# ISLA-UH/quantum-inferno

Measured on AMD Instinct MI355X. Metric: TFR Mpoints/sec (CWT+STX+entropy), higher is better.
Workload: dtype f32; 1 GPU; BASELINE configs[1]: 1 channel(s) per GPU x 2^20 samples @ 1000 Hz, order N=3, CWT+STX+entropy, 48 bands; channels_per_gpu=1, n=1048576, bands=48, engine=auto, world_size=1, backend=none, gather_message_bytes_per_rank=0

## Files before the change

include/qi_tfr.h:

```cpp
#ifndef QI_TFR_H
#define QI_TFR_H

#include <stddef.h>
#include <stdint.h>

#ifdef __cplusplus
extern "C" {
#endif

#define QI_TFR_ABI_VERSION 1

typedef struct qi_plan qi_plan;
typedef void* qi_stream;

typedef enum { QI_F32 = 0, QI_F64 = 1 } qi_dtype;

typedef enum {
  QI_OK = 0,
  QI_ERR_ARG = -1,
  QI_ERR_STATE = -2,
  QI_ERR_HIP = -3,
  QI_ERR_FFT = -4,
  QI_ERR_NOMEM = -5,
  QI_ERR_UNSUPPORTED = -6
} qi_status;

typedef enum {
  QI_BANK_STYX = 0,
  QI_BANK_ATOMS = 1
} qi_bank;

typedef enum {
  QI_ENGINE_AUTO = 0,
  QI_ENGINE_HIPFFT = 1,
  QI_ENGINE_NATIVE = 2
} qi_engine;

typedef struct {
  int64_t n;
  int32_t dtype;
  int32_t device;
  int32_t engine;
  int32_t flags;
  int64_t workspace_bytes;
} qi_plan_desc;

typedef struct {
  void* coef;
  void* bits;
  void* power_band;
  void* power_time;
  void* stats;
  double power_scale;
  double eps;
} qi_tfr_out;

int qi_abi_version(void);
const char* qi_last_error(void);
int qi_device_info(int device, char* name, size_t name_len, int64_t* hbm_bytes, int32_t* compute_units);

int qi_plan_create(qi_plan** plan, const qi_plan_desc* desc);
int qi_plan_destroy(qi_plan* plan);

int qi_plan_set_gabor_bank(qi_plan* plan, int bank, int32_t n_bands, const double* p_re, const double* p_im,
                           const double* omega, const double* amp, qi_stream stream);

int qi_gabor_atoms(int device, int64_t n, int32_t n_bands, const double* p_re, const double* p_im,
                   const double* omega, const double* amp, void* out, qi_stream stream);

int qi_gabor_atoms_at(int device, int64_t n, int32_t n_bands, const double* p_re, const double* p_im,
                      const double* omega, const double* amp, const void* x, void* out, qi_stream stream);

int qi_plan_set_stx_bands(qi_plan* plan, int32_t n_bands, const int64_t* shift_index, const double* sigma);

int64_t qi_plan_bands(const qi_plan* plan, int which );
int64_t qi_plan_stage_bands(const qi_plan* plan, int which, int stage);

int64_t qi_plan_forward_low(const qi_plan* plan, int which );

typedef struct {
  int32_t stage, cls, run_cls, flags;
} qi_band_route;
#define QI_ROUTE_ANALYTIC(f) ((f) & 3)
#define QI_ROUTE_NARROW(f) (((f) >> 2) & 3)
#define QI_ROUTE_NOWRAP 16
#define QI_ROUTE_SPLIT 32
#define QI_ROUTE_PASS2_KIND(f) (((f) >> 6) & 3)
#define QI_ROUTE_BEHIND 256
#define QI_ROUTE_F64_ZOOM 512
int qi_plan_band_route(const qi_plan* plan, int which, int32_t band, int64_t records, qi_band_route* route);

typedef enum {
  QI_STAGE_FORWARD = 0,
  QI_STAGE_MULTIPLY = 1,
  QI_STAGE_INVERSE = 2,
  QI_STAGE_EPILOGUE = 3,
  QI_STAGE_PASS1 = 4,
  QI_STAGE_PASS2 = 5,
  QI_STAGE_BLOCK = 6,
  QI_STAGE_ZOOM = 7,
  QI_STAGE_ZOOM_COARSE = 8,
  QI_STAGE_SMALL = 9,
  QI_STAGE_COUNT = 10
} qi_stage;
int qi_plan_profile(qi_plan* plan, int enable);
int qi_plan_profile_read(qi_plan* plan, double* stage_ms, int64_t* stage_launches, int32_t n_stages);

int qi_cwt(qi_plan* plan, int bank, const void* sig, int64_t n_channels, const qi_tfr_out* out, qi_stream stream);

int qi_stx(qi_plan* plan, const void* sig, int64_t n_channels, const qi_tfr_out* out, qi_stream stream);

int qi_cwt_stx(qi_plan* plan, int bank, const void* sig, int64_t n_channels, const qi_tfr_out* out_cwt,
               const qi_tfr_out* out_stx, qi_stream stream);

int64_t qi_stft_segments(int64_t n, int64_t seg, int64_t hop);
int64_t qi_stft_scratch_bytes(int dtype, int64_t n_channels, int64_t n, int64_t seg, int64_t hop, int64_t nfft);
int qi_stft(int dtype, int device, const void* sig, int64_t n_channels, int64_t n, const void* window, int64_t seg,
            int64_t hop, int64_t nfft, double scale, void* Z, void* bits, double eps, void* scratch,
            int64_t scratch_bytes, qi_stream stream);

int64_t qi_welch_scratch_bytes(int dtype, int64_t n_channels, int64_t n, int64_t seg, int64_t hop, int64_t nfft);
int qi_welch(int dtype, int device, const void* sig, int64_t n_channels, int64_t n, const void* window, int64_t seg,
             int64_t hop, int64_t nfft, double scale, void* pxx, void* scratch, int64_t scratch_bytes,
             qi_stream stream);

int qi_power_marginals(int dtype, int device, const void* power, int64_t n_channels, int64_t n_bands, int64_t n,
                       void* power_band, void* power_time, void* stats, void* scratch, int64_t scratch_bytes,
                       qi_stream stream);
int64_t qi_power_marginals_scratch_bytes(int64_t n_channels, int64_t n_bands, int64_t n);

int qi_log2_offset(int dtype, int device, const void* in, void* out, int64_t n_channels, int64_t count, double eps,
                   const void* ref, qi_stream stream);

int qi_widen(int device, const void* in, void* out, int64_t count, qi_stream stream);

int qi_log2_abs(int dtype, int device, const void* in, int is_complex, void* out, int64_t count, double eps,
                qi_stream stream);

int qi_shannon_panel(int dtype, int device, const void* power, const void* mult, int mode, int64_t n_channels,
                     int64_t n_bands, int64_t n, double deg_free, void* info, void* shannon_bits, void* isnr,
                     void* esnr, qi_stream stream);

int64_t qi_sliding_scratch_bytes(int dtype, int64_t n_channels, int64_t nfft, int64_t n_slices);
int qi_sliding_stft(int dtype, int device, const void* sig, int64_t n_channels, int64_t n, const void* window,
                    int64_t seg, int64_t hop, int64_t nfft, int64_t first, int64_t n_slices, int pad_mode, int detrend,
                    int64_t roll, void* Z, void* real_out, int real_kind, void* scratch, int64_t scratch_bytes,
                    qi_stream stream);
int qi_sliding_istft(int dtype, int device, const void* S, int64_t n_channels, const void* dual_window, int64_t seg,
                     int64_t hop, int64_t nfft, int64_t first, int64_t n_slices, int64_t roll, int64_t k0, int64_t k1,
                     void* out, void* scratch, int64_t scratch_bytes, qi_stream stream);

int qi_shannon_1d(int dtype, int device, const void* marginal, int64_t n_channels, int64_t n, void* info, void* entropy,
                  void* isnr, void* esnr, qi_stream stream);
int64_t qi_shannon_scratch_bytes(int dtype, int64_t n_channels, int64_t n);
int qi_shannon_tdr(int dtype, int device, const void* sig, int64_t n_channels, int64_t n, void* sig_norm, void* marginal,
                   void* scratch, int64_t scratch_bytes, qi_stream stream);
int qi_shannon_fft(int dtype, int device, const void* sig, int64_t n_channels, int64_t n, void* spectrum, void* angle,
                   void* marginal, void* scratch, int64_t scratch_bytes, qi_stream stream);

typedef enum { QI_POOL_NTH = 0, QI_POOL_AVERAGE = 1, QI_POOL_MAX = 2, QI_POOL_MIN = 3, QI_POOL_MEDIAN = 4 } qi_pool_method;
typedef enum { QI_POOL_REAL = 0,
// ... 30 lines not shown
```

quantum_inferno_amd/_lib.py:

```python
import ctypes as C
import os

import torch

_HERE = os.path.dirname(os.path.abspath(__file__))
LIB_PATH = os.environ.get("QI_TFR_LIB") or os.path.join(_HERE, "libqi_tfr.so")

QI_F32, QI_F64 = 0, 1
QI_BANK_STYX, QI_BANK_ATOMS, QI_TABLE_STX = 0, 1, 2
QI_ENGINE_AUTO, QI_ENGINE_HIPFFT, QI_ENGINE_NATIVE = 0, 1, 2
STAGES = ("forward", "multiply", "inverse", "epilogue", "pass1", "pass2", "block", "zoom", "zoom_coarse", "small")
QI_POOL_NTH, QI_POOL_AVERAGE, QI_POOL_MAX, QI_POOL_MIN, QI_POOL_MEDIAN = 0, 1, 2, 3, 4
QI_POOL_REAL, QI_POOL_COMPLEX, QI_POOL_POWER = 0, 1, 2
QI_IIR_BA, QI_IIR_SOS = 0, 1
IIR_MAX = 16
POOL_MEDIAN_MAX = 4096
ROUTE_NOWRAP, ROUTE_SPLIT, ROUTE_BEHIND, ROUTE_F64_ZOOM = 16, 32, 256, 512


def route_analytic(flags):
    return flags & 3


def route_narrow(flags):
    return (flags >> 2) & 3


def route_pass2_kind(flags):
    return (flags >> 6) & 3


class QiError(RuntimeError):
    pass


class PlanDesc(C.Structure):
    _fields_ = [
        ("n", C.c_int64),
        ("dtype", C.c_int32),
        ("device", C.c_int32),
        ("engine", C.c_int32),
        ("flags", C.c_int32),
        ("workspace_bytes", C.c_int64),
    ]


class BandRoute(C.Structure):
    _fields_ = [("stage", C.c_int32), ("cls", C.c_int32), ("run_cls", C.c_int32), ("flags", C.c_int32)]


class TfrOut(C.Structure):
    _fields_ = [
        ("coef", C.c_void_p),
        ("bits", C.c_void_p),
        ("power_band", C.c_void_p),
        ("power_time", C.c_void_p),
        ("stats", C.c_void_p),
        ("power_scale", C.c_double),
        ("eps", C.c_double),
    ]


_P = C.c_void_p
_D = C.POINTER(C.c_double)
_I64 = C.POINTER(C.c_int64)
_i64, _i32, _int, _dbl = C.c_int64, C.c_int32, C.c_int, C.c_double

PROTOTYPES = {
    "qi_abi_version": (_int, []),
    "qi_last_error": (C.c_char_p, []),
    "qi_device_info": (_int, [_int, C.c_char_p, C.c_size_t, _I64, C.POINTER(_i32)]),
    "qi_plan_create": (_int, [C.POINTER(_P), C.POINTER(PlanDesc)]),
    "qi_plan_destroy": (_int, [_P]),
    "qi_plan_set_gabor_bank": (_int, [_P, _int, _i32, _D, _D, _D, _D, _P]),
    "qi_gabor_atoms": (_int, [_int, _i64, _i32, _D, _D, _D, _D, _P, _P]),
    "qi_gabor_atoms_at": (_int, [_int, _i64, _i32, _D, _D, _D, _D, _P, _P, _P]),
    "qi_plan_set_stx_bands": (_int, [_P, _i32, _I64, _D]),
    "qi_plan_bands": (_i64, [_P, _int]),
    "qi_plan_stage_bands": (_i64, [_P, _int, _int]),
    "qi_plan_forward_low": (_i64, [_P, _int]),
    "qi_plan_band_route": (_int, [_P, _int, _i32, _i64, C.POINTER(BandRoute)]),
    "qi_plan_profile": (_int, [_P, _int]),
    "qi_plan_profile_read": (_int, [_P, _D, _I64, _i32]),
    "qi_cwt": (_int, [_P, _int, _P, _i64, C.POINTER(TfrOut), _P]),
    "qi_stx": (_int, [_P, _P, _i64, C.POINTER(TfrOut), _P]),
    "qi_cwt_stx": (_int, [_P, _int, _P, _i64, C.POINTER(TfrOut), C.POINTER(TfrOut), _P]),
    "qi_stft_segments": (_i64, [_i64, _i64, _i64]),
    "qi_stft_scratch_bytes": (_i64, [_int, _i64, _i64, _i64, _i64, _i64]),
    "qi_stft": (_int, [_int, _int, _P, _i64, _i64, _P, _i64, _i64, _i64, _dbl, _P, _P, _dbl, _P, _i64, _P]),
    "qi_stft_out_scratch_bytes": (_i64, [_int, _i64, _i64, _i64, _i64, _i64, _int, _int]),
    "qi_stft_out": (_int, [_int, _int, _P, _i64, _i64, _P, _i64, _i64, _i64, _dbl, C.POINTER(TfrOut), _P, _i64, _P]),
    "qi_welch_scratch_bytes": (_i64, [_int, _i64, _i64, _i64, _i64, _i64]),
    "qi_welch": (_int, [_int, _int, _P, _i64, _i64, _P, _i64, _i64, _i64, _dbl, _P, _P, _i64, _P]),
    "qi_power_marginals": (_int, [_int, _int, _P, _i64, _i64, _i64, _P, _P, _P, _P, _i64, _P]),
    "qi_power_marginals_scratch_bytes": (_i64, [_i64, _i64, _i64]),
    "qi_log2_offset": (_int, [_int, _int, _P, _P, _i64, _i64, _dbl, _P, _P]),
    "qi_widen": (_int, [_int, _P, _P, _i64, _P]),
    "qi_log2_abs": (_int, [_int, _int, _P, _int, _P, _i64, _dbl, _P]),
    "qi_shannon_panel": (_int, [_int, _int, _P, _P, _int, _i64, _i64, _i64, _dbl, _P, _P, _P, _P, _P]),
    "qi_sliding_scratch_bytes": (_i64, [_int, _i64, _i64, _i64]),
    "qi_sliding_stft": (_int, [_int, _int, _P, _i64, _i64, _P, _i64, _i64, _i64, _i64, _i64, _int, _int, _i64, _P, _P, _int, _P, _i64, _P]),
    "qi_sliding_istft": (_int, [_int, _int, _P, _i64, _P, _i64, _i64, _i64, _i64, _i64, _i64, _i64, _i64, _P, _P, _i64, _P]),
    "qi_shannon_1d": (_int, [_int, _int, _P, _i64, _i64, _P, _P, _P, _P, _P]),
    "qi_shannon_scratch_bytes": (_i64, [_int, _i64, _i64]),
    "qi_shannon_tdr": (_int, [_int, _int, _P, _i64, _i64, _P, _P, _P, _i64, _P]),
    "qi_shannon_fft": (_int, [_int, _int, _P, _i64, _i64, _P, _P, _P, _P, _i64, _P]),
    "qi_pool_columns": (_i64, [_i64, _i64, _int]),
    "qi_pool_panel": (_int, [_int, _int, _P, _int, _i64, _i64, _i64, _int, _dbl, _P, _P]),
    "qi_pool_strip": (_int, [_int, _int, _P, _i64, _i64, _i64, _i64, _i64, _dbl, _P, _P, _i64, _P, _P]),
    "qi_pool_strip_stats": (_int, [_int, _P, _i64, _i64, _P, _P]),
    "qi_filtfilt_scratch_bytes": (_i64, [_i64, _i64, _i64]),
    "qi_filtfilt": (_int, [_int, _int, _P, _i64, _i64, _P, _int, _i32, _i32, _D, _D, _i64, _P, _P, _i64, _P]),
}

_lib = None


def _hip_runtimes_mapped():
    try:
        with open("/proc/self/maps") as fh:
            return sorted({ln.split()[-1] for ln in fh if "libamdhip64" in ln})
    except OSError:
        return []


def load():
    global _lib
    if _lib is not None:
        return _lib
    if not os.path.exists(LIB_PATH):
        raise QiError(
            f"{LIB_PATH} is missing: build it with `python -c 'import __graft_entry__ as g; g.build()'` "
            "(hipcc --offload-arch=gfx950).  There is no CPU fallback."
        )
    lib = C.CDLL(LIB_PATH)
    for name, (res, args) in PROTOTYPES.items():
        fn = getattr(lib, name)
        fn.restype = res
        fn.argtypes = args
    rts = _hip_runtimes_mapped()
    if len(rts) > 1:
        raise QiError(f"two HIP runtimes are mapped ({rts}); libqi_tfr.so must share torch's")
    _lib = lib
    return lib


def check(rc):
    if rc != 0:
        msg = load().qi_last_error()
        raise QiError(f"libqi_tfr error {rc}: {msg.decode() if msg else '?'}")


def require_gpu():
    if not torch.cuda.is_available():
        raise QiError("no HIP device visible: the TFR transforms run only on the GPU (no CPU fallback)")
    return load()


def darr(a):
    import numpy as np

    a = np.ascontiguousarray(a, dtype=np.float64)
    return a, a.ctypes.data_as(_D)
# ... 16 lines not shown
```

quantum_inferno_amd/csrc/qi_api.hip:

```cpp
#include "qi_host.hpp"

using namespace qi;
using namespace qi::host;

extern "C" {

int qi_abi_version(void) { return QI_TFR_ABI_VERSION; }
const char* qi_last_error(void) { return qi::last_error(); }

int qi_device_info(int device, char* name, size_t name_len, int64_t* hbm_bytes, int32_t* compute_units) {
  hipDeviceProp_t prop;
  QI_HIP(hipGetDeviceProperties(&prop, device));
  if (name && name_len) snprintf(name, name_len, "%s (%s)", prop.name, prop.gcnArchName);
  if (hbm_bytes) *hbm_bytes = (int64_t)prop.totalGlobalMem;
  if (compute_units) *compute_units = prop.multiProcessorCount;
  return QI_OK;
}

int qi_plan_create(qi_plan** plan, const qi_plan_desc* desc) {
  QI_REQUIRE(plan && desc, "null plan/desc");
  *plan = nullptr;
  QI_REQUIRE(desc->n >= 2 && desc->n <= (1ll << 28), "n = %lld out of range", (long long)desc->n);
  QI_REQUIRE(desc->dtype == QI_F32 || desc->dtype == QI_F64, "bad dtype %d", desc->dtype);
  QI_REQUIRE(desc->engine >= QI_ENGINE_AUTO && desc->engine <= QI_ENGINE_NATIVE, "bad engine %d", desc->engine);
  QI_REQUIRE(desc->flags == 0, "qi_plan_desc.flags = %d: the field is reserved and must be 0", desc->flags);
  if (desc->engine == QI_ENGINE_NATIVE && !(is_pow2(desc->n) && desc->n >= (1 << 18) &&
                                            (desc->dtype == QI_F32 || desc->n == (1 << 20)))) {
    set_error("native engine: float32 records of a power-of-two length >= 2^18, float64 records of 2^20 samples (got n = %lld, dtype %d)",
              (long long)desc->n, desc->dtype);
    return QI_ERR_UNSUPPORTED;
  }
  DeviceGuard g(desc->device);
  if (!g.ok) {
    set_error("hipSetDevice(%d) failed", desc->device);
    return QI_ERR_HIP;
  }
  qi_plan* p = new (std::nothrow) qi_plan();
  QI_REQUIRE(p, "out of host memory");
  p->d = *desc;
  p->n = desc->n;
  p->L = is_pow2(desc->n) ? 2 * desc->n : next_pow2(2 * desc->n - 1);
  if (p->native_kmax > (int64_t)native::kMaxPrunedTerms * native::kN2)
    p->native_kmax = (int64_t)native::kMaxPrunedTerms * native::kN2;
  if (const char* e = tune_env("QI_NATIVE_DEBUG")) p->native_debug = atoi(e);
  if (const char* e = tune_env("QI_NATIVE_FWD")) p->native_fwd = atoi(e);
  if (const char* e = tune_env("QI_NATIVE_FWD_LOW")) p->native_fwd_low = atoi(e);
#ifdef QI_NATIVE_STAMPS
  if (tune_env("QI_NATIVE_STAMPS")) {
    if (hipMalloc((void**)&p->stamps, 65536 * 8 * sizeof(unsigned long long)) != hipSuccess) p->stamps = nullptr;
    if (p->stamps) (void)hipMemset(p->stamps, 0, 65536 * 8 * sizeof(unsigned long long));
    if (hipMalloc((void**)&p->blk_stamps, 65536 * 8 * sizeof(unsigned long long)) != hipSuccess) p->blk_stamps = nullptr;
    if (p->blk_stamps) (void)hipMemset(p->blk_stamps, 0, 65536 * 8 * sizeof(unsigned long long));
  }
#endif
  if (const char* e = tune_env("QI_NATIVE_SHORT")) p->native_short = atoi(e);
  if (const char* e = tune_env("QI_NATIVE_BLOCK")) p->native_block = atoi(e);
  if (const char* e = tune_env("QI_NATIVE_ZOOM")) p->native_zoom = atoi(e);
  if (const char* e = tune_env("QI_NATIVE_ZOOM_LEVELS")) p->native_zoom_max_level = atoi(e);
  if (const char* e = tune_env("QI_NATIVE_SPLIT")) p->native_split = atoi(e);
  if (const char* e = tune_env("QI_NATIVE_FUSE")) p->native_fuse = atoi(e);
  if (const char* e = tune_env("QI_NATIVE_F64")) p->native_f64 = atoi(e);
  if (const char* e = tune_env("QI_NATIVE_Z64")) p->native_z64 = atoi(e);
  if (const char* e = tune_env("QI_NATIVE_Z64_FINE")) p->native_z64_fine = atoi(e);
  if (const char* e = tune_env("QI_NATIVE_Z64_COARSE")) p->native_z64_coarse = atoi(e);
  if (const char* e = tune_env("QI_NATIVE_Z64_BLOCK_FROM")) p->native_z64_block_from = atoi(e);
  if (const char* e = tune_env("QI_NATIVE_BLK64_WTAB")) p->native_blk64_wtab = atoi(e);
  if (const char* e = tune_env("QI_NATIVE_BLK64_NARROW")) p->native_blk64_narrow = atoi(e);
  if (const char* e = tune_env("QI_NATIVE_MIN_LOG2N")) p->native_min_log2n = atoi(e);
  if (desc->dtype == QI_F64) {
    if (!tune_env("QI_NATIVE_MIN_LOG2N")) p->native_min_log2n = 15;
    const int short64 = p->native_short && !(tune_env("QI_NATIVE_SHORT64") && atoi(tune_env("QI_NATIVE_SHORT64")) == 0);
    const int block64 = p->native_block && !(tune_env("QI_NATIVE_BLOCK64") && atoi(tune_env("QI_NATIVE_BLOCK64")) == 0);
    const int split64 = p->native_split && block64 && p->native_z64 &&
                        !(tune_env("QI_NATIVE_SPLIT64") && atoi(tune_env("QI_NATIVE_SPLIT64")) == 0);
    p->native_zoom = 0;
    p->native_split = split64;
    p->native_split_e = 2048;
    p->native_block = block64;
    p->native_short = short64;
    p->native_rows = 8;
    if (p->native_group <= 0) p->native_group = 8;
  }
  p->ws_bytes = desc->workspace_bytes > 0 ? (size_t)desc->workspace_bytes : ((size_t)2 << 30);
  if (hipMalloc((void**)&p->ws, p->ws_bytes) != hipSuccess) {
    set_error("hipMalloc of %zu workspace bytes failed", p->ws_bytes);
    delete p;
    return QI_ERR_HIP;
  }
  if (const char* e = tune_env("QI_SMALL_CHUNK_BANDS")) p->small_chunk_bands = atoi(e);
  if (const char* e = tune_env("QI_SMALL_JOINT")) p->small_joint = atoi(e);
  if (build_small_twiddles(p) != QI_OK) {
    free_device(p->ws);
    delete p;
    return QI_ERR_HIP;
  }
  *plan = p;
  return QI_OK;
}

int qi_plan_destroy(qi_plan* p) {
  if (!p) return QI_OK;
  DeviceGuard g(p->d.device);
  (void)hipDeviceSynchronize();
  p->fft.clear();
  p->prof.clear();
#ifdef QI_NATIVE_STAMPS
  if (p->stamps) {
    std::vector<unsigned long long> h(65536 * 8);
    if (hipMemcpy(h.data(), p->stamps, h.size() * sizeof(unsigned long long), hipMemcpyDeviceToHost) == hipSuccess) {
      double sum[8] = {0};
      long cnt = 0;
      for (size_t w = 0; w < 65536; ++w) {
        unsigned long long tot = 0;
        for (int k = 0; k < 8; ++k) tot += h[w * 8 + k];
        if (!tot) continue;
        ++cnt;
        for (int k = 0; k < 8; ++k) sum[k] += (double)h[w * 8 + k];
      }
      fprintf(stderr, "[qi stamps] last pass-2 launch, %ld workgroups, mean cycles per workgroup: load %.0f | barrier %.0f | "
              "step1 %.0f | barrier %.0f | exchange %.0f | step2 %.0f | epilogue %.0f | loop head %.0f\n", cnt,
              sum[0] / cnt, sum[1] / cnt, sum[2] / cnt, sum[3] / cnt, sum[4] / cnt, sum[5] / cnt, sum[6] / cnt, sum[7] / cnt);
    }
    (void)hipFree(p->stamps);
  }
  if (p->blk_stamps) {
    std::vector<unsigned long long> h(65536 * 8);
    if (hipMemcpy(h.data(), p->blk_stamps, h.size() * sizeof(unsigned long long), hipMemcpyDeviceToHost) == hipSuccess) {
      if (const char* path = tune_env("QI_NATIVE_TIMELINE")) {
        if (FILE* f = fopen(path, "w")) {
// ... 107 lines not shown
  drop_band_slots(p, bank);
  const int rc = build_gabor_bank(p, bank, B, p_re, p_im, omega, amp, use_native, st);
  if (rc == QI_OK) {
    p->nb[bank] = B;
  } else {
    drop_gabor_tables(p, bank);
    free_device(p->bank[bank]);
  }
  return rc;
}

static int atoms_rows(int64_t n, int32_t B, const double* p_re, const double* p_im, const double* omega, const double* amp,
                      const double* x, void* out, hipStream_t st) {
  std::vector<double> host;
  DeviceTemp<double> d_par;
  QI_TRY(upload_atom_params(B, p_re, p_im, omega, amp, &host, &d_par));
  const double* q = d_par.ptr;
  QI_TRY(launch_bank_rows((double2*)out, n, n, 1, q, q + B, q + 2 * B, q + 3 * B, 0, B, st, 0.0, x));
  if (hipStreamSynchronize(st) != hipSuccess) {
    set_error("atom kernel failed: %s", hipGetErrorString(hipGetLastError()));
    return QI_ERR_HIP;
  }
  return QI_OK;
}

int qi_gabor_atoms(int device, int64_t n, int32_t B, const double* p_re, const double* p_im, const double* omega,
                   const double* amp, void* out, qi_stream stream) {
  QI_REQUIRE(p_re && p_im && omega && amp && out, "null argument");
  QI_REQUIRE(n >= 2 && B > 0 && B <= 65535, "bad atom bank shape");
  DeviceGuard g(device);
  return atoms_rows(n, B, p_re, p_im, omega, amp, nullptr, out, (hipStream_t)stream);
}

int qi_gabor_atoms_at(int device, int64_t n, int32_t B, const double* p_re, const double* p_im, const double* omega,
                      const double* amp, const void* x, void* out, qi_stream stream) {
  QI_REQUIRE(p_re && p_im && omega && amp && x && out, "null argument");
  QI_REQUIRE(n >= 1 && B > 0 && B <= 65535, "bad atom bank shape");
  DeviceGuard g(device);
  return atoms_rows(n, B, p_re, p_im, omega, amp, static_cast<const double*>(x), out, (hipStream_t)stream);
}

int qi_plan_set_stx_bands(qi_plan* p, int32_t B, const int64_t* shift_index, const double* sigma) {
  QI_REQUIRE(p && shift_index && sigma, "null argument");
  QI_REQUIRE(B > 0 && B <= 65535, "band count %d out of range", B);
  for (int32_t j = 0; j < B; ++j)
    QI_REQUIRE(shift_index[j] >= 0 && shift_index[j] < p->n, "shift_index[%d] = %lld outside [0, n)", j,
               (long long)shift_index[j]);
  for (int32_t j = 0; j < B; ++j)
    QI_REQUIRE(std::isfinite(sigma[j]) && sigma[j] > 0.0, "sigma[%d] = %g: must be positive and finite", j, sigma[j]);
  DeviceGuard g(p->d.device);
  p->table_gen++;
  if (p->d_stx_idx) {
    QI_HIP(hipDeviceSynchronize());
    QI_HIP(hipFree(p->d_stx_idx));
    QI_HIP(hipFree(p->d_stx_coef));
    p->d_stx_idx = nullptr;
    p->d_stx_coef = nullptr;
    p->nb_stx = 0;
  }
  std::vector<double> coef(B);
  const double k = 2.0 * M_PI / (double)p->n * std::sqrt(0.5 * M_LOG2E);
  for (int32_t j = 0; j < B; ++j) coef[j] = sigma[j] * k;
  QI_TRY(upload_table(&p->d_stx_idx, std::vector<int64_t>(shift_index, shift_index + B)));
  QI_TRY(upload_table(&p->d_stx_coef, coef));
  p->nb_stx = 0;
  drop_stx_tables(p);
  drop_band_slots(p, 2);
  QI_TRY(build_stx_tables(p, B, shift_index, sigma, coef));
  p->nb_stx = B;
  return QI_OK;
}

int64_t qi_plan_bands(const qi_plan* p, int which) {
  if (!p) return 0;
  if (which == QI_BANK_STYX || which == QI_BANK_ATOMS) return p->nb[which];
  return which == 2 ? p->nb_stx : 0;
}

int64_t qi_plan_forward_low(const qi_plan* p, int which) {
  if (!p || which < 0 || which > 2 || !forward_low(p)) return 0;
  return table_low_bins(p, which);
}

int64_t qi_plan_stage_bands(const qi_plan* p, int which, int stage) {
  if (!p || which < 0 || which > 2) return 0;
  const int64_t total = qi_plan_bands(p, which);
  if (on_small(p, which)) return stage == QI_STAGE_SMALL ? total : 0;
  if (!p->nat[which].ready) return stage == QI_STAGE_INVERSE ? total : 0;
  int64_t blk = 0;
  if (which != 1 && p->blk[which].ready) blk = p->blk[which].rows;
  const int64_t zoom = p->nat[which].nzoom + p->nat[which].nz64;
  const int64_t left = which == 2 ? p->stx_left_n : 0;
  if (stage == QI_STAGE_BLOCK) return blk;
  if (stage == QI_STAGE_ZOOM) return zoom;
  if (stage == QI_STAGE_INVERSE) return left;
  return stage == QI_STAGE_PASS2 ? total - blk - zoom - left : 0;
}

int qi_plan_band_route(const qi_plan* p, int which, int32_t band, int64_t records, qi_band_route* route) {
  QI_REQUIRE(p && route, "null argument");
  QI_REQUIRE(which >= 0 && which <= 2, "bad table %d", which);
  QI_REQUIRE(band >= 0 && band < qi_plan_bands(p, which), "band %d outside the table's %lld rows", band,
             (long long)qi_plan_bands(p, which));
  QI_REQUIRE(records > 0, "records must be positive");
  *route = qi_band_route{QI_STAGE_INVERSE, 0, 0, 0};
  const auto& t = p->nat[which];
  if (on_small(p, which)) {
    int32_t lg = 0;
    while (((int64_t)1 << lg) < (which == 0 ? p->L : p->n)) ++lg;
    *route = qi_band_route{QI_STAGE_SMALL, lg, lg, 0};
    return QI_OK;
  }
  if (!t.ready) return QI_OK;
  if (which == 2 && p->stx_left_n > 0 && band >= p->stx_left_lo && band < p->stx_left_lo + p->stx_left_n) {
    route->flags = QI_ROUTE_BEHIND;
    return QI_OK;
  }
  int found = 0;
  const bool split = which == 0 && std::find(p->h_split_bands.begin(), p->h_split_bands.end(), band) != p->h_split_bands.end();
  for (const auto& z : t.h_zoom)
    if (z.first == band) {
      const int run = records < p->native_zoom_short_from && z.second >= native::kZoomLevels ? 0 : z.second;
      *route = qi_band_route{QI_STAGE_ZOOM, z.second, run, split ? QI_ROUTE_SPLIT : 0};
      ++found;
    }
  for (size_t q = 0; q < t.h_z64.size(); ++q)
    if (t.h_z64[q] == band) {
      int level = -1, fine = -1;
      for (int g = 0; g < native::kZ64Levels; ++g)
        if ((int32_t)q >= t.z64_first[g] && (int32_t)q < t.z64_first[g] + t.z64_count[g]) level = g;
      for (int c = 0; c < native::kZ64FineClasses; ++c)
        if ((int32_t)q >= t.zf_first[c] && (int32_t)q < t.zf_first[c] + t.zf_count[c]) fine = c;
      *route = qi_band_route{QI_STAGE_ZOOM, level, fine, QI_ROUTE_F64_ZOOM | (split ? QI_ROUTE_SPLIT : 0)};
      ++found;
    }
  if (which != 1 && p->blk[which].ready) {
    const int cut = records >= batch_from(p) ? 1 : 0;
    for (const auto& b : p->blk[which].var[cut].h_route)
      if (b.out_band == band) {
        *route = qi_band_route{QI_STAGE_BLOCK, b.wq, b.wq, (b.analytic & 3) | ((b.narrow & 3) << 2) | (b.nowrap ? QI_ROUTE_NOWRAP : 0)};
        ++found;
      }
  }
  for (size_t q = 0; q < t.h_rows.size(); ++q)
    if (t.h_rows[q] == band) {
      *route = qi_band_route{QI_STAGE_PASS2, 0, 0, (t.h_row_mode[q] & 3) << 6};
      ++found;
    }
  if (which == 0 && p->nat[3].ready)
    for (int32_t r : p->nat[3].h_rows)
      if (r == band) {
        *route = qi_band_route{QI_STAGE_PASS2, 0, 0, 2 << 6};
        ++found;
      }
  if (found != 1) {
    set_error("band %d of table %d has %d producers", band, which, found);
    return QI_ERR_STATE;
  }
  return QI_OK;
}

int qi_plan_profile(qi_plan* p, int enable) {
  QI_REQUIRE(p, "null plan");
  DeviceGuard g(p->d.device);
  double ms[Profiler::kStages];
  int64_t c[Profiler::kStages];
// ... 152 lines not shown
```

quantum_inferno_amd/csrc/qi_block.hip:

```cpp
#include "qi_common.hpp"
#include "qi_device.hpp"
#include "qi_native.hpp"
#include "qi_fft_reg.hpp"
#include "qi_zoom_gather.hpp"

namespace qi {
namespace native {

namespace {

constexpr int kBlkThreads = 256;
#ifndef QI_BLK_WAVES
#define QI_BLK_WAVES 3
#endif
#ifndef QI_BLK_LONG_WAVES
#define QI_BLK_LONG_WAVES 2
#endif
#ifdef QI_NATIVE_DEBUG
#define QI_BDBG(bit) (a.debug & (bit))
#else
#define QI_BDBG(bit) false
#endif
#ifdef QI_NATIVE_STAMPS
#define QI_BSTAMP(k)                                               \
// ... 194 lines not shown
  fft_reg<T, 16, DIR>(v);
}

template <typename T>
__device__ __forceinline__ void flush_band_sum(const BlockArgs<T>& a, int64_t ch, int64_t blk, int pending, const double* sums,
                                               int tid) {
  if (pending >= 0 && tid == 0) {
    double r = 0.0;
    for (int q = 0; q < kBlkThreads / kWave; ++q) r += sums[q];
    a.part_band[((int64_t)ch * a.panel_bands + pending) * a.nblk + blk] = r;
  }
}

template <typename T>
__device__ __forceinline__ void reduce_stats(const BlockArgs<T>& a, cplx<T>* __restrict__ buf, double r0, double r1, double r2,
                                             int64_t ch, int32_t stat_slot, int tid, bool follows = false, int64_t band_slot = -1) {
  constexpr int NW = kBlkThreads / kWave;
  if (!a.part_stat && band_slot < 0) return;
  const int lane = tid & (kWave - 1), wv = tid / kWave;
  double* fin = reinterpret_cast<double*>(buf);
  if (lane == 0) {
    fin[wv] = r0;
    fin[NW + wv] = r1;
    fin[2 * NW + wv] = r2;
  }
  __syncthreads();
  if (tid == 0) {
    double m = 0.0, s1 = 0.0, s2 = 0.0;
    for (int q = 0; q < NW; ++q) {
      m = fin[q] > m ? fin[q] : m;
      s1 += fin[NW + q];
      s2 += fin[2 * NW + q];
    }
    if (band_slot >= 0 && a.part_band) a.part_band[band_slot] = s1;
    if (a.part_stat) {
      double* o = a.part_stat + ((int64_t)ch * a.stat_stride + a.stat_base + stat_slot) * 3;
      o[0] = follows ? (o[0] > m ? o[0] : m) : m;
      o[1] = follows ? o[1] + s1 : s1;
      o[2] = follows ? o[2] + s2 : s2;
    }
  }
}

template <typename T, bool DEMOD>
__device__ __forceinline__ T gauss_weight(const BlockBandT<T>& bd, int k, bool fold) {
  T dk = (T)(k - bd.kappa_int) - (T)bd.kappa_frac;
  T amp = (T)bd.amp;
  if (fold && dk > (T)(kBlk / 2)) {
    dk -= (T)kBlk;
    if (!DEMOD) amp = -amp;
  }
  if (DEMOD && fold && dk < -(T)(kBlk / 2)) dk += (T)kBlk;
  const T e = (T)bd.cw * dk;
  return amp * fast_exp2(-e * e);
}
template <typename T>
__device__ __forceinline__ T gauss_weight_nowrap(const BlockBandT<T>& bd, T kf) {
  const T e = fma_t((T)bd.cw, kf, -(T)bd.cw * (T)bd.kappa_frac);
  return fast_exp2(fma_t(-e, e, (T)bd.la));
}

template <typename T, bool CIRC>
__device__ __forceinline__ void block_forward(const T* __restrict__ sig, int64_t n, int64_t t0, cplx<T> (&S)[16],
                                              cplx<T>* __restrict__ buf, const cplx<T>* __restrict__ tw256, cplx<T> w,
                                              int tid, int col) {
#pragma unroll
  for (int b = 0; b < 16; ++b) {
    int64_t t = t0 + col + 256 * b;
    T x;
    if (CIRC) {
      t = (t + n) & (n - 1);
      x = sig[t];
    } else {
      x = (t >= 0 && t < n) ? sig[t] : T(0);
    }
    S[b] = mk<T>(x, T(0));
  }
  fft4096<T, -1>(S, buf, tw256, w, tid, col);
  cplx<T> t[16];
#pragma unroll
  for (int c = 0; c < 16; ++c) t[c] = S[brev(c, 4)];
#pragma unroll
  for (int c = 0; c < 16; ++c) S[c] = t[c];
}

template <typename T, int WQ, bool DEMOD, bool COEF, bool BITS, bool EDGE = false>
__device__ __forceinline__ void block_bands(const BlockArgs<T>& a, int32_t blk_i, int32_t band_first, int32_t band_count,
                                            int32_t plane, int32_t stat_slot, cplx<T> (&S)[16], cplx<T>* __restrict__ buf,
                                            const cplx<T>* __restrict__ tw256, double (*s_red)[kBlkThreads / kWave],
                                            cplx<T> w, int col, int edge_piece = 0) {
  static_assert(!EDGE || !DEMOD, "split bands belong to the styx table");
  constexpr int W = 256 * WQ, V = kBlk - 2 * W, NOUT = 16 - 2 * WQ;
  constexpr bool F64 = sizeof(T) == 8;
  const int tid = threadIdx.x, lane = tid & (kWave - 1), wv = tid / kWave;
  const int64_t blk = blk_i, ch = blockIdx.z;
  const int64_t n = a.n;
#ifdef QI_NATIVE_STAMPS
  unsigned long long st_acc[8] = {0, 0, 0, 0, 0, 0, 0, 0};
  unsigned long long st_last = __builtin_amdgcn_s_memtime();
#endif
  const int64_t t0 = blk * V - W;
  if (!DEMOD && !EDGE) {
    const cplx<T> r0 = unit_phasor<T>(-(double)col / (double)kBlk);
    rotate_rows16<T>(S, r0, std::make_integer_sequence<int, 16>{});
  }

  QI_BSTAMP(0);
  T col_p[NOUT];
#pragma unroll
  for (int i = 0; i < NOUT; ++i) col_p[i] = T(0);
  T mx = T(0);
  double plogp = 0.0;
  const uint32_t tb0 = (uint32_t)(t0 + W + col);
  const uint32_t tb_pair = (uint32_t)(t0 + W + kWave * wv + 2 * (lane & 31)) + (lane < 32 ? 0u : 256u);
  int pending = -1, par = 0;

  BlockBandT<T> bd_next{};
  if constexpr (!EDGE) bd_next = load_uniform(a.bands + band_first);
  for (int jj = 0; jj < band_count; ++jj) {
    BlockBandT<T> bd = bd_next;
    if constexpr (EDGE) {
      bd.out_band = a.edge_band[band_first + jj];
    } else {
      if (jj + 1 < band_count) bd_next = load_uniform(a.bands + band_first + jj + 1);
    }
    cplx<T> v[16];
    if (!EDGE && bd.narrow == 1) {
      QI_BSTAMP(1);
      QI_BSTAMP(2);
      const int kres = (col - bd.klo) & 255;
      const int k = (bd.klo + kres) & (kBlk - 1);
      const bool first = (k >> 8) == (bd.klo >> 8);
      const cplx<T> x = pick_pair16<T>(S, __builtin_amdgcn_readfirstlane(bd.klo >> 8), first);
      T r;
      if constexpr (F64) {
        r = a.gauss_w[(int64_t)(band_first + jj) * kBlk + k];
      } else {
        r = gauss_weight<T, DEMOD>(bd, k, true);
      }
      cplx<T> wq = w;
      asm volatile("" : "+v"(wq.x), "+v"(wq.y));
      const cplx<T> om = cmul(wq, first ? mk<T>((T)bd.rot_a[0], (T)bd.rot_a[1]) : mk<T>((T)bd.rot_b[0], (T)bd.rot_b[1]));
      sparse_head16<T>(v, mk<T>(x.x * r, x.y * r), om);
      if (!QI_BDBG(4)) fft4096_tail<T, 1>(v, buf, tw256, tid, col);
    } else if (!EDGE && F64 && a.gauss_w) {
      const T* __restrict__ gw = a.gauss_w + (int64_t)(band_first + jj) * kBlk + col;
      T r[16];
#pragma unroll
      for (int b = 0; b < 16; ++b) r[b] = gw[256 * b];
#pragma unroll
      for (int b = 0; b < 16; ++b) v[b] = mk<T>(S[b].x * r[b], S[b].y * r[b]);
    } else if (!EDGE && (F64 || bd.analytic)) {
      QI_BSTAMP(1);
      QI_BSTAMP(2);
      const bool lower = bd.narrow == 2;
      if (bd.nowrap) {
        const T kf0 = (T)(col - bd.kappa_int);
#pragma unroll
        for (int b = 0; b < 8; ++b) {
          const T r = gauss_weight_nowrap<T>(bd, kf0 + (T)(256 * b));
          v[b] = mk<T>(S[b].x * r, S[b].y * r);
        }
        if (lower) {
#pragma unroll
          for (int b = 8; b < 16; ++b) v[b] = mk<T>(T(0), T(0));
        } else {
// ... 63 lines not shown
    T rowacc = T(0), pl = T(0);
    [[maybe_unused]] const cplx<T> R1 = mk<T>((T)bd.rot[0], (T)bd.rot[1]), R4 = mk<T>((T)bd.rot[4], (T)bd.rot[5]);
    uint32_t tp = tb_pair;
    asm volatile("" : "+v"(tp));
    auto finish_band = [&](auto guard) {
      constexpr bool GUARD = decltype(guard)::value;
      cplx<T> seed = ph, rcur = ph;
#pragma unroll
      for (int i = 0; i < NOUT; i += 2) {
        cplx<T> z[2];
#pragma unroll
        for (int h = 0; h < 2; ++h) {
          z[h] = v[brev(i + h + WQ, 4)];
          if constexpr (DEMOD && F64) {
            if constexpr (COEF)
              if (!QI_BDBG(32)) z[h] = cmul_rn(z[h], cmul_rn(ph, mk<T>(demod_pow[2 * (i + h)], demod_pow[2 * (i + h) + 1])));
          } else if (DEMOD && !QI_BDBG(32)) {
            if (i + h > 0) {
              if (((i + h) & 3) == 0) {
                seed = cmul_rn(seed, R4);
                rcur = seed;
              } else {
                rcur = cmul_rn(rcur, R1);
              }
            }
            z[h] = cmul_rn(z[h], rcur);
          }
        }
        half_swap(z[0].x, z[1].x);
        half_swap(z[0].y, z[1].y);
        const uint32_t tt = tp + 256u * (uint32_t)i;
        const bool inside = !GUARD || tt < (uint32_t)n;
        if constexpr (EDGE) {
          if (inside) {
            const cplx<T> pa = part[tt], pb = part[tt + 1];
            z[0].x += pa.x;
            z[0].y += pa.y;
            z[1].x += pb.x;
            z[1].y += pb.y;
          }
        }
        T lg[2];
#pragma unroll
        for (int h = 0; h < 2; ++h) {
          const T m2 = norm2(z[h].x, z[h].y);
          if (BITS) lg[h] = log2_t(sqrt_t(m2) + a.eps);
          const T p = inside ? mul_rn(a.power_scale, m2) : T(0);
          col_p[i + h] += p;
          rowacc += p;
          mx = max_t(mx, p);
          if constexpr (F64) {
            if (!QI_BDBG(16)) pl += plog2p_flat(p, reinterpret_cast<const double (*)[2]>(tw256 + 256));
          } else {
            if (!QI_BDBG(16)) pl += plog2p(p);
          }
        }
        if (COEF && inside && !QI_BDBG(1)) store_pair(coef_row, tt, z[0], z[1]);
        if (BITS && inside) store_real_pair(bits_row, tt, lg[0], lg[1]);
      }
    };
    if (t0 + W + V > n) finish_band(std::true_type{});
    else finish_band(std::false_type{});
    plogp += (double)pl;
    if (a.part_band && !QI_BDBG(64)) {
      const double r = wave_sum((double)rowacc);
      if (lane == 0) s_red[par][wv] = r;
      pending = bd.out_band;
      par ^= 1;
    }
    QI_BSTAMP(4);
  }
#ifdef QI_NATIVE_STAMPS
  if (a.stamps && tid == 0) {
    unsigned long long* o = a.stamps + ((int64_t)blockIdx.z * gridDim.x + blockIdx.x) * 8;
    for (int k = 0; k < 5; ++k) o[k] = st_acc[k];
    o[5] = (unsigned long long)band_count;
  }
#endif

  T tot = T(0);
  char* __restrict__ time_row = reinterpret_cast<char*>(
      a.time_part ? a.time_part + ((int64_t)ch * a.chunk_total + a.chunk_base + plane) * n : nullptr);
#pragma unroll
  for (int i = 0; i < NOUT; i += 2) {
    tot += col_p[i] + col_p[i + 1];
    const uint32_t tt = tb_pair + 256u * (uint32_t)i;
    if (time_row && tt < (uint32_t)n) store_real_pair(time_row, tt, col_p[i], col_p[i + 1]);
  }
  const double r0 = wave_max((double)mx), r1 = wave_sum((double)tot), r2 = wave_sum(plogp);
  __syncthreads();
  flush_band_sum(a, ch, blk, pending, s_red[par ^ 1], tid);
  reduce_stats(a, buf, r0, r1, r2, ch, stat_slot, tid);
}

template <typename T, int WQ, bool DEMOD, bool COEF, bool BITS>
__device__ __forceinline__ void block_item(const BlockArgs<T>& a, const BlockItem& it, cplx<T>* __restrict__ buf,
                                           const cplx<T>* __restrict__ tw256, double (*s_red)[kBlkThreads / kWave],
                                           cplx<T> w, int col) {
  cplx<T> S[16];
  block_forward<T, DEMOD>(a.sig + (int64_t)blockIdx.z * a.n, a.n, (int64_t)it.block * (kBlk - 512 * WQ) - 256 * WQ, S, buf, tw256,
                          w, threadIdx.x, col);
  block_bands<T, WQ, DEMOD, COEF, BITS>(a, it.block, it.band_first, it.band_count, it.plane, it.stat_slot, S, buf, tw256,
                                        s_red, w, col);
}


template <typename T, bool CIRC>
__device__ __forceinline__ void block_forward8(const T* __restrict__ sig, int64_t n, int64_t t0, cplx<T> (&S)[16],
                                               cplx<T>* __restrict__ buf, const cplx<T>* __restrict__ tw256, cplx<T> w,
                                               cplx<T> w8, int tid, int col) {
  cplx<T> O[16];
#pragma unroll
  for (int par = 1; par >= 0; --par) {
#pragma unroll
    for (int b = 0; b < 16; ++b) {
      int64_t t = t0 + 2 * (col + 256 * b) + par;
      T x;
      if (CIRC) {
        t = (t + n) & (n - 1);
        x = sig[t];
      } else {
        x = (t >= 0 && t < n) ? sig[t] : T(0);
      }
      S[b] = mk<T>(x, T(0));
    }
    fft4096<T, -1>(S, buf, tw256, w, tid, col);
    if (par == 1) {
#pragma unroll
      for (int c = 0; c < 16; ++c) O[c] = S[brev(c, 4)];
    }
  }
  const cplx<T> w8c = cconj<T>(w8);
  cplx<T> t[16];
#pragma unroll
  for (int c = 0; c < 16; ++c) t[c] = S[brev(c, 4)];
  long_combine<T>(S, t, O, w8c, std::make_integer_sequence<int, 16>{});
}

template <typename T, bool DEMOD, bool COEF, bool BITS>
__device__ __forceinline__ void long_bands(const BlockArgs<T>& a, int32_t blk_i, int32_t band_first, int32_t band_count,
                                           int32_t plane, int32_t stat_slot, cplx<T> (&S)[16], cplx<T>* __restrict__ buf,
                                           const cplx<T>* __restrict__ tw256, double (*s_red)[kBlkThreads / kWave],
                                           cplx<T> w, cplx<T> w8, int col) {
  constexpr int W = 1024, V = kBlkLongValid, NOUT = 12, C0 = 2;
  const int tid = threadIdx.x, lane = tid & (kWave - 1), wv = tid / kWave;
  const int64_t blk = blk_i, ch = blockIdx.z, n = a.n;
  const int64_t t0 = blk * V - W;
  if (!DEMOD) {
    float sn, cs;
    sincospif(-(float)col * (1.0f / (float)kBlkLong), &sn, &cs);
    long_rotate<T>(S, mk<T>((T)cs, (T)sn), std::make_integer_sequence<int, 16>{});
  }
  T col_p[2 * NOUT];
#pragma unroll
  for (int i = 0; i < 2 * NOUT; ++i) col_p[i] = T(0);
  T mx = T(0);
  double plogp = 0.0;
  const uint32_t tb0 = (uint32_t)(t0 + 2 * (col + 256 * C0));
  int pending = -1, par = 0;
  BlockBand bd_next = load_uniform(a.bands + band_first);
  for (int jj = 0; jj < band_count; ++jj) {
    const BlockBand bd = bd_next;
    if (jj + 1 < band_count) bd_next = load_uniform(a.bands + band_first + jj + 1);
    const int kres = (col - bd.klo) & 255;
    const int k = (bd.klo + kres) & (kBlk - 1);
    const bool first = (k >> 8) == (bd.klo >> 8);
    const cplx<T> x = pick_pair16<T>(S, __builtin_amdgcn_readfirstlane(bd.klo >> 8), first);
    const T r = gauss_weight<T, DEMOD>(bd, k, false);
    const cplx<T> y = mk<T>(x.x * r, x.y * r);
    cplx<T> wq = w, wq8 = w8;
    asm volatile("" : "+v"(wq.x), "+v"(wq.y), "+v"(wq8.x), "+v"(wq8.y));
    const cplx<T> om = cmul(wq, first ? mk<T>((T)bd.rot_a[0], (T)bd.rot_a[1]) : mk<T>((T)bd.rot_b[0], (T)bd.rot_b[1]));
    const cplx<T> tw_odd = cmul(wq8, first ? mk<T>((T)bd.rot8_a[0], (T)bd.rot8_a[1]) : mk<T>((T)bd.rot8_b[0], (T)bd.rot8_b[1]));
    cplx<T> v[16];
    cplx<T> ph = mk<T>(T(1), T(0)), ph1 = ph;
    if (DEMOD) {
      const uint32_t m = (0u - (uint32_t)bd.shift * tb0) & (uint32_t)(n - 1);
      float s, c;
      sincospif((float)m * a.two_over_n, &s, &c);
      ph = mk<T>((T)c, (T)s);
      ph1 = mk<T>((T)bd.rot1[0], (T)bd.rot1[1]);
    }
    const int64_t orow = ((int64_t)ch * a.panel_bands + bd.out_band) * n;
    char* __restrict__ coef_row = reinterpret_cast<char*>(a.coef ? a.coef + orow : nullptr);
    char* __restrict__ bits_row = reinterpret_cast<char*>(a.bits ? a.bits + orow : nullptr);
    uint32_t tb = tb0;
    asm volatile("" : "+v"(tb));
    T rowacc = T(0), pl = T(0);
    const cplx<T> R1 = mk<T>((T)bd.rot[2], (T)bd.rot[3]), R4 = mk<T>((T)bd.rot[6], (T)bd.rot[7]);
    {
      cplx<T> ze[NOUT];
      sparse_head16<T>(v, y, om);
      fft4096_tail<T, 1>(v, buf, tw256, tid, col);
#pragma unroll
      for (int i = 0; i < NOUT; ++i) ze[i] = v[brev(i + C0, 4)];
      sparse_head16<T>(v, cmul(y, tw_odd), om);
      fft4096_tail<T, 1>(v, buf, tw256, tid, col);
      flush_band_sum(a, ch, blk, pending, s_red[par ^ 1], tid);
      auto finish_band = [&](auto guard) {
      constexpr bool GUARD = decltype(guard)::value;
      cplx<T> seed = ph, rcur = ph;
#pragma unroll
      for (int i = 0; i < NOUT; ++i) {
        cplx<T> z[2] = {ze[i], v[brev(i + C0, 4)]};
        if (DEMOD) {
          if (i > 0) {
            if ((i & 3) == 0) {
              seed = cmul_rn(seed, R4);
              rcur = seed;
            } else {
              rcur = cmul_rn(rcur, R1);
            }
          }
          z[0] = cmul_rn(z[0], rcur);
          z[1] = cmul_rn(z[1], cmul_rn(rcur, ph1));
        }
        const uint32_t tt = tb + 512u * (uint32_t)i;
        const bool inside = !GUARD || tt < (uint32_t)n;
        T lg[2];
#pragma unroll
        for (int hh = 0; hh < 2; ++hh) {
          const T m2 = norm2(z[hh].x, z[hh].y);
          if (BITS) lg[hh] = log2_t(sqrt_t(m2) + a.eps);
          const T p = inside ? mul_rn(a.power_scale, m2) : T(0);
          col_p[2 * i + hh] += p;
          rowacc += p;
          mx = max_t(mx, p);
          pl += plog2p(p);
        }
        if (COEF && inside)
          stream_store(reinterpret_cast<float4*>(coef_row + (size_t)(tt * (uint32_t)sizeof(cplx<T>))),
                       make_float4(z[0].x, z[0].y, z[1].x, z[1].y));
        if (BITS && inside) *reinterpret_cast<float2*>(bits_row + (size_t)(tt * (uint32_t)sizeof(T))) = make_float2(lg[0], lg[1]);
      }
      };
      if (t0 + W + V > n) finish_band(std::true_type{});
      else finish_band(std::false_type{});
    }
    plogp += (double)pl;
    if (a.part_band) {
      const double rs = wave_sum((double)rowacc);
      if (lane == 0) s_red[par][wv] = rs;
      pending = bd.out_band;
      par ^= 1;
    }
  }
  T tot = T(0);
  char* __restrict__ time_row = reinterpret_cast<char*>(
      a.time_part ? a.time_part + ((int64_t)ch * a.chunk_total + a.chunk_base + plane) * n : nullptr);
#pragma unroll
  for (int i = 0; i < NOUT; ++i) {
    tot += col_p[2 * i] + col_p[2 * i + 1];
    const uint32_t tt = tb0 + 512u * (uint32_t)i;
    if (time_row && tt < (uint32_t)n)
      *reinterpret_cast<float2*>(time_row + (size_t)(tt * (uint32_t)sizeof(T))) = make_float2(col_p[2 * i], col_p[2 * i + 1]);
  }
  const double r0 = wave_max((double)mx), r1 = wave_sum((double)tot), r2 = wave_sum(plogp);
  __syncthreads();
  flush_band_sum(a, ch, blk, pending, s_red[par ^ 1], tid);
  reduce_stats(a, buf, r0, r1, r2, ch, stat_slot, tid);
}

template <typename T, bool DEMOD, bool COEF, bool BITS>
__device__ __forceinline__ void long_item(const BlockArgs<T>& a, const BlockItem& it, cplx<T>* __restrict__ buf,
                                          const cplx<T>* __restrict__ tw256, double (*s_red)[kBlkThreads / kWave], cplx<T> w,
                                          cplx<T> w8, int col) {
  cplx<T> S[16];
  block_forward8<T, DEMOD>(a.sig + (int64_t)blockIdx.z * a.n, a.n, (int64_t)it.block * kBlkLongValid - 1024, S, buf, tw256, w, w8,
                           threadIdx.x, col);
  long_bands<T, DEMOD, COEF, BITS>(a, it.block, it.band_first, it.band_count, it.plane, it.stat_slot, S, buf, tw256, s_red, w, w8,
                                   col);
}

template <typename T, bool COEF, bool BITS>
__device__ __forceinline__ void long_dual_item(const BlockArgs<T>& a0, const BlockArgs<T>& a2, const DualItem& it,
                                               cplx<T>* __restrict__ buf, const cplx<T>* __restrict__ tw256,
                                               double (*s_red)[kBlkThreads / kWave], cplx<T> w, cplx<T> w8, int col) {
  const int tid = threadIdx.x;
  const int64_t n = a0.n, t0 = (int64_t)it.block * kBlkLongValid - 1024;
  const bool inside = t0 >= 0 && t0 + kBlkLong <= n;
  const T* sig = a0.sig + (int64_t)blockIdx.z * n;
  cplx<T> S[16];
  if (it.count2 > 0 || inside) block_forward8<T, true>(sig, n, t0, S, buf, tw256, w, w8, tid, col);
  if (it.count2 > 0)
    long_bands<T, true, COEF, BITS>(a2, it.block, it.first2, it.count2, it.plane2, it.slot2, S, buf, tw256, s_red, w, w8, col);
  if (it.count0 > 0) {
    if (!inside) block_forward8<T, false>(sig, n, t0, S, buf, tw256, w, w8, tid, col);
    long_bands<T, false, COEF, BITS>(a0, it.block, it.first0, it.count0, it.plane0, it.slot0, S, buf, tw256, s_red, w, w8, col);
  }
}

template <typename T, int WQ, bool COEF, bool BITS>
__device__ __forceinline__ void dual_item(const BlockArgs<T>& a0, const BlockArgs<T>& a2, const DualItem& it,
                                          cplx<T>* __restrict__ buf, const cplx<T>* __restrict__ tw256,
                                          double (*s_red)[kBlkThreads / kWave], cplx<T> w, int col) {
  const int tid = threadIdx.x;
  const int64_t n = a0.n, t0 = (int64_t)it.block * (kBlk - 512 * WQ) - 256 * WQ;
  const bool inside = t0 >= 0 && t0 + kBlk <= n;
  const T* sig = a0.sig + (int64_t)blockIdx.z * n;
  cplx<T> S[16];
  if (it.count2 > 0 || inside) block_forward<T, true>(sig, n, t0, S, buf, tw256, w, tid, col);
  if (it.count2 > 0)
    block_bands<T, WQ, true, COEF, BITS>(a2, it.block, it.first2, it.count2, it.plane2, it.slot2, S, buf, tw256, s_red, w, col);
  if (it.count0 > 0) {
    if (!inside) block_forward<T, false>(sig, n, t0, S, buf, tw256, w, tid, col);
    block_bands<T, WQ, false, COEF, BITS>(a0, it.block, it.first0, it.count0, it.plane0, it.slot0, S, buf, tw256, s_red, w, col);
  }
}

template <typename T, int WQ, bool COEF, bool BITS>
__device__ __forceinline__ void edge_item(const BlockArgs<T>& a, const BlockItem& it, cplx<T>* __restrict__ buf,
                                          const cplx<T>* __restrict__ tw256, cplx<T> w, int col, bool follows = false) {
  constexpr int W = 256 * WQ, V = kBlk - 2 * W, NOUT = 16 - 2 * WQ;
  const int tid = threadIdx.x;
  const int64_t n = a.n, ch = blockIdx.z, blk = it.block;
  const int sb = it.band_first, out_band = a.edge_band[sb];
  const int64_t t0 = blk * V - W;
  const T* __restrict__ sig = a.sig + ch * n;
  const cplx<T>* __restrict__ bank = a.edge_bank + (int64_t)sb * 2 * kBlk;
  const cplx<T>* __restrict__ part = a.edge_part + (ch * a.nsplit + sb) * n;
  const uint32_t tb = (uint32_t)(t0 + W + col);
  cplx<T> z0[NOUT];
#pragma unroll
  for (int i = 0; i < NOUT; ++i) {
    const uint32_t t = tb + 256u * (uint32_t)i;
    z0[i] = t < (uint32_t)n ? part[t] : mk<T>(T(0), T(0));
  }
  cplx<T> acc[16];
#pragma unroll
  for (int b = 0; b < 16; ++b) acc[b] = mk<T>(T(0), T(0));
  for (int piece = 0; piece < 2; ++piece) {
    const int64_t in0 = t0 + (piece == 0 ? n / 2 - W : -(n / 2 - W));
    if (in0 >= n || in0 + kBlk <= 0) continue;
    cplx<T> S[16];
#pragma unroll
// ... 231 lines not shown
  fft4096<double, 1>(v, buf, tw256, w, tid, col);
  double2* __restrict__ z = a.Z + ((int64_t)ch * a.nbands + band) * (a.M + 2 * kZ64Pad) + kZ64Pad;
#pragma unroll
  for (int c = 0; c < 16; ++c) {
    const int64_t tau = (int64_t)P * (col + 256 * c) + tau1;
    const double2 val = v[brev(c, 4)];
    z[tau] = val;
    if (tau < kZ64Pad) z[a.M + tau] = val;
    if (tau >= a.M - kZ64Pad) z[tau - a.M] = val;
  }
}

template <typename T, bool DEMOD, bool COEF, bool BITS>
__global__ void __launch_bounds__(kBlkThreads, QI_BLK_LONG_WAVES) k_block_long(BlockArgs<T> a, const BlockItem* __restrict__ items) {
  __shared__ cplx<T> buf[kBlkBuf];
  __shared__ cplx<T> tw256[256];
  __shared__ double s_red[2][kBlkThreads / kWave];
  const int tid = threadIdx.x, col = fft4096_col(tid);
  const cplx<T> w = fft4096_setup<T>(tw256, tid, col), w8 = long_setup_w8<T>(col);
  long_item<T, DEMOD, COEF, BITS>(a, load_uniform(items + blockIdx.x), buf, tw256, s_red, w, w8, col);
}
template <typename T, bool COEF, bool BITS>
__global__ void __launch_bounds__(kBlkThreads, QI_BLK_LONG_WAVES) k_block_long_dual(BlockArgs<T> a0, BlockArgs<T> a2,
                                                                                    const DualItem* __restrict__ items) {
  __shared__ cplx<T> buf[kBlkBuf];
  __shared__ cplx<T> tw256[256];
  __shared__ double s_red[2][kBlkThreads / kWave];
  const int tid = threadIdx.x, col = fft4096_col(tid);
  const cplx<T> w = fft4096_setup<T>(tw256, tid, col), w8 = long_setup_w8<T>(col);
  long_dual_item<T, COEF, BITS>(a0, a2, load_uniform(items + blockIdx.x), buf, tw256, s_red, w, w8, col);
}

template <typename T, bool COEF, bool BITS>
__global__ void __launch_bounds__(kBlkThreads, QI_BLK_WAVES) k_block_dual(BlockArgs<T> a0, BlockArgs<T> a2,
                                                                         const DualItem* __restrict__ items) {
  __shared__ cplx<T> buf[kBlkBuf];
  __shared__ cplx<T> tw256[256];
  __shared__ double s_red[2][kBlkThreads / kWave];
  const int tid = threadIdx.x, col = fft4096_col(tid);
  const cplx<T> w = fft4096_setup<T>(tw256, tid, col);
  const DualItem it = load_uniform(items + blockIdx.x);
#ifdef QI_NATIVE_STAMPS
  const unsigned long long wall0 = __builtin_amdgcn_s_memrealtime();
#endif
  if (it.wq < 0) {
    const BlockItem e{it.wq, it.block, it.first0, it.count0, it.plane0, it.slot0};
    QI_WITH_REACH(-it.wq, edge_item<T, WQ, COEF, BITS>(a0, e, buf, tw256, w, col));
  } else {
    QI_WITH_REACH(it.wq, dual_item<T, WQ, COEF, BITS>(a0, a2, it, buf, tw256, s_red, w, col));
  }
#ifdef QI_NATIVE_STAMPS
  if (a0.stamps && tid == 0) {
    asm volatile("s_waitcnt vmcnt(0) lgkmcnt(0)" ::: "memory");
    unsigned long long* o = a0.stamps + ((int64_t)blockIdx.z * gridDim.x + blockIdx.x) * 8;
    unsigned hw;
    asm volatile("s_getreg_b32 %0, hwreg(HW_REG_HW_ID)" : "=s"(hw));
    unsigned xcc;
    asm volatile("s_getreg_b32 %0, hwreg(HW_REG_XCC_ID)" : "=s"(xcc));
    o[6] = (wall0 & 0xffffffffffffull) | ((unsigned long long)(xcc & 15) << 56) | ((unsigned long long)((hw >> 8) & 0xff) << 48);
    o[7] = (__builtin_amdgcn_s_memrealtime() & 0xffffffffffffull) | ((unsigned long long)(it.wq & 0xff) << 56) |
           ((unsigned long long)((it.count0 + it.count2) & 0xff) << 48);
  }
#endif
}

template <typename T>
__device__ __forceinline__ void zoom_coarse_plane(cplx<T>* __restrict__ plane0) {
  __shared__ cplx<T> buf[kBlkBuf];
  __shared__ cplx<T> tw256[256];
  const int tid = threadIdx.x, col = fft4096_col(tid);
  cplx<T>* __restrict__ plane = plane0 + col;
  cplx<T> v[16];
#pragma unroll
  for (int b = 0; b < 16; ++b) v[b] = plane[256 * b];
  const cplx<T> w = fft4096_setup<T>(tw256, tid, col);
  fft4096<T, 1>(v, buf, tw256, w, tid, col);
#pragma unroll
  for (int c = 0; c < 16; ++c) plane[256 * c] = v[brev(c, 4)];
}
template <typename T, bool STX, int NF>
__device__ __forceinline__ void zoom_coarse_plane_gather(const ZoomArgs<T>& a, const uint32_t plane_i,
                                                         cplx<T>* __restrict__ buf, cplx<T>* __restrict__ tw256) {
  const int tid = threadIdx.x, col = fft4096_col(tid);
  const BandDesc bd = load_uniform(a.bands + *as_const(a.plane_band + plane_i));
  const uint32_t tau1 = plane_i - (uint32_t)bd.edge;
  const int64_t ch = blockIdx.z;
  const cplx<T>* __restrict__ X = a.X + ch * ((int64_t)a.x_mask + 1);
  cplx<T> v[16];
#ifdef QI_NATIVE_DEBUG
  if (a.debug & 256) {
#pragma unroll
    for (int b = 0; b < 16; ++b) v[b] = mk<T>((T)(col + b), (T)tau1);
  } else
#endif
  zoom_gather16<T, STX, NF>(a, bd, tau1, col, X, v);
  const cplx<T> w = fft4096_setup<T>(tw256, tid, col);
#ifdef QI_NATIVE_DEBUG
  if (!(a.debug & 512))
#endif
  fft4096<T, 1>(v, buf, tw256, w, tid, col);
  cplx<T>* __restrict__ plane = a.coarse + ((int64_t)ch * a.planes + plane_i) * kBlk + col;
#ifdef QI_NATIVE_DEBUG
  if ((a.debug & 1024) && v[3].x != (T)12345.678f) return;
#endif
#pragma unroll
  for (int c = 0; c < 16; ++c) plane[256 * c] = v[brev(c, 4)];
}
template <typename T, int NF>
__global__ void __launch_bounds__(kBlkThreads) k_zoom_coarse2g(ZoomArgs<T> a0, ZoomArgs<T> a2) {
  __shared__ cplx<T> buf[kBlkBuf];
  __shared__ cplx<T> tw256[256];
#ifdef QI_COARSE_PLAIN_ORDER
  const uint32_t pi = blockIdx.x;
#else
  const uint32_t q = blockIdx.x >> 3, pi = (q >> 3) * 64u + (blockIdx.x & 7u) * 8u + (q & 7u);
#endif
  if (pi >= (uint32_t)(a0.planes + a2.planes)) return;
  if (pi < (uint32_t)a0.planes) zoom_coarse_plane_gather<T, false, NF>(a0, pi, buf, tw256);
  else zoom_coarse_plane_gather<T, true, NF>(a2, pi - (uint32_t)a0.planes, buf, tw256);
}
template <typename T, bool STX>
__global__ void __launch_bounds__(kBlkThreads) k_zoom_coarse_g(ZoomArgs<T> a) {
  __shared__ cplx<T> buf[kBlkBuf];
  __shared__ cplx<T> tw256[256];
  zoom_coarse_plane_gather<T, STX, 8>(a, blockIdx.x, buf, tw256);
}

template <typename T>
__global__ void __launch_bounds__(kBlkThreads) k_zoom_coarse(ZoomArgs<T> a) {
  zoom_coarse_plane<T>(a.coarse + ((int64_t)blockIdx.z * a.planes + blockIdx.x) * kBlk);
}
template <typename T>
__global__ void __launch_bounds__(kBlkThreads) k_zoom_coarse2(ZoomArgs<T> a0, ZoomArgs<T> a2) {
  const bool first = blockIdx.x < (uint32_t)a0.planes;
  const ZoomArgs<T>& a = first ? a0 : a2;
  const int64_t plane = first ? blockIdx.x : blockIdx.x - (uint32_t)a0.planes;
  zoom_coarse_plane<T>(a.coarse + ((int64_t)blockIdx.z * a.planes + plane) * kBlk);
}

__global__ void k_block_taps_gabor(double2* __restrict__ g, int w, const double* __restrict__ par, int nb_total,
                                   const int32_t* __restrict__ ids) {
  const int j = ids[blockIdx.y];
  const double p_re = par[j], p_im = par[nb_total + j], omega = par[2 * nb_total + j], amp = par[3 * nb_total + j];
  double2* row = g + (int64_t)blockIdx.y * kBlk;
  for (int m = blockIdx.x * blockDim.x + threadIdx.x; m < kBlk; m += gridDim.x * blockDim.x) {
    int u;
    bool on = true;
    if (m <= w) u = -m;
    else if (m > kBlk - w) u = kBlk - m;
    else { u = 0; on = false; }
    double2 v = make_double2(0.0, 0.0);
    if (on) {
      const double x = (double)u + 0.5;
      const double env = amp * exp(-p_re * x * x);
      const double ph = omega * x - p_im * x * x;
      double s, c;
      sincos(ph, &s, &c);
      v = make_double2(env * c, -env * s);
    }
    row[m] = v;
  }
}


__global__ void k_block_taps_edge(double2* __restrict__ g, int w, int64_t n, double taper_e,
                                  const double* __restrict__ par, int nb_total, const int32_t* __restrict__ ids) {
  const int j = ids[blockIdx.y >> 1], piece = blockIdx.y & 1;
// ... 307 lines not shown
```

quantum_inferno_amd/csrc/qi_host.hpp:

```cpp
#pragma once
#include <algorithm>
#include <cmath>
#include <cstring>
#include <map>
#include <mutex>
#include <new>
#include <tuple>
#include <vector>

#include <cstdlib>

#include "qi_common.hpp"
#include "qi_native.hpp"

namespace qi {

struct DeviceGuard {
  int prev = -1;
  bool ok = true;
  explicit DeviceGuard(int dev) {
    if (hipGetDevice(&prev) != hipSuccess) prev = -1;
    if (prev != dev) ok = hipSetDevice(dev) == hipSuccess;
  }
  ~DeviceGuard() {
// ... 136 lines not shown
      }
    }
    for (auto e : used) pool.push_back(e);
    used.clear();
    spans.clear();
    cur = last = -1;
  }
  void clear() {
    double ms[kStages];
    int64_t c[kStages];
    read(ms, c);
    for (auto e : pool) (void)hipEventDestroy(e);
    pool.clear();
  }
};

template <typename P>
inline void free_device(P*& ptr) {
  if (ptr) (void)hipFree(ptr);
  ptr = nullptr;
}
template <typename P, typename X>
inline int upload_table(P** dst, const std::vector<X>& v) {
  QI_HIP(hipMalloc((void**)dst, v.size() * sizeof(X)));
  QI_HIP(hipMemcpy(*dst, v.data(), v.size() * sizeof(X), hipMemcpyHostToDevice));
  return QI_OK;
}
template <typename X>
struct DeviceTemp {
  X* ptr = nullptr;
  DeviceTemp() = default;
  DeviceTemp(const DeviceTemp&) = delete;
  DeviceTemp& operator=(const DeviceTemp&) = delete;
  ~DeviceTemp() { free_device(ptr); }
};

extern std::mutex g_stft_mu;
extern std::map<int, FftCache> g_stft_fft;
const char* last_error();

}

using namespace qi;

struct FusedCarry {
  bool active = false;
  size_t ws_used = 0;
  native::BlockArgs<float> blk{};
  int demod = 0;
  int64_t ct = 0;
  native::TailCall<float> tail;
  bool has_zoom = false;
  native::ZoomArgs<float> zoom{};
};

struct qi_plan {
  qi_plan_desc d{};
  int64_t n = 0;
  int64_t L = 0;
  void* bank[2] = {nullptr, nullptr};
  int32_t nb[2] = {0, 0};
  int64_t* d_stx_idx = nullptr;
  double* d_stx_coef = nullptr;
  int32_t nb_stx = 0;
  char* ws = nullptr;
  size_t ws_bytes = 0;
  FftCache fft;
  Profiler prof;
  struct NativeGroup {
    int32_t first = 0, count = 0;
    int32_t gen_first = 0, ngen = 0;
  };
  struct NativeTable {
    bool ready = false;
    int64_t Lf = 0;
    int32_t nbands = 0, ngen = 0, imd_slots = 0;
    native::BandDesc* d_bands = nullptr;
    int32_t* d_gen_list = nullptr;
    std::vector<NativeGroup> groups;
    void* Hc = nullptr;
    void* Hfull = nullptr;
    native::BandDesc* d_zoom = nullptr;
    int32_t* d_zoom_plane_band = nullptr;
    std::vector<std::pair<int32_t, int32_t>> h_zoom;
    std::vector<int32_t> h_rows;
    std::vector<int32_t> h_row_mode;
    std::vector<int32_t> h_z64;
    int32_t nzoom = 0, zoom_count[native::kZoomClasses] = {0, 0, 0, 0, 0, 0, 0};
    int64_t x_lo = 0, x_hi = -1;
    int64_t zoom_planes = 0;
    int zoom_max_level = 0;
    native::BandDesc* d_z64 = nullptr;
    int32_t nz64 = 0, z64_first[native::kZ64Levels] = {}, z64_count[native::kZ64Levels] = {};
    int32_t zf_first[native::kZ64FineClasses] = {}, zf_count[native::kZ64FineClasses] = {};
    double2* d_z64_lane_ph = nullptr;
    double2* d_z64_wave_ph = nullptr;
    void release() {
      free_device(d_z64);
      free_device(d_z64_lane_ph);
      free_device(d_z64_wave_ph);
      free_device(d_zoom);
      free_device(d_zoom_plane_band);
      free_device(d_bands);
      free_device(d_gen_list);
      free_device(Hc);
      free_device(Hfull);
      *this = NativeTable();
    }
  } nat[4];
  struct BlockTable {
    bool ready = false;
    int demod = 0;
    void* bank = nullptr;
    int32_t rows = 0;
    struct ItemList {
      void* d_bands = nullptr;
      void* d_demod_pow = nullptr;
      void* d_gauss_w = nullptr;
      std::vector<std::pair<int32_t, int32_t>> h_bands;
      struct Route {
        int32_t out_band, wq, analytic, narrow, nowrap;
      };
      std::vector<Route> h_route;
      native::BlockItem* d_items = nullptr;
      int32_t nitems = 0, nplanes = 0;
      int32_t nlong = 0;
      int32_t nedge_items = 0;
      bool edge_merged = false;
      std::vector<native::BlockItem> h_items;
    } var[2];
    int64_t max_blocks = 0;
    void release() {
      free_device(bank);
      for (auto& v : var) {
        free_device(v.d_bands);
        free_device(v.d_demod_pow);
        free_device(v.d_gauss_w);
        free_device(v.d_items);
      }
      *this = BlockTable();
    }
  } blk[3];
  struct {
    int64_t C = -1, tile = 0;
    unsigned flags = 0;
    uint64_t gen = 0;
  } tile_cache;
  uint64_t table_gen = 1;
  int native_block = 1;
  const void* shared_sig = nullptr;
  int64_t shared_C = 0;
  bool shared_valid = false;
  int32_t* d_band_slots[3][2] = {};
  int native_zoom = 1;
  int native_zoom_short = 1;
  int native_zoom_short_from = 4;
  int native_zoom_max_level = 3;
  int native_zoom_waves = 2048;
  int native_zoom_wgs_joint = 768;
  int native_zoom_wgs = 0;
  float* d_zoom_w[native::kZoomClasses] = {};
  int native_z64 = 1;
  int native_z64_levels = native::kZ64Levels;
  double* d_z64_w[native::kZ64Levels] = {};
  double* d_z64f_w[native::kZ64FineClasses] = {};
  double2* d_demod_t1 = nullptr;
  double2* d_demod_t2 = nullptr;
  int native_z64_fine = 1;
  int32_t stx_left_lo = -1, stx_left_n = 0;
  void* small_tw = nullptr;
  int small_chunk_bands = 2;
  int small_joint = 2;
  int native_min_log2n = 14;
  int native_blk64_narrow = 1;
  int native_blk64_wtab = 1;
  int native_z64_block_from = 4;
  int native_z64_coarse = 3;
  int native_z64_rows = 0;
  int native_f64 = 1;
  int native_gather_fused = 1;
  hipStream_t side = nullptr;
  hipEvent_t ev_fork = nullptr, ev_join = nullptr;
  int native_split = 1;
  int64_t native_split_e = 1024;
  void* split_bank = nullptr;
  int32_t* d_split_bands = nullptr;
  std::vector<int32_t> h_split_bands;
  int32_t nsplit = 0;
  int native_blk_analytic = 1;
  FusedCarry carry;
  native::DualItem* d_dual[2] = {nullptr, nullptr};
  int32_t n_dual[2] = {0, 0};
  int32_t n_dual_long[2] = {0, 0};
  bool dual_valid[2] = {false, false};
  int native_fuse = 4;
  int native_blk_narrow = 1;
  int native_blk_fastw = 1;
  int native_edge_merge = 1;
  int native_blk_long = 1;
  int native_blk_half = 1;
  int native_tail = 1;
  int64_t native_tile = 0;
  int native_blk_maxwq = 4;
  int native_blk_bands = 6;
  int native_blk_bands_batch = 12;
  int native_blk_batch_from = 0;
  native::EdgeBand* d_edge = nullptr;
  int32_t nedge = 0;
  int64_t edge_wmax = 0;
  int native_short = 1;
  int64_t native_kmax = 12288;
  int native_debug = 0;
  int native_fwd = 1;
  int native_fwd_low = 1;
  int native_wgs = 256;
  unsigned long long* stamps = nullptr;
  unsigned long long* blk_stamps = nullptr;
  int native_group = 0;
  int native_rows = 16;
};

namespace qi {
namespace host {

inline size_t align_up(size_t v, size_t a = 256) { return (v + a - 1) / a * a; }
inline double power_scale_or_default(double power_scale) { return power_scale == 0.0 ? 1.0 : power_scale; }
inline double eps_or_default(double eps) { return eps == 0.0 ? 2.220446049250313e-16 : eps; }
enum class Kind { Linear, Circular, Stockwell };
#ifdef QI_HOST_SANITIZE
void layout_begin(const qi_plan* p, const char* run, bool keep_previous);
void layout_note(const qi_plan* p, const char* what, const void* ptr, size_t bytes, bool shared = false);
#define QI_LAYOUT_BEGIN(p, run, keep) ::qi::host::layout_begin(p, run, keep)
#define QI_LAYOUT_NOTE(p, what, ptr, bytes, ...) ::qi::host::layout_note(p, what, ptr, bytes, ##__VA_ARGS__)
#else
#define QI_LAYOUT_BEGIN(p, run, keep) ((void)0)
#define QI_LAYOUT_NOTE(p, what, ptr, bytes, ...) ((void)0)
#endif
constexpr int kZoomListOrder[native::kZoomClasses] = {6, 5, 0, 1, 2, 3, 4};

bool native_len_ok(int64_t Lf);
bool native_wanted(const qi_plan* p, int kind);
int64_t table_low_bins(const qi_plan* p, int kind);
bool forward_low(const qi_plan* p);
int batch_from(const qi_plan* p);
void release_styx_extras(qi_plan* p);
void drop_gabor_tables(qi_plan* p, int bank);
void drop_stx_tables(qi_plan* p);
void drop_band_slots(qi_plan* p, int kind);
int upload_atom_params(int32_t B, const double* p_re, const double* p_im, const double* omega, const double* amp,
                       std::vector<double>* host, DeviceTemp<double>* d_par);
template <typename T>
int build_native_bank(qi_plan* p, int bank, int32_t B, const double* d_par, const double* h_par, hipStream_t st);
template <typename T>
int build_bank(qi_plan* p, int bank, int32_t B, const double* d_par, hipStream_t st);
int build_stx_tables(qi_plan* p, int32_t B, const int64_t* shift_index, const double* sigma, const std::vector<double>& coef);

bool small_wanted(const qi_plan* p, int kind);
bool on_small(const qi_plan* p, int kind);
int build_small_twiddles(qi_plan* p);

template <typename T>
int run_transform(qi_plan* p, Kind kind, const void* sig_v, int64_t C, const qi_tfr_out* out, hipStream_t st);
template <typename T>
int run_native(qi_plan* p, int kind, const void* sig_v, int64_t C, const qi_tfr_out* out, hipStream_t st,
               bool may_share = false, FusedCarry* defer = nullptr, FusedCarry* finish = nullptr, size_t* probe = nullptr);
template <typename T>
int run_stx_leftover(qi_plan* p, const void* sig, int64_t C, const qi_tfr_out* out, hipStream_t st);
template <typename T>
int run_small(qi_plan* p, int njobs, const int* kinds, const qi_tfr_out* const* outs, const void* sig_v, int64_t C, hipStream_t st,
              bool* ran);
int run_native64(qi_plan* p, int kind, const void* sig_v, int64_t C, const qi_tfr_out* out, hipStream_t st);
int flush_carry(qi_plan* p, FusedCarry* c, hipStream_t st);

}
}
```

quantum_inferno_amd/csrc/qi_native.hip:

```cpp
#include <utility>

#include "qi_common.hpp"
#include "qi_device.hpp"
#include "qi_native.hpp"
#include "qi_fft_reg.hpp"
#include "qi_finalize.hpp"

namespace qi {
namespace native {

namespace {

template <typename T, int G_ = 16>
struct Cfg {
  static constexpr int NR = 1024, G = G_, TH = 64 * G_;
  static constexpr int SR = NR + 1;
  static constexpr int SA = 16 * G + 1;
  static constexpr int BUF = (G * SR > 64 * SA) ? G * SR : 64 * SA;
  static constexpr int TW1 = (kMaxPrunedTerms + 1) * G;
  static constexpr int TW2 = 64;
  static constexpr size_t LDS_BYTES = ((size_t)BUF + NR + TW2 + TW1) * sizeof(cplx<T>) + 256;
};

#ifdef QI_NATIVE_DEBUG
// ... 464 lines not shown
    T rowacc = T(0), pl = T(0);
    if (KIND == 1 && !COEF && bd.edge > 0 && a.edge_z) {
      cplx<T>* ez = a.edge_z + ((int64_t)ch * a.nedge + bd.edge_slot) * 2 * a.edge_wmax;
      const uint32_t t_lo = tb, t_hi = (uint32_t)a.n - 1u - (tb + 15u * tstep);
      if (t_lo < (uint32_t)bd.edge) ez[t_lo] = u[brev(8, 4)];
      if (t_hi < (uint32_t)bd.edge) ez[a.edge_wmax + t_hi] = u[brev(7, 4)];
    }
#pragma unroll
    for (int i = 0; i < NOUT; ++i) {
      const int c = KIND == 0 ? i + 4 : (KIND == 1 ? ((i + 8) & 15) : i);
      const cplx<T> z = u[brev(c, 4)];
      const uint32_t tt = tb + (uint32_t)i * tstep;
      if (COEF && !QI_DBG(1)) stream_store(reinterpret_cast<cplx<T>*>(coef_row + (size_t)(tt * (uint32_t)sizeof(cplx<T>))), z);
      const T m2 = norm2(z.x, z.y);
      if (BITS) *reinterpret_cast<T*>(bits_row + (size_t)(tt * (uint32_t)sizeof(T))) = log2_t(sqrt_t(m2) + a.eps);
      T p = mul_rn(a.power_scale, m2);
      if (KIND == 1) {
        const bool inside = (uint32_t)(tt - (uint32_t)bd.edge) < (uint32_t)(a.n - 2 * (int64_t)bd.edge);
        p = inside ? p : T(0);
      }
      col[i] += p;
      if (!QI_DBG(8)) {
        rowacc += p;
        mx = max_t(mx, p);
        pl += plog2p(p, ltab);
      }
    }
    plogp += (double)pl;
    if (a.part_band) {
      const double r = wave_sum((double)rowacc);
      if (lane == 0) s_red[par][wv] = r;
      pending = j;
      par ^= 1;
    }
    QI_STAMP(6);
  }
#ifdef QI_NATIVE_STAMPS
  if (a.stamps && tid == 0) {
    unsigned long long* o = a.stamps + ((((int64_t)ch * gridDim.y + blockIdx.y) * gridDim.x + blockIdx.x) * 8);
    for (int k = 0; k < 8; ++k) o[k] = st_acc[k];
  }
#endif

  __syncthreads();
  if (pending >= 0 && tid == 0) {
    double s = 0.0;
    for (int w = 0; w < C::TH / kWave; ++w) s += s_red[par ^ 1][w];
    a.part_band[((int64_t)ch * a.panel_bands + pending) * a.nblk + grp] = s;
  }
  T tot = T(0);
  char* __restrict__ time_row =
      reinterpret_cast<char*>(a.time_part ? a.time_part + ((int64_t)ch * a.chunk_total + a.chunk_base + blockIdx.y) * a.n
                                          : nullptr);
#pragma unroll
  for (int i = 0; i < NOUT; ++i) {
    tot += col[i];
    const uint32_t tt = tbase + (uint32_t)i * tstep;
    if (time_row) *reinterpret_cast<T*>(time_row + (size_t)(tt * (uint32_t)sizeof(T))) = col[i];
  }
  if (a.part_stat) {
    const double r0 = wave_max((double)mx), r1 = wave_sum((double)tot), r2 = wave_sum(plogp);
    if (lane == 0) {
      s_fin[0][wv] = r0;
      s_fin[1][wv] = r1;
      s_fin[2][wv] = r2;
    }
    __syncthreads();
    if (tid == 0) {
      double m = 0.0, s1 = 0.0, s2 = 0.0;
      for (int w = 0; w < C::TH / kWave; ++w) {
        m = s_fin[0][w] > m ? s_fin[0][w] : m;
        s1 += s_fin[1][w];
        s2 += s_fin[2][w];
      }
      double* o = a.part_stat + ((int64_t)ch * a.stat_stride + (int64_t)(a.chunk_base + blockIdx.y) * a.stat_nblk + grp) * 3;
      o[0] = m;
      o[1] = s1;
      o[2] = s2;
    }
  }
}

template <typename T, int VEC>
__device__ __forceinline__ void time_reduce_block(const T* __restrict__ part, T* __restrict__ out, int64_t n, int nchunk,
                                                  const T* __restrict__ edge_time, int64_t wmax, int64_t bx, int64_t gx,
                                                  int64_t c) {
  struct alignas(sizeof(T) * VEC) Pack {
    T v[VEC];
  };
  for (int64_t t = (bx * blockDim.x + threadIdx.x) * VEC; t < n; t += gx * blockDim.x * VEC) {
    if (t + VEC <= n) {
      Pack s = *reinterpret_cast<const Pack*>(part + (c * nchunk) * n + t);
      for (int q = 1; q < nchunk; ++q) {
        const Pack x = *reinterpret_cast<const Pack*>(part + (c * nchunk + q) * n + t);
#pragma unroll
        for (int i = 0; i < VEC; ++i) s.v[i] += x.v[i];
      }
      if (edge_time) {
#pragma unroll
        for (int i = 0; i < VEC; ++i) {
          if (t + i < wmax) s.v[i] += edge_time[(c * 2 + 0) * wmax + t + i];
          if (t + i >= n - wmax) s.v[i] += edge_time[(c * 2 + 1) * wmax + (n - 1 - t - i)];
        }
      }
      *reinterpret_cast<Pack*>(out + c * n + t) = s;
    } else {
      for (int64_t u = t; u < n; ++u) {
        T s = T(0);
        for (int q = 0; q < nchunk; ++q) s += part[(c * nchunk + q) * n + u];
        if (edge_time) {
          if (u < wmax) s += edge_time[(c * 2 + 0) * wmax + u];
          if (u >= n - wmax) s += edge_time[(c * 2 + 1) * wmax + (n - 1 - u)];
        }
        out[c * n + u] = s;
      }
    }
  }
}
template <typename T, int VEC>
__global__ void __launch_bounds__(256) k_time_reduce(const T* __restrict__ part, T* __restrict__ out, int64_t n, int nchunk,
                                                     const T* __restrict__ edge_time, int64_t wmax) {
  time_reduce_block<T, VEC>(part, out, n, nchunk, edge_time, wmax, blockIdx.x, gridDim.x, blockIdx.y);
}

struct TailFin {
  const double* part_band;
  const double* part_stat;
  double* power_band;
  double* stats;
  int64_t B, nblk, nstat;
  const int32_t* band_slots;
};
template <typename T, int VEC>
__global__ void __launch_bounds__(256) k_tail(const T* __restrict__ part, T* __restrict__ out, int64_t n, int nchunk,
                                              const T* __restrict__ edge_time, int64_t wmax, TailFin f, int nfin) {
  __shared__ double s[3][256 / kWave];
  if ((int)blockIdx.x < nfin) {
    finalize_block(f.part_band, f.part_stat, f.power_band, f.stats, f.B, f.nblk, f.nstat, f.band_slots, blockIdx.x,
                   blockIdx.y, s);
    return;
  }
  time_reduce_block<T, VEC>(part, out, n, nchunk, edge_time, wmax, (int64_t)blockIdx.x - nfin, (int64_t)gridDim.x - nfin,
                            blockIdx.y);
}

template <typename T>
__global__ void k_even_bins(const cplx<T>* __restrict__ x2, cplx<T>* __restrict__ x1, int64_t n) {
  const int64_t k = (int64_t)blockIdx.x * blockDim.x + threadIdx.x, c = blockIdx.y;
  if (k < n) x1[c * n + k] = x2[c * 2 * n + 2 * k];
}

template <typename T>
__global__ void __launch_bounds__(256) k_edge_fix(EdgeArgs<T> a) {
  const int lane = threadIdx.x & (kWave - 1), wv = threadIdx.x / kWave;
  const int64_t e = blockIdx.y, c = blockIdx.z;
  const EdgeBand eb = a.bands[e];
  const int64_t o = (int64_t)blockIdx.x * (256 / kWave) + wv;
  const int side = o >= a.wmax ? 1 : 0;
  const int64_t tloc = o - (int64_t)side * a.wmax;
  if (tloc >= eb.w) return;
  const int64_t cnt = eb.w - tloc;
  const int64_t t = side ? a.n - 1 - tloc : tloc;
  const T* __restrict__ sig = a.sig + c * a.n;
  T sr = T(0), si = T(0);
  const int64_t m0 = side ? 0 : a.n - eb.w + t;
  const double x0 = (side ? (double)(1 + tloc) : (double)(-eb.w)) + 0.5;
  const int64_t chunk = (cnt + kWave - 1) / kWave;
  if constexpr (sizeof(T) == 8) {
    for (int64_t i = lane; i < cnt; i += kWave) {
      const double x = x0 + (double)i;
      const double ph = eb.omega * x - eb.p_im * x * x;
      const double turns = ph * 0.15915494309189535;
      double sn, cs;
      sincospi(2.0 * (turns - rint(turns)), &sn, &cs);
      const double env = eb.amp * exp(-(eb.p_re * x * x));
      const double v = (double)sig[m0 + i] * env;
      sr += (T)(v * cs);
      si -= (T)(v * sn);
    }
  } else if (eb.p_im == 0.0 && chunk >= 4) {
    const int64_t i0 = (int64_t)lane * chunk;
    const int64_t i1 = i0 + chunk < cnt ? i0 + chunk : cnt;
    if (i0 < i1) {
      const double x = x0 + (double)i0;
      const double turns = eb.omega * x * 0.15915494309189535;
      float sn, cs, sw, cw;
      sincospif(2.0f * (float)(turns - rint(turns)), &sn, &cs);
      const double tw_ = eb.omega * 0.15915494309189535;
      sincospif(2.0f * (float)(tw_ - rint(tw_)), &sw, &cw);
      float env = (float)eb.amp * expf(-(float)(eb.p_re * x * x));
      float ratio = expf(-(float)(eb.p_re * (2.0 * x + 1.0)));
      const float ratio2 = expf(-(float)(2.0 * eb.p_re));
      float pr = cs, pi = -sn;
      for (int64_t i = i0; i < i1; ++i) {
        const T v = sig[m0 + i] * (T)env;
        sr += v * (T)pr;
        si += v * (T)pi;
        const float nr = pr * cw + pi * sw;
        pi = pi * cw - pr * sw;
        pr = nr;
        env *= ratio;
        ratio *= ratio2;
      }
    }
  } else {
    for (int64_t i = lane; i < cnt; i += kWave) {
      const double x = x0 + (double)i;
      const double ph = eb.omega * x - eb.p_im * x * x;
      const double turns = ph * 0.15915494309189535;
      float sn, cs;
      sincospif(2.0f * (float)(turns - rint(turns)), &sn, &cs);
      const float env = (float)eb.amp * expf(-(float)(eb.p_re * x * x));
      const T v = sig[m0 + i] * (T)env;
      sr += v * (T)cs;
      si -= v * (T)sn;
    }
  }
  sr = wave_sum(sr);
  si = wave_sum(si);
  if (lane == 0) {
    const int64_t row = (c * a.panel_bands + eb.out_band) * a.n;
    cplx<T> z = a.coef ? a.coef[row + t] : a.edge_z[((c * a.nedge + e) * 2 + side) * a.wmax + tloc];
    z.x -= sr;
    z.y -= si;
    if (a.coef) a.coef[row + t] = z;
// ... 186 lines not shown

template <typename T, class C1, bool LOW>
static int launch_forward_p1(const RowArgs<T>& a0, int64_t n_channels, hipStream_t st) {
  RowArgs<T> a = a0;
  a.phase_split = a.N1 == 2048 && (a.N2 / C1::G) * n_channels < 256 ? 1 : 0;
  dim3 g1((unsigned)(a.N2 / C1::G), a.phase_split ? 2u : 1u, (unsigned)n_channels);
  if (a.N1 == 1024) return launch_p1<T, C1, 2, 1, LOW>(a, g1, st);
  if (a.N1 == 2048) return launch_p1<T, C1, 2, 2, LOW>(a, g1, st);
  set_error("native forward transform supports N1 = 1024 or 2048, got %lld", (long long)a.N1);
  return QI_ERR_UNSUPPORTED;
}
template <typename T, class C1>
static int launch_forward_cfg(const RowArgs<T>& a, cplx<T>* Xout, int64_t n_channels, hipStream_t st) {
  using C2 = C1;
  QI_TRY((launch_forward_p1<T, C1, false>(a, n_channels, st)));
  auto kern = k_fwd2<T, C2>;
  QI_TRY(allow_dynamic_lds(reinterpret_cast<const void*>(kern), C2::LDS_BYTES));
  dim3 g2((unsigned)(a.N1 / C2::G), 1, (unsigned)n_channels);
  kern<<<g2, C2::TH, C2::LDS_BYTES, st>>>(a, Xout);
  QI_LAUNCH_CHECK();
  return QI_OK;
}
template <typename T, class C2>
static int launch_fwd2_low(const RowArgs<T>& a, cplx<T>* Xlow, int64_t n_channels, hipStream_t st) {
  auto kern = k_fwd2_low<T, C2>;
  QI_TRY(allow_dynamic_lds(reinterpret_cast<const void*>(kern), C2::LDS_BYTES));
  dim3 g2((unsigned)ceil_div(fwd_low_rows(a.N1), C2::G), 1, (unsigned)n_channels);
  kern<<<g2, C2::TH, C2::LDS_BYTES, st>>>(a, Xlow);
  QI_LAUNCH_CHECK();
  return QI_OK;
}
template <>
int launch_forward<float>(const RowArgs<float>& a, float2* Xout, int64_t n_channels, hipStream_t st, bool low) {
  const bool few = n_channels * (a.N2 / 16) < 256;
  if (!low) {
    if (few) return launch_forward_cfg<float, Cfg<float, 8>>(a, Xout, n_channels, st);
    return launch_forward_cfg<float, Cfg<float, 16>>(a, Xout, n_channels, st);
  }
  if (few) QI_TRY((launch_forward_p1<float, Cfg<float, 8>, true>(a, n_channels, st)));
  else QI_TRY((launch_forward_p1<float, Cfg<float, 16>, true>(a, n_channels, st)));
  const int64_t rows = fwd_low_rows(a.N1) * n_channels;
  if (rows >= 256 * 16) return launch_fwd2_low<float, Cfg<float, 16>>(a, Xout, n_channels, st);
  if (rows >= 256 * 8) return launch_fwd2_low<float, Cfg<float, 8>>(a, Xout, n_channels, st);
  return launch_fwd2_low<float, Cfg<float, 4>>(a, Xout, n_channels, st);
}
template <>
int launch_forward<double>(const RowArgs<double>& a, double2* Xout, int64_t n_channels, hipStream_t st, bool low) {
  if (low) {
    set_error("the low-bins forward transform is float32 only");
    return QI_ERR_UNSUPPORTED;
  }
  return launch_forward_cfg<double, Cfg<double, 8>>(a, Xout, n_channels, st);
}

template <typename T, class C>
static int launch_pass2_cfg(const RowArgs<T>& a, int kind, int nchunk, int64_t n_channels, hipStream_t st) {
  dim3 grid((unsigned)(a.N1 / C::G), (unsigned)nchunk, (unsigned)n_channels);
  switch (kind) {
    case 0: return launch_p2<T, C, 0>(a, grid, st);
    case 1: return launch_p2<T, C, 1>(a, grid, st);
    default: return launch_p2<T, C, 2>(a, grid, st);
  }
}
template <>
int launch_pass2<double>(const RowArgs<double>& a, int kind, int rows_per_group, int nchunk, int64_t n_channels,
                         hipStream_t st) {
  if (rows_per_group != 8) {
    set_error("float64 pass 2 runs 8 rows per workgroup, got %d", rows_per_group);
    return QI_ERR_UNSUPPORTED;
  }
  return launch_pass2_cfg<double, Cfg<double, 8>>(a, kind, nchunk, n_channels, st);
}

template <>
int launch_pass2<float>(const RowArgs<float>& a, int kind, int rows_per_group, int nchunk, int64_t n_channels,
                        hipStream_t st) {
  if (rows_per_group == 16) return launch_pass2_cfg<float, Cfg<float, 16>>(a, kind, nchunk, n_channels, st);
  if (rows_per_group == 8) return launch_pass2_cfg<float, Cfg<float, 8>>(a, kind, nchunk, n_channels, st);
  set_error("pass 2 supports 8 or 16 rows per workgroup, got %d", rows_per_group);
  return QI_ERR_UNSUPPORTED;
}

template <typename T>
int launch_time_reduce(const T* part, T* out, int64_t C, int64_t n, int nchunk, const T* edge_time, int64_t wmax,
                       hipStream_t st) {
  const bool aligned = n % 4 == 0 && reinterpret_cast<uintptr_t>(out) % (4 * sizeof(T)) == 0 &&
                       reinterpret_cast<uintptr_t>(part) % (4 * sizeof(T)) == 0;
  if (aligned) {
    dim3 g((unsigned)(ceil_div(n, 1024) > 4096 ? 4096 : ceil_div(n, 1024)), (unsigned)C);
    k_time_reduce<T, 4><<<g, 256, 0, st>>>(part, out, n, nchunk, edge_time, wmax);
  } else {
    dim3 g((unsigned)(ceil_div(n, 256) > 4096 ? 4096 : ceil_div(n, 256)), (unsigned)C);
    k_time_reduce<T, 1><<<g, 256, 0, st>>>(part, out, n, nchunk, edge_time, wmax);
  }
  QI_LAUNCH_CHECK();
  return QI_OK;
}
template <typename T>
struct TailPack {
  const T* part;
  T* out;
  int64_t n;
  int nchunk, nfin;
  TailFin f;
};
template <typename T, int VEC>
__global__ void __launch_bounds__(256) k_tail2(TailPack<T> p0, TailPack<T> p1) {
  __shared__ double s[3][256 / kWave];
  const TailPack<T>& p = blockIdx.z == 0 ? p0 : p1;
  if ((int)blockIdx.x < p.nfin) {
    finalize_block(p.f.part_band, p.f.part_stat, p.f.power_band, p.f.stats, p.f.B, p.f.nblk, p.f.nstat, p.f.band_slots,
                   blockIdx.x, blockIdx.y, s);
    return;
  }
  time_reduce_block<T, VEC>(p.part, p.out, p.n, p.nchunk, nullptr, 0, (int64_t)blockIdx.x - p.nfin,
                            (int64_t)gridDim.x - p.nfin, blockIdx.y);
}

template <typename T>
int launch_tail(const TailCall<T>& t, hipStream_t st) {
  const bool aligned = t.n % 4 == 0 && reinterpret_cast<uintptr_t>(t.out_time) % (4 * sizeof(T)) == 0 &&
                       reinterpret_cast<uintptr_t>(t.time_part) % (4 * sizeof(T)) == 0;
  if (!aligned) {
    if (int rc = launch_time_reduce<T>(t.time_part, t.out_time, t.ct, t.n, t.chunk_total, t.edge_time, t.wmax, st)) return rc;
    return launch_finalize(t.part_band, t.part_stat, t.power_band, t.stats, t.ct, t.B, t.nbk, t.stat_slots, st, t.band_slots);
  }
  const TailFin f{t.part_band, t.part_stat, t.power_band, t.stats, t.B, t.nbk, t.stat_slots, t.band_slots};
  const int nfin = (int)t.B + 1;
  const int64_t gt = ceil_div(t.n, 1024) > 4096 ? 4096 : ceil_div(t.n, 1024);
  dim3 g((unsigned)(gt + nfin), (unsigned)t.ct);
  k_tail<T, 4><<<g, 256, 0, st>>>(t.time_part, t.out_time, t.n, t.chunk_total, t.edge_time, t.wmax, f, nfin);
  QI_LAUNCH_CHECK();
  return QI_OK;
}

template <typename T>
int launch_tail2(const TailCall<T>& t0, const TailCall<T>& t1, hipStream_t st) {
  const int64_t n = t1.n;
  const bool aligned = n % 4 == 0 && reinterpret_cast<uintptr_t>(t0.out_time) % 16 == 0 &&
                       reinterpret_cast<uintptr_t>(t0.time_part) % 16 == 0 && reinterpret_cast<uintptr_t>(t1.out_time) % 16 == 0 &&
                       reinterpret_cast<uintptr_t>(t1.time_part) % 16 == 0;
  if (!aligned) {
    if (int rc = launch_tail<T>(t0, st)) return rc;
    return launch_tail<T>(t1, st);
  }
  TailPack<T> p0{t0.time_part, t0.out_time, n, t0.chunk_total, (int)t0.B + 1,
                 TailFin{t0.part_band, t0.part_stat, t0.power_band, t0.stats, t0.B, t0.nbk, t0.stat_slots, t0.band_slots}};
  TailPack<T> p1{t1.time_part, t1.out_time, n, t1.chunk_total, (int)t1.B + 1,
                 TailFin{t1.part_band, t1.part_stat, t1.power_band, t1.stats, t1.B, t1.nbk, t1.stat_slots, t1.band_slots}};
  const int64_t gt = ceil_div(n, 1024) > 4096 ? 4096 : ceil_div(n, 1024);
  const int nfin = p0.nfin > p1.nfin ? p0.nfin : p1.nfin;
  dim3 g((unsigned)(gt + nfin), (unsigned)t1.ct, 2);
  k_tail2<T, 4><<<g, 256, 0, st>>>(p0, p1);
  QI_LAUNCH_CHECK();
  return QI_OK;
}
template int launch_tail2<float>(const TailCall<float>&, const TailCall<float>&, hipStream_t);
template int launch_tail2<double>(const TailCall<double>&, const TailCall<double>&, hipStream_t);
template int launch_tail<float>(const TailCall<float>&, hipStream_t);
template int launch_tail<double>(const TailCall<double>&, hipStream_t);
template int launch_time_reduce<float>(const float*, float*, int64_t, int64_t, int, const float*, int64_t, hipStream_t);
template int launch_time_reduce<double>(const double*, double*, int64_t, int64_t, int, const double*, int64_t,
                                        hipStream_t);

template <typename T>
int launch_even_bins(const cplx<T>* x2, cplx<T>* x1, int64_t C, int64_t n, hipStream_t st) {
  dim3 g((unsigned)ceil_div(n, 256), (unsigned)C);
  k_even_bins<T><<<g, 256, 0, st>>>(x2, x1, n);
  QI_LAUNCH_CHECK();
  return QI_OK;
}
template int launch_even_bins<float>(const float2*, float2*, int64_t, int64_t, hipStream_t);
template int launch_even_bins<double>(const double2*, double2*, int64_t, int64_t, hipStream_t);

template <typename T>
int launch_edge(const EdgeArgs<T>& a, int64_t C, T* edge_time, double* part_band, int64_t nblk, int64_t band_slot,
                double* part_stat, int64_t stat_slot, hipStream_t st) {
  if (a.nedge <= 0) return QI_OK;
  dim3 g((unsigned)ceil_div(2 * a.wmax, 256 / kWave), (unsigned)a.nedge, (unsigned)C);
  k_edge_fix<T><<<g, 256, 0, st>>>(a);
  QI_LAUNCH_CHECK();
  dim3 gr((unsigned)(a.nedge + ceil_div(2 * a.wmax, 256)), (unsigned)C);
  k_edge_reduce<T><<<gr, 256, 0, st>>>(a, edge_time, part_band, nblk, band_slot, part_stat, stat_slot);
  QI_LAUNCH_CHECK();
  return QI_OK;
}
template int launch_edge<float>(const EdgeArgs<float>&, int64_t, float*, double*, int64_t, int64_t, double*, int64_t,
                                hipStream_t);
template int launch_edge<double>(const EdgeArgs<double>&, int64_t, double*, double*, int64_t, int64_t, double*, int64_t,
                                 hipStream_t);

int launch_band_support(const double2* F, int64_t L, int nb, double thr2, double* out, hipStream_t st) {
  k_band_support<<<nb, 256, 0, st>>>(F, L, thr2, out);
  QI_LAUNCH_CHECK();
  return QI_OK;
}

template <typename T>
int launch_copy_window(const double2* F, cplx<T>* dst, int64_t k_lo, int64_t count, int conj, double scale,
                       int64_t row_len, hipStream_t st, double ramp, int64_t ramp_center) {
  k_copy_window<T><<<(unsigned)ceil_div(count, 256), 256, 0, st>>>(F, dst, k_lo, count, conj, scale, row_len, ramp, ramp_center);
  QI_LAUNCH_CHECK();
  return QI_OK;
}
template int launch_copy_window<float>(const double2*, float2*, int64_t, int64_t, int, double, int64_t, hipStream_t, double,
                                       int64_t);
template int launch_copy_window<double>(const double2*, double2*, int64_t, int64_t, int, double, int64_t, hipStream_t,
                                        double, int64_t);

}
}
```

quantum_inferno_amd/csrc/qi_native.hpp:

```cpp
#pragma once
#include "qi_common.hpp"

namespace qi {
namespace native {

constexpr int kN2 = 1024;
constexpr int kMaxPrunedTerms = 16;

struct BandDesc {
  int32_t mode;
  int32_t k_lo;
  int32_t k_len;
  int32_t gen_slot;
  int32_t out_band;
  int32_t bank_row;
  int32_t edge;
  int32_t edge_slot;
  int32_t add_row;
  int32_t pad_;
  int64_t src_off;
  int64_t shift;
  double coef;
};

// ... 43 lines not shown
template <typename T>
int launch_pass2(const RowArgs<T>& a, int kind, int rows_per_group, int nchunk, int64_t n_channels, hipStream_t st);
struct EdgeBand {
  int32_t out_band, w;
  double p_re, p_im, omega, amp;
};
template <typename T>
struct EdgeArgs {
  const EdgeBand* bands;
  int32_t nedge, panel_bands;
  int64_t n, wmax, stat_slots;
  const T* sig;
  cplx<T>* coef;
  cplx<T>* edge_z;
  T* bits;
  T* edge_p;
  T power_scale, eps;
};

constexpr int kBlk = 4096;
template <typename R>
struct BlockBandT {
  int32_t out_band;
  int32_t bank_row;
  int32_t shift;
  int32_t analytic;
  R rot[8];
  int32_t kappa_int;
  R kappa_frac, cw, amp;
  int32_t narrow, klo;
  R rot_a[2], rot_b[2];
  R rot8_a[2], rot8_b[2];
  R rot1[2];
  int32_t nowrap;
  R la;
};
using BlockBand = BlockBandT<float>;

constexpr int kBlkLongWq = 8;
constexpr int kBlkLong = 2 * kBlk;
constexpr int kBlkLongValid = kBlkLong - 2048;
struct BlockItem {
  int32_t wq;
  int32_t block;
  int32_t band_first, band_count;
  int32_t plane;
  int32_t stat_slot;
};
struct DualItem {
  int32_t wq, block;
  int32_t first0, count0, plane0, slot0;
  int32_t first2, count2, plane2, slot2;
};
template <typename T>
struct BlockArgs {
  int64_t n;
  int32_t nitems, panel_bands;
  int32_t nedge_items, nsplit;
  int32_t edge_merged;
  int32_t edge_wq;
  int32_t nlong;
  const int32_t* edge_band;
  const cplx<T>* edge_bank;
  const cplx<T>* edge_part;
  const BlockItem* items;
  const BlockBandT<T>* bands;
  const cplx<T>* bank;
  const T* gauss_w;
  const cplx<T>* demod_pow;
  const cplx<T>* demod_t1;
  const cplx<T>* demod_t2;
  const T* sig;
  cplx<T>* coef;
  T* bits;
  T* time_part;
  double* part_band;
  double* part_stat;
  int64_t nblk, stat_stride, stat_base;
  int32_t chunk_base, chunk_total;
  T power_scale, eps;
  float two_over_n;
  int32_t debug;
  unsigned long long* stamps;
};
int block_valid(int wq);
template <typename T>
int launch_block(const BlockArgs<T>& a, int demod, int64_t n_channels, hipStream_t st, hipStream_t side = nullptr,
                 hipEvent_t fork = nullptr, hipEvent_t join = nullptr);
template <typename T>
int launch_block_dual(const BlockArgs<T>& a0, const BlockArgs<T>& a2, const DualItem* items, int32_t nitems, int32_t nlong,
                      int32_t n_edge, int64_t n_channels, hipStream_t st);
int launch_block_taps_gabor(double2* g, int w, const double* d_par, int nb_total, const int32_t* d_ids, int count,
                            hipStream_t st);
int launch_block_taps_stx(double2* g, int w, const double2* om, int64_t n, int64_t idx, hipStream_t st);
int launch_stx_window_row(double2* row, int64_t n, double coef, hipStream_t st);
int launch_block_rotate_rows(double2* rows, int count, hipStream_t st);

int launch_block_taps_edge(double2* g, int w, int64_t n, double taper_e, const double* d_par, int nb_total,
                           const int32_t* d_ids, int count, hipStream_t st);

constexpr int kZoomD = 64;
constexpr int kZoomLevels = 5;
constexpr int kZoomClasses = 7;
constexpr int zoom_grid(int cls) { return cls < kZoomLevels ? cls : 0; }
constexpr int zoom_ntap(int cls) { return cls < kZoomLevels ? 10 : (cls == 5 ? 6 : 4); }
constexpr int zoom_design_oversampling(int cls) { return cls < kZoomLevels ? 4 : (cls == 5 ? 8 : 32); }
constexpr int zoom_span(int cls) { return 1 << zoom_grid(cls); }
constexpr int zoom_taps(int cls) { return zoom_ntap(cls) + zoom_span(cls) - 1; }
constexpr int zoom_steps(int cls) { return zoom_grid(cls) <= 2 ? 16 : (64 >> zoom_grid(cls)); }
constexpr int kZoomOversample = 4;
template <typename T>
struct ZoomArgs {
  int64_t n, Lf;
  int64_t planes;
  int32_t nbands, panel_bands;
  const BandDesc* bands;
  const int32_t* plane_band;
  int32_t lvl_first[kZoomClasses], lvl_count[kZoomClasses], lvl_chunk0[kZoomClasses], lvl_nchunk[kZoomClasses];
  int64_t lvl_stat_base[kZoomClasses];
  const float* lvl_weights[kZoomClasses];
  const cplx<T>* X;
  int32_t x_shift;
  uint32_t x_mask;
  const cplx<T>* Hc;
  cplx<T>* split_part;
  int32_t split_rows;
  int32_t debug;
  cplx<T>* coarse;
  int32_t stx;
  int32_t lane_off;
  int64_t tau_off;
  T inv_len;
  float two_over_len;
  cplx<T>* coef;
  T* bits;
  T* time_part;
  double* part_band;
  double* part_stat;
  int64_t nblk, stat_stride;
  int32_t chunk_base, chunk_total;
  T power_scale, eps;
};
int64_t zoom_groups(int64_t n, int level);
template <typename T>
int launch_zoom_gather(const ZoomArgs<T>& a, int64_t n_channels, hipStream_t st);
template <typename T>
int launch_zoom_coarse(const ZoomArgs<T>& a, int64_t n_channels, hipStream_t st);
template <typename T>
int launch_zoom(const ZoomArgs<T>& a, int64_t n_channels, hipStream_t st);
template <typename T>
int launch_zoom_gather2(const ZoomArgs<T>& a0, const ZoomArgs<T>& a2, int64_t n_channels, hipStream_t st);
template <typename T>
int launch_zoom2(const ZoomArgs<T>& a0, const ZoomArgs<T>& a2, int64_t n_channels, hipStream_t st);
template <typename T>
int launch_zoom_coarse2(const ZoomArgs<T>& a0, const ZoomArgs<T>& a2, int64_t n_channels, hipStream_t st);
template <typename T>
int launch_zoom_coarse_gather(const ZoomArgs<T>& a, int64_t n_channels, hipStream_t st);
template <typename T>
int launch_zoom_coarse_gather2(const ZoomArgs<T>& a0, const ZoomArgs<T>& a2, int64_t n_channels, hipStream_t st);
constexpr int kZ64Taps = 16;
#ifndef QI_Z64_TILE
#define QI_Z64_TILE 2048
#endif
constexpr int kZ64Tile = QI_Z64_TILE;
constexpr int kZ64Levels = 5;
constexpr int kZ64Pad = 16;
struct Z64Args {
  int64_t Lf, n, M;
  int32_t log2d, kind;
  int32_t nbands, panel_bands;
  const BandDesc* bands;
  const cplx<double>* X;
  const cplx<double>* Hc;
  cplx<double>* Z;
  const double* weights;
  double inv_len;
  float two_over_len;
  cplx<double>* coef;
  double* bits;
  cplx<double>* split_part;
  int32_t split_rows;
  double* time_part;
  double* part_band;
  double* part_stat;
  int64_t nblk, stat_stride;
  int64_t pb_stride, stat_nblk;
  int32_t chunk_base, chunk_total;
  double power_scale, eps;
};
int launch_z64_gather(const Z64Args& a, int64_t n_channels, hipStream_t st);
int launch_z64_interp(const Z64Args& a, int nchunk, int64_t n_channels, hipStream_t st);
int launch_z64_pad(cplx<double>* Z, int64_t M, int64_t rows, hipStream_t st);
int launch_z64_coarse(const Z64Args& a, int64_t n_channels, hipStream_t st);
void z64_weights(int log2d, double* w );

constexpr int kZ64FineLevels = 2;
constexpr int kZ64FineClasses = kZ64FineLevels + 4;
constexpr int z64f_level(int c) { return c < kZ64FineLevels ? c : 0; }
constexpr int z64f_ntap(int c) { return c < kZ64FineLevels ? 16 : 12 - 2 * (c - kZ64FineLevels); }
constexpr int z64f_oversampling(int c) { return c < kZ64FineLevels ? 4 : (8 << (c - kZ64FineLevels)); }
constexpr int z64f_span(int c) { return 1 << z64f_level(c); }
constexpr int z64f_win(int c) { return z64f_ntap(c) + z64f_span(c) - 1; }
constexpr int kZ64FineSteps = 16;
constexpr int kZ64FineWave = 64 * kZ64FineSteps;
struct Z64FineArgs {
  Z64Args z;
  int32_t cls;
  int32_t nrow;
  int32_t lvl_bands;
  int32_t lvl_index0;
  const double* w;
  const cplx<double>* lane_ph;
  const cplx<double>* wave_ph;
  int32_t debug;
};
int launch_z64_fine(const Z64FineArgs& a, int64_t n_channels, hipStream_t st);
void z64_fine_weights(int cls, double* w );

void zoom_weights(int level, int lane_off, float* w );
void chebyshev_taps(int N, long double band, long double x, long double* out );

constexpr int kSmallMinLog2 = 10, kSmallMaxLog2 = 14;
constexpr size_t kSmallLdsBytes = 128 * 1024;
bool small_len_ok(int64_t L, size_t elem_bytes);
template <typename T>
struct SmallArgs {
  const cplx<T>* X;
  const cplx<T>* H;
  const int64_t* stx_idx;
  const double* stx_coef;
  const cplx<T>* tw;
  int32_t tw_shift;
  int32_t kind;
  int32_t n, L, off;
  int32_t B, nchunk;
  int32_t chunk_total;
  cplx<T>* coef;
  T* bits;
  T* time_part;
  double* part_band;
  double* part_stat;
  T power_scale, eps;
};
template <typename T>
int launch_small_band(const SmallArgs<T>& a, int64_t ct, hipStream_t st);
template <typename T>
int launch_small_forward(const T* sig, cplx<T>* X2, cplx<T>* X1, const cplx<T>* tw, int64_t tw_len, int64_t n, int64_t ct,
                         hipStream_t st);

template <typename T>
int launch_time_reduce(const T* part, T* out, int64_t C, int64_t n, int nchunk, const T* edge_time, int64_t wmax,
                       hipStream_t st);
template <typename T>
struct TailCall {
  const T* time_part = nullptr;
  T* out_time = nullptr;
  int64_t ct = 0, n = 0;
  int chunk_total = 0;
  const T* edge_time = nullptr;
  int64_t wmax = 0;
  const double* part_band = nullptr;
  const double* part_stat = nullptr;
  double* power_band = nullptr;
  double* stats = nullptr;
  int64_t B = 0, nbk = 0, stat_slots = 0;
  const int32_t* band_slots = nullptr;
};
template <typename T>
int launch_tail(const TailCall<T>& t, hipStream_t st);
template <typename T>
int launch_tail2(const TailCall<T>& t0, const TailCall<T>& t1, hipStream_t st);
template <typename T>
int launch_even_bins(const cplx<T>* x2, cplx<T>* x1, int64_t C, int64_t n, hipStream_t st);
template <typename T>
int launch_edge(const EdgeArgs<T>& a, int64_t C, T* edge_time, double* part_band, int64_t nblk, int64_t band_slot,
                double* part_stat, int64_t stat_slot, hipStream_t st);
int launch_band_support(const double2* F, int64_t L, int nb, double thr2, double* out, hipStream_t st);
template <typename T>
int launch_copy_window(const double2* F, cplx<T>* dst, int64_t k_lo, int64_t count, int conj, double scale,
                       int64_t row_len, hipStream_t st, double ramp = 0.0, int64_t ramp_center = 0);

}
}
```

quantum_inferno_amd/csrc/qi_plan_build.hip:

```cpp
#include <algorithm>

#include "qi_host.hpp"

using namespace qi;

namespace qi {
namespace host {

bool native_len_ok(int64_t Lf) { return Lf == (1ll << 20) || Lf == (1ll << 21); }

int64_t table_low_bins(const qi_plan* p, int kind) {
  const auto& t = p->nat[kind];
  if (!t.ready || p->d.dtype != QI_F32 || !p->native_fwd || !p->native_fwd_low || !native_len_ok(t.Lf)) return 0;
  if (!t.h_rows.empty() || (kind == 0 && p->nat[3].ready && p->nedge > 0)) return 0;
  const int64_t kmax = native::fwd_low_bins(t.Lf);
  int64_t K = 1;
  while (K <= kmax && !(t.x_lo > -K && t.x_hi < K)) K *= 2;
  return K <= kmax ? K : 0;
}
bool forward_low(const qi_plan* p) {
  if (p->d.dtype != QI_F32) return false;
  bool any = false;
  for (int kind = 0; kind < 3; ++kind) {
    if (!p->nat[kind].ready) continue;
// ... 92 lines not shown
  int wq;
  int64_t shift;
  int analytic = 0;
  double kappa = 0.0, cw = 0.0, amp = 0.0;
};
int block_group_of(double reach) { return reach <= 256.0 ? 1 : (reach <= 512.0 ? 2 : (reach <= 1024.0 ? 4 : 0)); }
void gabor_gaussian(BlockPick& pk, double p_re, double om, double am) {
  pk.kappa = om * (double)native::kBlk / (2.0 * M_PI);
  pk.cw = (2.0 * M_PI / (double)native::kBlk) * std::sqrt(M_LOG2E / (4.0 * p_re));
  pk.amp = am * std::sqrt(M_PI / p_re) / (double)native::kBlk;
}
void stx_gaussian(BlockPick& pk, int64_t n, double sigma) {
  pk.kappa = (double)pk.shift * (double)native::kBlk / (double)n;
  pk.cw = (2.0 * M_PI / (double)native::kBlk) * sigma * std::sqrt(M_LOG2E / 2.0);
  pk.amp = 1.0 / (double)native::kBlk;
}

double2 unit_root(int64_t m, int64_t N, bool negative) {
  const long double two_pi = 6.283185307179586476925286766559005768L;
  const long double ang = (negative ? -two_pi : two_pi) * (long double)(((m % N) + N) % N) / (long double)N;
  return make_double2((double)cosl(ang), (double)sinl(ang));
}

int upload_zoom_list(qi_plan* p, qi_plan::NativeTable& t, int64_t Lf, std::vector<native::BandDesc>& bands, bool stx) {
  std::vector<native::BandDesc> rest;
  std::vector<std::vector<native::BandDesc>> by_level(native::kZoomClasses);
  for (const auto& d : bands) {
    if (d.mode >= 2) by_level[d.mode - 2].push_back(d);
    else rest.push_back(d);
  }
  auto join = [&](int from, int to) {
    by_level[to].insert(by_level[to].begin(), by_level[from].begin(), by_level[from].end());
    by_level[from].clear();
  };
  if (!by_level[6].empty() && by_level[6].size() < 6) join(6, 5);
  if (!by_level[5].empty() && by_level[5].size() < 6) join(5, 0);
  for (int g = 0; g + 1 < native::kZoomLevels; ++g) {
    if (by_level[g].empty() || by_level[g].size() >= 6) continue;
    for (int h = g + 1; h <= g + 2 && h < native::kZoomLevels; ++h)
      if (!by_level[h].empty()) {
        join(g, h);
        break;
      }
  }
  std::vector<native::BandDesc> zoom;
  t.h_zoom.clear();
  t.zoom_planes = 0;
  t.zoom_max_level = 0;
  t.x_lo = 0;
  t.x_hi = -1;
  for (const auto& lvl : by_level)
    for (const auto& d : lvl) {
      const int64_t lo = d.k_lo + (stx ? d.shift : 0), hi = lo + d.k_len - 1;
      if (t.x_lo > t.x_hi) {
        t.x_lo = lo;
        t.x_hi = hi;
      }
      t.x_lo = lo < t.x_lo ? lo : t.x_lo;
      t.x_hi = hi > t.x_hi ? hi : t.x_hi;
    }
  for (int g = 0; g < native::kZoomClasses; ++g) t.zoom_count[g] = (int32_t)by_level[g].size();
  for (int gi = 0; gi < native::kZoomClasses; ++gi) {
    const int g = kZoomListOrder[gi];
    const int grid = native::zoom_grid(g);
    for (auto d : by_level[g]) {
      d.edge_slot = grid;
      d.edge = (int32_t)t.zoom_planes;
      t.zoom_planes += ((Lf / native::kZoomD) << grid) / native::kBlk;
      if (grid > t.zoom_max_level) t.zoom_max_level = grid;
      zoom.push_back(d);
      t.h_zoom.push_back({d.out_band, g});
    }
  }
  bands.swap(rest);
  if (zoom.empty()) return QI_OK;
  QI_TRY(upload_table(&t.d_zoom, zoom));
  t.nzoom = (int32_t)zoom.size();
  std::vector<int32_t> owner((size_t)t.zoom_planes);
  for (size_t j = 0; j < zoom.size(); ++j) {
    const int64_t planes = ((Lf / native::kZoomD) << zoom[j].edge_slot) / native::kBlk;
    for (int64_t q = 0; q < planes; ++q) owner[(size_t)(zoom[j].edge + q)] = (int32_t)j;
  }
  QI_TRY(upload_table(&t.d_zoom_plane_band, owner));
  for (int g = 0; g < native::kZoomClasses; ++g) {
    const bool needed = t.zoom_count[g] > 0 || (g == 0 && t.zoom_count[5] + t.zoom_count[6] > 0);
    if (p->d_zoom_w[g] || !needed) continue;
    std::vector<float> w((size_t)64 * native::zoom_taps(g));
    native::zoom_weights(g, 0, w.data());
    QI_TRY(upload_table(&p->d_zoom_w[g], w));
  }
  return QI_OK;
}

int order_z64_fine_classes(qi_plan* p, qi_plan::NativeTable& t, int64_t Lf, std::vector<std::vector<native::BandDesc>>& lvl) {
  const int64_t M0 = Lf / 64;
  std::vector<std::vector<native::BandDesc>> cls(native::kZ64FineClasses);
  for (const auto& d : lvl[0]) {
    int c = 0;
    for (int q = native::kZ64FineClasses - 1; q >= native::kZ64FineLevels && c == 0; --q)
      if ((int64_t)native::z64f_oversampling(q) * d.k_len <= M0) c = q;
    cls[c].push_back(d);
  }
  for (int q = native::kZ64FineClasses - 1; q >= native::kZ64FineLevels; --q) {
    if (cls[q].empty() || cls[q].size() >= 4) continue;
    const int to = q == native::kZ64FineLevels ? 0 : q - 1;
    cls[to].insert(cls[to].end(), cls[q].begin(), cls[q].end());
    cls[q].clear();
  }
  lvl[0].clear();
  int32_t pos = 0;
  std::vector<int> order0{0};
  for (int c = native::kZ64FineLevels; c < native::kZ64FineClasses; ++c) order0.push_back(c);
  for (int c : order0) {
    t.zf_first[c] = pos;
    t.zf_count[c] = (int32_t)cls[c].size();
    pos += t.zf_count[c];
    lvl[0].insert(lvl[0].end(), cls[c].begin(), cls[c].end());
  }
  for (int g = 1; g < native::kZ64FineLevels && g < native::kZ64Levels; ++g) {
    t.zf_first[g] = pos;
    t.zf_count[g] = (int32_t)lvl[g].size();
    pos += t.zf_count[g];
  }
  for (int c = 0; c < native::kZ64FineClasses; ++c) {
    if (t.zf_count[c] == 0 || p->d_z64f_w[c]) continue;
    std::vector<double> w((size_t)native::z64f_win(c) * 64);
    native::z64_fine_weights(c, w.data());
    QI_TRY(upload_table(&p->d_z64f_w[c], w));
  }
  return QI_OK;
}

int upload_z64_carriers(qi_plan::NativeTable& t, int kind, int64_t Lf, const std::vector<native::BandDesc>& z) {
  const int e = kind == 0 ? 1 : 0;
  std::vector<double2> lane(z.size() * 65);
  for (size_t j = 0; j < z.size(); ++j) {
    const int64_t kc = (int64_t)z[j].k_lo + z[j].k_len / 2;
    for (int l = 0; l < 64; ++l) lane[j * 65 + l] = unit_root(kc * (l - e), Lf, false);
    lane[j * 65 + 64] = unit_root(kc * 64, Lf, false);
  }
  const int64_t nw = Lf / native::kZ64FineWave;
  std::vector<double2> wave((size_t)nw);
  for (int64_t j = 0; j < nw; ++j) wave[(size_t)j] = unit_root(j * native::kZ64FineWave, Lf, false);
  QI_TRY(upload_table(&t.d_z64_lane_ph, lane));
  return upload_table(&t.d_z64_wave_ph, wave);
}

int upload_z64_list(qi_plan* p, qi_plan::NativeTable& t, int kind, int64_t Lf, std::vector<native::BandDesc>& bands) {
  std::vector<native::BandDesc> rest;
  std::vector<std::vector<native::BandDesc>> lvl(native::kZ64Levels);
  for (const auto& d : bands) {
    const int g = d.mode == 0 ? z64_level(p, kind, Lf, d.k_len) : -1;
    if (g >= 0) lvl[g].push_back(d);
    else rest.push_back(d);
  }
  for (int c = 0; c < native::kZ64FineClasses; ++c) t.zf_first[c] = t.zf_count[c] = 0;
  if (p->native_z64_fine) QI_TRY(order_z64_fine_classes(p, t, Lf, lvl));
  std::vector<native::BandDesc> z;
  for (int g = 0; g < native::kZ64Levels; ++g) {
    t.z64_first[g] = (int32_t)z.size();
    t.z64_count[g] = (int32_t)lvl[g].size();
    z.insert(z.end(), lvl[g].begin(), lvl[g].end());
    if (!lvl[g].empty() && !p->d_z64_w[g]) {
      const int log2d = 6 - g;
      std::vector<double> w((size_t)(1 << log2d) * native::kZ64Taps);
      native::z64_weights(log2d, w.data());
// ... 172 lines not shown
  const double half8 = std::ceil(std::sqrt(drop_bits(false)) / (0.5 * pk.cw));
  const int64_t klo8 = long_window(pk);
  return 2.0 * pk.kappa - half8 - 1.0 >= (double)klo8 && 2.0 * pk.kappa + half8 + 1.0 <= (double)(klo8 + 255);
}

template <typename T>
int block_band_desc(const qi_plan* p, const BlockPick& pk, int32_t row, bool is_long, native::BlockBandT<T>* out) {
  constexpr bool F64 = sizeof(T) == 8;
  native::BlockBandT<T>& b = *out;
  memset(&b, 0, sizeof(b));
  b.out_band = pk.band;
  b.bank_row = row;
  b.shift = (int32_t)pk.shift;
  b.analytic = p->native_blk_analytic ? pk.analytic : 0;
  const double grid = is_long ? 2.0 : 1.0;
  const double kappa = grid * pk.kappa, cw = pk.cw / grid;
  b.kappa_int = (int32_t)std::floor(kappa);
  b.kappa_frac = (T)(kappa - std::floor(kappa));
  b.cw = (T)cw;
  b.amp = (T)(pk.amp / grid);
  const double half = std::ceil(std::sqrt(drop_bits(F64)) / cw);
  if (F64 && !b.analytic) {
    set_error("block engine: float64 tables take analytic (Gaussian) bands only");
    return QI_ERR_STATE;
  }
  if ((!F64 || (b.analytic == 1 && p->native_blk64_wtab && p->native_blk64_narrow)) && b.analytic && p->native_blk_narrow &&
      2.0 * half + 2.0 <= 256.0) {
    b.narrow = 1;
    b.klo = is_long ? (int32_t)long_window(pk)
                    : (int32_t)((((int64_t)std::llround(kappa) - 128) % native::kBlk + native::kBlk) % native::kBlk);
    const int ba = b.klo >> 8;
    b.rot_a[0] = (T)std::cos(2.0 * M_PI * ba / 16.0);
    b.rot_a[1] = (T)std::sin(2.0 * M_PI * ba / 16.0);
    b.rot_b[0] = (T)std::cos(2.0 * M_PI * ((ba + 1) & 15) / 16.0);
    b.rot_b[1] = (T)std::sin(2.0 * M_PI * ((ba + 1) & 15) / 16.0);
    b.rot8_a[0] = (T)std::cos(M_PI * ba / 16.0);
    b.rot8_a[1] = (T)std::sin(M_PI * ba / 16.0);
    b.rot8_b[0] = (T)std::cos(M_PI * (ba + 1) / 16.0);
    b.rot8_b[1] = (T)std::sin(M_PI * (ba + 1) / 16.0);
  } else if (!F64 && b.analytic && p->native_blk_half && kappa - half - 1.0 >= 0.0 && kappa + half + 1.0 < (double)(native::kBlk / 2)) {
    b.narrow = 2;
  }
  if (b.analytic && p->native_blk_fastw && b.amp > (T)0 && kappa - half - 1.0 >= 0.0 && kappa + half + 1.0 < (double)native::kBlk) {
    b.nowrap = 1;
    b.la = (T)std::log2(pk.amp / grid);
  }
  for (int k = 0; k < 4; ++k) {
    const int64_t m = (int64_t)(((__int128)pk.shift * 256 * (1 << k)) % p->n);
    const double ang = -2.0 * M_PI * (double)m / (double)p->n;
    b.rot[2 * k] = (T)std::cos(ang);
    b.rot[2 * k + 1] = (T)std::sin(ang);
  }
  const int64_t m1 = pk.shift % p->n;
  b.rot1[0] = (T)std::cos(-2.0 * M_PI * (double)m1 / (double)p->n);
  b.rot1[1] = (T)std::sin(-2.0 * M_PI * (double)m1 / (double)p->n);
  return QI_OK;
}

template <typename T>
std::vector<native::BlockItem> block_cut_items(const qi_plan* p, int kind, int cut, qi_plan::BlockTable::ItemList& il,
                                               const std::vector<native::BlockBandT<T>>& list, const int32_t* first,
                                               const int32_t* count, int64_t split_blocks) {
  std::vector<native::BlockItem> items;
  for (int g = 0; g < kBlockGroups; ++g) {
    if (count[g] == 0) continue;
    const int per_wg = cut == 0 ? p->native_blk_bands : p->native_blk_bands_batch;
    const int32_t nchunk = (int32_t)ceil_div(count[g], per_wg);
    const int64_t nblocks = ceil_div(p->n, native::block_valid(kBlockGroupWq[g]));
    if (tune_env("QI_NATIVE_VERBOSE")) {
      auto count_if = [&](auto pred) { return (int)std::count_if(list.begin() + first[g], list.begin() + first[g] + count[g], pred); };
      fprintf(stderr, "[qi plan] block table %d cut %d, reach <= %d%s: %d bands (%d analytic, %d narrow, %d half) in %d workgroups x %lld blocks\n", kind, cut,
              g == 3 ? 1024 : 256 * (kBlockGroupWq[g] & 15), g == 3 ? " (8192-sample blocks)" : "", count[g],
              count_if([](const native::BlockBandT<T>& b) { return b.analytic != 0; }),
              count_if([](const native::BlockBandT<T>& b) { return b.narrow == 1; }),
              count_if([](const native::BlockBandT<T>& b) { return b.narrow == 2; }), nchunk, (long long)nblocks);
    }
    for (int32_t c = 0; c < nchunk; ++c) {
      const int32_t lo = first[g] + (int32_t)((int64_t)count[g] * c / nchunk);
      const int32_t hi = first[g] + (int32_t)((int64_t)count[g] * (c + 1) / nchunk);
      for (int64_t b = 0; b < nblocks; ++b) items.push_back({kBlockGroupWq[g], (int32_t)b, lo, hi - lo, il.nplanes, 0});
      il.nplanes += 1;
    }
  }
  std::stable_sort(items.begin(), items.end(), [](const native::BlockItem& x, const native::BlockItem& y) {
    const bool lx = x.wq == native::kBlkLongWq, ly = y.wq == native::kBlkLongWq;
    return lx != ly ? lx : x.band_count > y.band_count;
  });
  for (size_t i = 0; i < items.size(); ++i) items[i].stat_slot = (int32_t)i;
  il.nitems = (int32_t)items.size();
  il.nlong = (int32_t)std::count_if(items.begin(), items.end(), [](const native::BlockItem& x) { return x.wq == native::kBlkLongWq; });
  if (kind == 0 && p->nsplit > 0) {
    const int wq = (int)(p->native_split_e / 512);
    il.edge_merged = (cut == 1 && p->native_edge_merge != 0) || sizeof(T) == 8;
    if (il.edge_merged) {
      for (int64_t b = 0; b < split_blocks; ++b)
        items.push_back({-wq, (int32_t)b, 0, p->nsplit, il.nplanes, (int32_t)items.size()});
      il.nplanes += 1;
    } else {
      for (int32_t sb = 0; sb < p->nsplit; ++sb) {
        for (int64_t b = 0; b < split_blocks; ++b)
          items.push_back({-wq, (int32_t)b, sb, 0, il.nplanes, (int32_t)items.size()});
        il.nplanes += 1;
      }
    }
    il.nedge_items = (int32_t)items.size() - il.nitems;
  }
  return items;
}

std::vector<double> block_gauss_weights(const std::vector<native::BlockBandT<double>>& list, int demod) {
  std::vector<double> gw(list.size() * (size_t)native::kBlk);
  for (size_t q = 0; q < list.size(); ++q) {
    const auto& b = list[q];
    for (int k = 0; k < native::kBlk; ++k) {
      if (b.analytic == 2) {
        double acc = 0.0;
        for (int m = -6; m <= 6; ++m) {
          const double e = (double)b.cw * ((double)(k - b.kappa_int) - (double)b.kappa_frac + (double)native::kBlk * m);
          acc += ((m & 1) && !demod ? -1.0 : 1.0) * std::exp2(-e * e);
        }
        gw[q * native::kBlk + k] = (double)b.amp * acc;
        continue;
      }
      double dk = (double)(k - b.kappa_int) - (double)b.kappa_frac, amp = (double)b.amp;
      if (dk > (double)(native::kBlk / 2)) {
        dk -= (double)native::kBlk;
        if (!demod) amp = -amp;
      }
      if (demod && dk < -(double)(native::kBlk / 2)) dk += (double)native::kBlk;
      const double e = (double)b.cw * dk;
      gw[q * native::kBlk + k] = amp * std::exp2(-e * e);
    }
  }
  return gw;
}

int upload_demod_tables(qi_plan* p, qi_plan::BlockTable::ItemList& il, const std::vector<native::BlockBandT<double>>& list) {
  std::vector<double2> pw(list.size() * 16);
  for (size_t q = 0; q < list.size(); ++q)
    for (int i = 0; i < 16; ++i) pw[q * 16 + i] = unit_root((int64_t)(((__int128)list[q].shift * 256 * i) % p->n), p->n, true);
  QI_TRY(upload_table(&il.d_demod_pow, pw));
  if (p->d_demod_t1 || p->n < 1024) return QI_OK;
  std::vector<double2> t1((size_t)(p->n / 1024)), t2(1024);
  for (int64_t j = 0; j < p->n / 1024; ++j) t1[(size_t)j] = unit_root(1024 * j, p->n, true);
  for (int64_t j = 0; j < 1024; ++j) t2[(size_t)j] = unit_root(j, p->n, true);
  QI_TRY(upload_table(&p->d_demod_t1, t1));
  return upload_table(&p->d_demod_t2, t2);
}

template <typename T>
int finish_block_table(qi_plan* p, int kind, int demod, const std::vector<BlockPick>& picks, double2* taps,
                       hipStream_t st) {
  constexpr bool F64 = sizeof(T) == 8;
  auto& bt = p->blk[kind];
  bt.release();
  p->dual_valid[0] = p->dual_valid[1] = false;
  if (picks.empty()) return QI_OK;
  const int32_t rows = (int32_t)picks.size();
  QI_TRY(fft_c2c<double>(p->fft, taps, native::kBlk, rows, HIPFFT_FORWARD, st));
  if (!demod) QI_TRY(native::launch_block_rotate_rows(taps, rows, st));
  QI_HIP(hipMalloc(&bt.bank, (size_t)rows * native::kBlk * sizeof(cplx<T>)));
  QI_TRY(launch_bank_convert<T>(taps, static_cast<cplx<T>*>(bt.bank), (int64_t)rows * native::kBlk, 0,
                                1.0 / (double)native::kBlk, st));
  bt.rows = rows;
  bt.demod = demod;
  const bool edges = kind == 0 && p->nsplit > 0;
// ... 432 lines not shown
```

quantum_inferno_amd/csrc/qi_run.hip:

```cpp
#include "qi_host.hpp"

using namespace qi;

namespace qi {
namespace host {



struct Tile {
  int64_t Ct, Bt, ntb, nblk;
  size_t off_x, off_y, off_pb, off_ps;
};

template <typename T>
int plan_tiles(const qi_plan* p, int64_t C, int64_t B, int64_t L, Tile* t) {
  const size_t row = (size_t)L * sizeof(cplx<T>);
  const int64_t nblk = ceil_div(p->n, kEpiSpan);
  const size_t part = align_up((size_t)B * nblk * 8) + align_up((size_t)B * nblk * 24);
  const size_t per_chan_full = row * (size_t)(B + 1) + part + 2048;
  int64_t Ct, Bt;
  if (per_chan_full <= p->ws_bytes) {
    Bt = B;
    Ct = (int64_t)(p->ws_bytes / per_chan_full);
    if (Ct > C) Ct = C;
// ... 479 lines not shown
      a.chunk_base = chunk_base;
      if (grp.ngen > 0) {
        p->prof.begin(st, QI_STAGE_PASS1);
        QI_TRY(native::launch_pass1<T>(a, sb.kernel_kind, ct, st));
        p->prof.end(QI_STAGE_PASS1, st);
      }
      p->prof.begin(st, QI_STAGE_PASS2);
      QI_TRY(native::launch_pass2<T>(a, sb.kernel_kind, G, sb.nchunk[g], ct, st));
      p->prof.end(QI_STAGE_PASS2, st);
      chunk_base += sb.nchunk[g];
    }
  }
  return QI_OK;
}

template <typename T>
native::BlockArgs<T> block_args(const qi_plan* p, const qi_plan::BlockTable& bt, const qi_plan::BlockTable::ItemList& il,
                                const TileOut<T>& v, const T* sig, cplx<T>* zadd, int32_t nsplit, int64_t stat_base,
                                int chunk_base) {
  native::BlockArgs<T> b{};
  b.n = v.n;
  b.nitems = il.nitems;
  b.nedge_items = il.nedge_items;
  b.edge_merged = il.edge_merged ? 1 : 0;
  b.nsplit = nsplit;
  b.edge_band = p->d_split_bands;
  b.edge_bank = static_cast<const cplx<T>*>(p->split_bank);
  b.edge_part = zadd;
  b.panel_bands = (int32_t)v.B;
  b.items = il.d_items;
  b.bands = static_cast<const native::BlockBandT<T>*>(il.d_bands);
  b.bank = static_cast<const cplx<T>*>(bt.bank);
  b.sig = sig;
  v.fill(b);
  b.stat_base = stat_base;
  b.chunk_base = chunk_base;
  b.two_over_n = (float)(2.0 / (double)v.n);
  b.debug = p->native_debug;
  b.stamps = p->blk_stamps;
  return b;
}

template <typename T>
int launch_edges(const qi_plan* p, const TileOut<T>& v, const Scratch<T>& s, const T* sig, int64_t ct, hipStream_t st) {
  native::EdgeArgs<T> e{};
  e.bands = p->d_edge;
  e.nedge = p->nedge;
  e.panel_bands = (int32_t)v.B;
  e.n = v.n;
  e.wmax = p->edge_wmax;
  e.stat_slots = v.stat_slots;
  e.sig = sig;
  v.fill_panel(e);
  e.edge_z = s.edge_z;
  e.edge_p = s.edge_p;
  return native::launch_edge<T>(e, ct, v.out_time ? s.edge_time : nullptr, v.part_band, v.nbk, v.nbk - 1, v.part_stat,
                                v.stat_slots - p->nedge, st);
}

template <typename T>
native::TailCall<T> tail_call(const TileOut<T>& v, int64_t ct, const int32_t* band_slots) {
  native::TailCall<T> t;
  t.time_part = v.time_part;
  t.out_time = v.out_time;
  t.ct = ct;
  t.n = v.n;
  t.chunk_total = v.chunk_total;
  t.part_band = v.part_band;
  t.part_stat = v.part_stat;
  t.power_band = v.power_band;
  t.stats = v.stats;
  t.B = v.B;
  t.nbk = v.nbk;
  t.stat_slots = v.stat_slots;
  t.band_slots = band_slots;
  return t;
}

template <typename T>
int launch_reductions(const native::TailCall<T>& t, bool time_via_part, bool one_launch, hipStream_t st) {
  const bool sums = t.part_band || t.part_stat;
  if (time_via_part && sums && one_launch) return native::launch_tail<T>(t, st);
  if (time_via_part)
    QI_TRY(native::launch_time_reduce<T>(t.time_part, t.out_time, t.ct, t.n, t.chunk_total, t.edge_time, t.wmax, st));
  if (sums)
    QI_TRY(launch_finalize(t.part_band, t.part_stat, t.power_band, t.stats, t.ct, t.B, t.nbk, t.stat_slots, st, t.band_slots));
  return QI_OK;
}


struct ZoomRows {
  int count[native::kZoomClasses] = {}, nchunk[native::kZoomClasses] = {};
  int64_t stat_base[native::kZoomClasses] = {}, groups[native::kZoomClasses] = {};
  int planes = 0;
  int64_t stats = 0, slots = 0;
};

ZoomRows plan_zoom_rows(const qi_plan* p, int kind, int64_t C, bool joint) {
  constexpr int NL = native::kZoomClasses;
  const auto& zt = p->nat[kind];
  const int64_t n = p->n;
  ZoomRows r;
  for (int g = 0; g < NL; ++g) r.count[g] = zt.zoom_count[g];
  if (C < p->native_zoom_short_from) {
    r.count[0] += r.count[5] + r.count[6];
    r.count[5] = r.count[6] = 0;
  }
  if (zt.nzoom <= 0) return r;
  const double level_cost[NL] = {1.0, 1.08, 1.25, 0.75, 1.0, 0.85, 0.75};
  int64_t wgs = 0;
  for (int g = 0; g < NL; ++g) {
    if (r.count[g] <= 0) continue;
    r.groups[g] = native::zoom_groups(n, g);
    r.nchunk[g] = 1;
    wgs += r.groups[g] * C;
  }
  const int64_t zoom_wgs = p->native_zoom_wgs > 0 ? p->native_zoom_wgs : (joint && p->native_fuse > 3 ? p->native_zoom_wgs_joint : 0);
  if (zoom_wgs > 0) {
    for (;;) {
      int best = -1;
      double best_load = 0.0;
      for (int g = 0; g < NL; ++g) {
        if (r.count[g] <= 0 || r.nchunk[g] >= r.count[g]) continue;
        const double load = level_cost[g] * (double)ceil_div(r.count[g], r.nchunk[g]);
        if (load > best_load) {
          best_load = load;
          best = g;
        }
      }
      if (best < 0 || wgs + r.groups[best] * C > zoom_wgs) break;
      bool is_max = true;
      for (int g = 0; g < NL; ++g)
        if (r.count[g] > 0 && level_cost[g] * (double)ceil_div(r.count[g], r.nchunk[g]) > best_load) is_max = false;
      if (!is_max) break;
      r.nchunk[best] += 1;
      wgs += r.groups[best] * C;
    }
  } else {
    for (int g = 0; g < NL; ++g) {
      if (r.count[g] <= 0) continue;
      int nc = (int)ceil_div(p->native_zoom_waves, 4 * r.groups[g] * C);
      if (nc < 1) nc = 1;
      if (nc > r.count[g]) nc = r.count[g];
      r.nchunk[g] = nc;
    }
  }
  for (int g = 0; g < NL; ++g) {
    if (r.count[g] <= 0) continue;
    r.planes += r.nchunk[g];
    r.stat_base[g] = r.stats;
    r.stats += (int64_t)r.nchunk[g] * r.groups[g];
    if (r.groups[g] > r.slots) r.slots = r.groups[g];
  }
  if (tune_env("QI_NATIVE_VERBOSE"))
    fprintf(stderr, "[qi run] zoom launch of table %d: bands per class %d %d %d %d %d | 6-tap %d 4-tap %d in rows %d %d %d %d %d | %d %d\n", kind,
            r.count[0], r.count[1], r.count[2], r.count[3], r.count[4], r.count[5],
            r.count[6], r.nchunk[0], r.nchunk[1], r.nchunk[2], r.nchunk[3], r.nchunk[4], r.nchunk[5], r.nchunk[6]);
  return r;
}

int upload_band_slots(qi_plan* p, int kind, int cut, int64_t nblk_max, bool blocks) {
  if (p->d_band_slots[kind][cut]) return QI_OK;
  std::vector<int32_t> slots((size_t)p->nat[kind].nbands, 0);
  for (int32_t r : p->nat[kind].h_rows) slots[r] = (int32_t)nblk_max;
  for (const auto& z : p->nat[kind].h_zoom) slots[z.first] = (int32_t)native::zoom_groups(p->n, z.second);
  if (blocks)
    for (const auto& b : p->blk[kind].var[cut].h_bands) slots[b.first] = b.second;
  return upload_table(&p->d_band_slots[kind][cut], slots);
}

native::ZoomArgs<float> zoom_args(const qi_plan* p, int kind, const ZoomRows& r, const TileOut<float>& v, const Scratch<float>& s,
                                  bool x_shift, int32_t nsplit, int64_t stat_base, int chunk_base) {
  using T = float;
  const auto& zt = p->nat[kind];
  const int64_t n = v.n;
  native::ZoomArgs<T> z{};
  z.n = n;
  z.Lf = zt.Lf;
  z.planes = zt.zoom_planes;
  z.nbands = zt.nzoom;
  z.panel_bands = (int32_t)v.B;
  z.bands = zt.d_zoom;
  z.plane_band = zt.d_zoom_plane_band;
  z.X = s.X;
  z.x_shift = x_shift ? 1 : 0;
  z.x_mask = (uint32_t)((forward_low(p) ? native::fwd_low_len(zt.Lf) : zt.Lf) << z.x_shift) - 1u;
  z.Hc = static_cast<const cplx<T>*>(zt.Hc);
  z.coarse = s.zoom;
  z.stx = kind == 2 ? 1 : 0;
  z.lane_off = kind == 0 ? 1 : 0;
  z.tau_off = kind == 2 ? 0 : n / 2 / native::kZoomD;
  z.inv_len = (T)(1.0 / (double)zt.Lf);
  z.two_over_len = (float)(2.0 / (double)zt.Lf);
  v.fill(z);
  z.chunk_base = chunk_base;
  z.split_part = s.zadd;
  z.split_rows = nsplit;
  z.debug = p->native_debug;
  int chunk0 = 0;
  for (int g = 0; g < native::kZoomClasses; ++g) {
    z.lvl_count[g] = r.count[g];
    z.lvl_chunk0[g] = chunk0;
    z.lvl_nchunk[g] = r.nchunk[g];
    z.lvl_stat_base[g] = stat_base + r.stat_base[g];
    z.lvl_weights[g] = p->d_zoom_w[g];
    chunk0 += r.nchunk[g];
  }
  int first = 0;
  for (int gi = 0; gi < native::kZoomClasses; ++gi) {
    const int g = kZoomListOrder[gi];
    z.lvl_first[g] = first;
    first += r.count[g];
    if (g == 0 && r.count[0] != zt.zoom_count[0]) z.lvl_first[0] = 0;
  }
  return z;
}

int launch_zoom_stage(qi_plan* p, const native::ZoomArgs<float>& z, FusedCarry* defer, FusedCarry* finish,
                      int64_t ct, hipStream_t st) {
  using T = float;
  if (defer) {
    defer->zoom = z;
    defer->has_zoom = true;
    defer->ct = ct;
    return QI_OK;
  }
  const bool joint = finish && finish->has_zoom && finish->ct == ct;
  p->prof.begin(st, QI_STAGE_ZOOM_COARSE);
  const bool gfused = p->native_gather_fused > 0 && ct >= p->native_gather_fused;
  if (joint && gfused) {
    QI_TRY(native::launch_zoom_coarse_gather2<T>(finish->zoom, z, ct, st));
  } else if (joint) {
    QI_TRY(native::launch_zoom_gather2<T>(finish->zoom, z, ct, st));
    QI_TRY(native::launch_zoom_coarse2<T>(finish->zoom, z, ct, st));
  } else if (gfused) {
    QI_TRY(native::launch_zoom_coarse_gather<T>(z, ct, st));
  } else {
    QI_TRY(native::launch_zoom_gather<T>(z, ct, st));
    QI_TRY(native::launch_zoom_coarse<T>(z, ct, st));
  }
  p->prof.end(QI_STAGE_ZOOM_COARSE, st);
  p->prof.begin(st, QI_STAGE_ZOOM);
  const bool joint_fine = joint && p->native_fuse > 3 && (finish->zoom.coef != nullptr) == (z.coef != nullptr) &&
                          (finish->zoom.bits != nullptr) == (z.bits != nullptr);
  if (joint_fine) {
    QI_TRY(native::launch_zoom2<T>(finish->zoom, z, ct, st));
  } else {
    if (joint) QI_TRY(native::launch_zoom<T>(finish->zoom, ct, st));
    QI_TRY(native::launch_zoom<T>(z, ct, st));
  }
  if (joint) finish->has_zoom = false;
  p->prof.end(QI_STAGE_ZOOM, st);
  return QI_OK;
}

int launch_block_stage(qi_plan* p, const native::BlockArgs<float>& b, int demod, int cut, FusedCarry* defer, FusedCarry* finish,
                       int64_t ct, hipStream_t st) {
  using T = float;
  if (defer) {
    defer->blk = b;
    defer->demod = demod;
    defer->ct = ct;
    return QI_OK;
  }
  const bool joint = finish && p->native_fuse > 1 && finish->ct == ct && !finish->demod && demod &&
                     (finish->blk.coef != nullptr) == (b.coef != nullptr) && (finish->blk.bits != nullptr) == (b.bits != nullptr);
  p->prof.unchain_span();
  p->prof.begin(st, QI_STAGE_BLOCK);
  if (joint) {
    QI_TRY(build_dual_items(p, cut));
    QI_TRY(native::launch_block_dual<T>(finish->blk, b, p->d_dual[cut], p->n_dual[cut], p->n_dual_long[cut],
                                        p->blk[0].var[cut].nedge_items, ct, st));
  } else {
    if (finish) QI_TRY(native::launch_block<T>(finish->blk, finish->demod, finish->ct, st));
    QI_TRY(native::launch_block<T>(b, demod, ct, st));
  }
  p->prof.end(QI_STAGE_BLOCK, st);
  p->prof.unchain_span();
  return QI_OK;
}

int launch_tails(FusedCarry* finish, const native::TailCall<float>& tc, hipStream_t st) {
  finish->active = false;
  const native::TailCall<float>& t0 = finish->tail;
  if (t0.ct == tc.ct && t0.n == tc.n) return native::launch_tail2<float>(t0, tc, st);
  QI_TRY(native::launch_tail<float>(t0, st));
  return native::launch_tail<float>(tc, st);
}

template <typename T>
int run_native(qi_plan* p, int kind, const void* sig_v, int64_t C, const qi_tfr_out* out, hipStream_t st, bool may_share,
               FusedCarry* defer, FusedCarry* finish, size_t* probe) {
  static_assert(std::is_same<T, float>::value, "the native engine is float32");
  const int64_t n = p->n, B = p->nat[kind].nbands, Lf0 = p->nat[kind].Lf;
  const T* sig = static_cast<const T*>(sig_v);
  const int G = p->native_rows;
  const TwoPass tp = plan_two_pass(p, kind, C, G);
  const bool shorts = tp.shorts;
  const int chunk_p2 = tp.chunk_total;
  int chunk_total = chunk_p2;
  const auto& bt = p->blk[kind];
  const bool blocks = kind != 1 && bt.ready;
  const int cut = C >= batch_from(p) ? 1 : 0;
  const auto& il = bt.var[cut];
  int64_t blk_stats = 0, blk_slots = 0;
  if (blocks) {
    chunk_total += il.nplanes;
    blk_stats = il.nitems + il.nedge_items;
    blk_slots = bt.max_blocks;
  }
  const auto& zt = p->nat[kind];
  const bool zoom = zt.nzoom > 0;
  const ZoomRows zr = plan_zoom_rows(p, kind, C, defer || (finish && (finish->active || probe)));
  const int chunk_z0 = chunk_total;
  chunk_total += zr.planes;
  int64_t nbk = tp.nblk_max + (shorts ? 1 : 0);
  if (blk_slots > nbk) nbk = blk_slots;
  if (zr.slots > nbk) nbk = zr.slots;
  const int64_t p2_stats = (int64_t)chunk_p2 * tp.nblk_max;
  const int64_t stat_slots = p2_stats + blk_stats + zr.stats + (shorts ? p->nedge : 0);
  const bool sums = out->power_band || out->stats;
  const bool time_via_part = out->power_time && (chunk_total > 1 || shorts);
  if (!shorts) QI_TRY(upload_band_slots(p, kind, cut, tp.nblk_max, blocks));
  const int32_t* band_slots = shorts ? nullptr : p->d_band_slots[kind][cut];
  bool share = may_share && kind == 2 && (probe || (p->shared_valid && p->shared_sig == sig_v && p->shared_C == C)) &&
               p->nat[kind].h_rows.empty() && !shorts;
  const int32_t nsplit = kind == 0 ? p->nsplit : 0;
  ScratchBytes e = scratch_bytes<T>(p, n, B, nbk, stat_slots, chunk_total, shorts, time_via_part, out->coef != nullptr, nsplit);
  const bool low = forward_low(p);
  const int64_t x_len = low ? native::fwd_low_len(Lf0) : Lf0;
  const int64_t fwd_imd = low ? native::fwd_low_rows(Lf0 / native::kN2) * native::kN2 : Lf0;
  if (tune_env("QI_NATIVE_VERBOSE"))
    fprintf(stderr, "[qi run] forward transform of table %d (Lf = %lld): %s, bins read (-%lld, %lld)\n", kind, (long long)Lf0,
            low ? "low bins" : "every bin", (long long)table_low_bins(p, kind), (long long)table_low_bins(p, kind));
  e.x = (size_t)(share ? 2 * x_len : x_len) * sizeof(cplx<T>);
  e.imd = (size_t)(tp.imd_elems < fwd_imd ? fwd_imd : tp.imd_elems) * sizeof(cplx<T>);
  e.zoom = zoom ? (size_t)zt.zoom_planes * native::kBlk * sizeof(cplx<T>) : 0;
  const size_t per_chan = e.per_record();
  if (probe) {
    *probe = per_chan;
    return QI_OK;
  }
  if (p->ws_bytes < per_chan + 4096) {
    set_error("workspace of %zu bytes cannot hold one record's native scratch of %zu bytes", p->ws_bytes,
              per_chan + 4096);
    return QI_ERR_NOMEM;
  }
  int64_t Ct = (int64_t)((p->ws_bytes - 4096) / per_chan);
  if (Ct > C) Ct = C;
  if (share && Ct != C) {
    set_error("internal: shared spectra need all records in one tile");
    return QI_ERR_STATE;
  }
  const bool tail_one = time_via_part && sums && p->native_tail;
  const bool deferring = defer && kind == 0 && Ct == C && blocks && !shorts && tail_one;
  bool finishing = finish && finish->active && kind == 2 && share && blocks && tail_one;
  if (finishing) {
    const size_t need = align_up(e.x * (size_t)C) + align_up(finish->ws_used) + (per_chan - e.x) * (size_t)C + 64 * 256;
    if (need > p->ws_bytes) finishing = false;
  }
  if (finish && finish->active && !finishing) QI_TRY(flush_carry(p, finish, st));
  if (kind == 0) {
    p->shared_valid = Ct == C;
    p->shared_sig = sig_v;
    p->shared_C = C;
  } else if (!share) {
    p->shared_valid = false;
  }
  QI_LAYOUT_BEGIN(p, kind == 0 ? "run_native styx" : (kind == 1 ? "run_native atoms" : "run_native stx"), finishing);
  Arena ar{p, p->ws, Ct, "native scratch", share};
  Scratch<T> s{};
  s.X = ar.carve<cplx<T>>(e.x);
  if (finishing) ar.w = p->ws + align_up(finish->ws_used);
  s.Xn = ar.carve<cplx<T>>(e.xn);
  s.imd = ar.carve<cplx<T>>(e.imd);
  ar.carve_reductions(e, &s);
  s.zoom = e.zoom ? ar.carve<cplx<T>>(e.zoom) : nullptr;
  s.zadd = e.add ? ar.carve<cplx<T>>(e.add) : nullptr;
  for (int64_t c0 = 0; c0 < C; c0 += Ct) {
    const int64_t ct = (C - c0 < Ct) ? C - c0 : Ct;
    const T* sig_t = sig + c0 * n;
    const TileOut<T> v = tile_out<T>(out, c0, B, n, time_via_part ? s.time_part : nullptr, s.part_band, s.part_stat, nbk,
                                     stat_slots, chunk_total);
    if (shorts) QI_HIP(hipMemsetAsync(s.parts0, 0, s.parts_bytes, st));
    QI_TRY(launch_spectra<T>(p, sig_t, n, Lf0, shorts, share, low, s, ct, st));
    QI_TRY(launch_two_pass<T>(p, tp, v, s, G, tp.nblk_max, true, ct, st));
    if (zoom)
      QI_TRY(launch_zoom_stage(p, zoom_args(p, kind, zr, v, s, share, nsplit, p2_stats + blk_stats, chunk_z0),
                               deferring && p->native_fuse > 2 ? defer : nullptr, finishing ? finish : nullptr, ct, st));
    if (finishing && finish->has_zoom) {
      QI_TRY(launch_zoom_all(p, finish->zoom, finish->ct, st));
      finish->has_zoom = false;
    }
    if (blocks) {
      native::BlockArgs<T> b = block_args<T>(p, bt, il, v, sig_t, s.zadd, nsplit, p2_stats, chunk_p2);
      b.nlong = il.nlong;
      QI_TRY(launch_block_stage(p, b, bt.demod, cut, deferring ? defer : nullptr, finishing ? finish : nullptr, ct, st));
    }
    p->prof.begin(st, QI_STAGE_EPILOGUE);
    if (shorts) QI_TRY(launch_edges<T>(p, v, s, sig_t, ct, st));
    native::TailCall<T> tc = tail_call<T>(v, ct, band_slots);
    if (deferring) {
      defer->tail = tc;
      defer->ws_used = (size_t)(ar.w - p->ws);
      defer->active = true;
    } else if (finishing) {
      QI_TRY(launch_tails(finish, tc, st));
    } else {
      tc.edge_time = shorts ? s.edge_time : nullptr;
      tc.wmax = p->edge_wmax;
      QI_TRY(launch_reductions<T>(tc, time_via_part, p->native_tail != 0, st));
    }
    p->prof.end(QI_STAGE_EPILOGUE, st);
  }
  return QI_OK;
}


struct Z64Rows {
  bool fine = false;
  int zchunk[native::kZ64Levels] = {};
  int frow[native::kZ64FineClasses] = {};
  size_t z_off[native::kZ64Levels] = {};
  size_t bytes = 0;
  int chunks = 0;
};

Z64Rows plan_z64_rows(const qi_plan* p, const qi_plan::NativeTable& t, int64_t C) {
  using T = double;
  const int64_t n = p->n, Lf = t.Lf;
  Z64Rows r;
  for (int c = 0; c < native::kZ64FineClasses; ++c) r.fine = r.fine || t.zf_count[c] > 0;
  const int64_t tiles_f = n / ((int64_t)native::kZ64FineWave * 4);
  for (int g = 0; g < native::kZ64Levels; ++g) {
    if (t.z64_count[g] == 0) continue;
    r.z_off[g] = r.bytes / sizeof(cplx<T>);
    r.bytes += (size_t)t.z64_count[g] * (size_t)(((Lf / 64) << g) + 2 * native::kZ64Pad) * sizeof(cplx<T>);
    if (r.fine && g < native::kZ64FineLevels) continue;
    int nc = (int)ceil_div(p->native_wgs, (n / native::kZ64Tile) * C);
    r.zchunk[g] = nc < 1 ? 1 : (nc > t.z64_count[g] ? t.z64_count[g] : nc);
    r.chunks += r.zchunk[g];
  }
  for (int c = 0; c < native::kZ64FineClasses; ++c) {
    if (t.zf_count[c] == 0) continue;
    double work = 0.0, mine = (double)t.zf_count[c] * (2.0 * native::z64f_win(c) + 40.0);
    for (int q = 0; q < native::kZ64FineClasses; ++q) work += (double)t.zf_count[q] * (2.0 * native::z64f_win(q) + 40.0);
    const double want_rows = std::max<double>((double)p->native_z64_rows, (double)p->native_wgs / (double)(tiles_f * C));
    int nr = (int)std::ceil(want_rows * (mine / work));
    r.frow[c] = nr < 1 ? 1 : (nr > t.zf_count[c] ? t.zf_count[c] : nr);
    r.chunks += r.frow[c];
  }
  return r;
}

int launch_z64_stage(qi_plan* p, int kind, const Z64Rows& r, const TileOut<double>& v, const Scratch<double>& s, int32_t nsplit,
                     int64_t stat_nblk, int chunk_base, int64_t ct, hipStream_t st) {
  using T = double;
  const auto& t = p->nat[kind];
  const int64_t n = v.n, Lf = t.Lf;
  native::Z64Args zl[native::kZ64Levels];
  for (int g = 0; g < native::kZ64Levels; ++g) {
    if (t.z64_count[g] == 0) continue;
    native::Z64Args& z = zl[g];
    z = native::Z64Args{};
    z.Lf = Lf;
    z.n = n;
    z.log2d = 6 - g;
    z.M = Lf >> z.log2d;
    z.kind = kind;
    z.nbands = t.z64_count[g];
    z.panel_bands = (int32_t)v.B;
    z.bands = t.d_z64 + t.z64_first[g];
    z.X = s.X;
    z.Hc = static_cast<const cplx<T>*>(t.Hc);
    z.Z = s.zoom + r.z_off[g] * (size_t)ct;
    z.weights = p->d_z64_w[g];
    z.inv_len = 1.0 / (double)Lf;
    z.two_over_len = (float)(2.0 / (double)Lf);
    z.split_part = s.zadd;
    z.split_rows = nsplit;
    v.fill(z);
    z.nblk = n / native::kZ64Tile;
    z.pb_stride = v.nbk;
    z.stat_nblk = stat_nblk;
// ... 250 lines not shown
```

quantum_inferno_amd/engine.py:

```python
import collections
import ctypes as C
import os
import threading
from dataclasses import dataclass
from typing import Optional

import numpy as np
import torch

from . import _lib
from . import scales_dyadic as scales

_EPI_SPAN = 1024


def _real_dtype(dtype):
    if dtype in (torch.float32, np.float32, "float32", "f32"):
        return torch.float32
    if dtype in (torch.float64, np.float64, "float64", "f64", float):
        return torch.float64
    raise TypeError(f"unsupported dtype {dtype}: float32 or float64")


def _complex_of(rdtype):
# ... 116 lines not shown
    def __init__(self, n, dtype=torch.float32, device=None, workspace_bytes=None, engine=_lib.QI_ENGINE_AUTO):
        self._lib = _lib.require_gpu()
        self.n = int(n)
        self.rdtype = _real_dtype(dtype)
        self.device = torch.device(device) if device is not None else default_device()
        if self.device.index is None:
            self.device = torch.device("cuda", torch.cuda.current_device())
        self.workspace_bytes = int(workspace_bytes) if workspace_bytes else 0
        self._handle = C.c_void_p()
        if os.environ.get("QI_FORCE_HIPFFT"):
            engine = _lib.QI_ENGINE_HIPFFT
        desc = _lib.PlanDesc(
            n=self.n,
            dtype=_lib.QI_F64 if self.rdtype == torch.float64 else _lib.QI_F32,
            device=self.device.index,
            engine=engine,
            flags=0,
            workspace_bytes=self.workspace_bytes,
        )
        _lib.check(self._lib.qi_plan_create(C.byref(self._handle), C.byref(desc)))
        self.freq = {}
        self._stage = None

    @staticmethod
    def workspace_for(n, n_bands, dtype, channels=1, cap_bytes=8 << 30):
        esz = 16 if _real_dtype(dtype) == torch.float64 else 8
        length = 2 * n if (n & (n - 1)) == 0 else 1 << (2 * n - 2).bit_length()
        nblk = -(-n // _EPI_SPAN)
        per_chan = (max(n_bands, 2) + 1) * length * esz + n_bands * nblk * 32 + 4096
        build = min(n_bands, 16) * length * 16
        need = max(per_chan * channels, build, 1 << 24)
        return int(min(max(need, per_chan), max(cap_bytes, per_chan)))

    def _stream(self):
        return _lib.stream_ptr(self.device)

    def set_gabor_bank(self, which, f_hz, p_re, p_im, omega, amp):
        keep = [_lib.darr(a) for a in (p_re, p_im, omega, amp)]
        with torch.cuda.device(self.device):
            _lib.check(
                self._lib.qi_plan_set_gabor_bank(
                    self._handle, which, len(keep[0][0]), keep[0][1], keep[1][1], keep[2][1], keep[3][1], self._stream()
                )
            )
        self.freq[which] = np.asarray(f_hz)

    def set_styx_bank(self, order, fs, dictionary_type="norm"):
        f_hz, p_re, p_im, omega, amp, _ = styx_bank_tables(order, self.n, fs, dictionary_type)
        self.set_gabor_bank(_lib.QI_BANK_STYX, f_hz, p_re, p_im, omega, amp)
        return f_hz

    def set_stx_bands(self, order, fs):
        f_hz = scales.log_frequency_hz_from_fft_points(fs, self.n, order)
        idx = scales.stx_shift_indices(f_hz, self.n, fs)
        sigma = scales.cycles_from_order(order) / (2 * np.pi * f_hz / fs)
        self.set_stx_table(f_hz, idx, sigma)
        return f_hz

    def set_stx_table(self, f_hz, shift_index, sigma):
        ia, ip = _lib.iarr(shift_index)
        sa, sp = _lib.darr(sigma)
        if len(ia) != len(sa):
            raise ValueError("shift_index and sigma must have one entry per band")
        _lib.check(self._lib.qi_plan_set_stx_bands(self._handle, len(ia), ip, sp))
        self.freq[_lib.QI_TABLE_STX] = np.asarray(f_hz)
        self.stx_index = ia

    def profile(self, enable=True, stages=None, period=1):
        code = 1 if enable else 0
        if enable and stages is not None:
            code = 0
            for name in stages:
                code |= 1 << (_lib.STAGES.index(name) + 1)
        if enable and period > 1:
            code |= int(period) << 16
        _lib.check(self._lib.qi_plan_profile(self._handle, code))

    def stage_bands(self, stage):
        k = _lib.STAGES.index(stage)
        return [int(self._lib.qi_plan_stage_bands(self._handle, which, k)) for which in (0, 1, 2)]

    def forward_low(self, which):
        return int(self._lib.qi_plan_forward_low(self._handle, which))

    def band_route(self, which, band, records=1):
        r = _lib.BandRoute()
        _lib.check(self._lib.qi_plan_band_route(self._handle, which, int(band), int(records), C.byref(r)))
        return _lib.STAGES[r.stage], r.cls, r.run_cls, r.flags

    def profile_read(self):
        ms = (C.c_double * len(_lib.STAGES))()
        cnt = (C.c_int64 * len(_lib.STAGES))()
        _lib.check(self._lib.qi_plan_profile_read(self._handle, ms, cnt, len(_lib.STAGES)))
        return {name: (ms[i], cnt[i]) for i, name in enumerate(_lib.STAGES)}

    def _signal(self, sig):
        if sig.dtype != self.rdtype or not sig.is_cuda or sig.device != self.device:
            sig = sig.to(device=self.device, dtype=self.rdtype)
        sig = sig.contiguous()
        if sig.dim() != 2 or sig.shape[1] != self.n:
            raise ValueError(f"signal must be [channels, {self.n}], got {tuple(sig.shape)}")
        return sig

    def _outputs(self, which, n_ch, coef, bits, reductions, power_scale, eps, out, reduced_out):
        f_hz = self.freq.get(which)
        if f_hz is None:
            raise _lib.QiError("band table not set on this plan")
        n_b = len(f_hz)
        dev = self.device
        if out is not None:
            res = out
            if (res.coef is not None and res.coef.shape[0] != n_ch) or (res.stats is not None and res.stats.shape[0] != n_ch):
                raise ValueError("out= buffers were made for another channel count")
            res.power_scale = power_scale
        else:
            res = TfrResult(frequency_hz=f_hz, power_scale=power_scale)
            if coef:
                res.coef = torch.empty((n_ch, n_b, self.n), dtype=_complex_of(self.rdtype), device=dev)
            if bits:
                res.bits = torch.empty((n_ch, n_b, self.n), dtype=self.rdtype, device=dev)
            if reductions:
                res.reduced, res.power_band, res.power_time, res.stats = reduced_views(
                    n_ch, n_b, self.n, self.rdtype, dev, reductions, reduced_out)
        desc = _lib.TfrOut(
            coef=_lib.ptr(res.coef),
            bits=_lib.ptr(res.bits),
            power_band=_lib.ptr(res.power_band),
            power_time=_lib.ptr(res.power_time),
            stats=_lib.ptr(res.stats),
            power_scale=float(power_scale),
            eps=float(eps),
        )
        return res, desc

    def _run(self, which, sig, coef, bits, reductions, power_scale, eps, out=None, reduced_out=None):
        sig = self._signal(sig)
        n_ch = sig.shape[0]
        res, desc = self._outputs(which, n_ch, coef, bits, reductions, power_scale, eps, out, reduced_out)
        with torch.cuda.device(self.device):
            if which == _lib.QI_TABLE_STX:
                rc = self._lib.qi_stx(self._handle, _lib.ptr(sig), n_ch, C.byref(desc), self._stream())
            else:
                rc = self._lib.qi_cwt(self._handle, which, _lib.ptr(sig), n_ch, C.byref(desc), self._stream())
        _lib.check(rc)
        return res

    def cwt_stx(self, sig, coef=True, bits=False, reductions=False, power_scale=1.0, eps=0.0, out=None, reduced_out=None):
        sig = self._signal(sig)
        n_ch = sig.shape[0]
        out = out or (None, None)
        reduced_out = reduced_out or (None, None)
        res_c, desc_c = self._outputs(_lib.QI_BANK_STYX, n_ch, coef, bits, reductions, power_scale, eps, out[0], reduced_out[0])
        res_s, desc_s = self._outputs(_lib.QI_TABLE_STX, n_ch, coef, bits, reductions, power_scale, eps, out[1], reduced_out[1])
        with torch.cuda.device(self.device):
            rc = self._lib.qi_cwt_stx(self._handle, _lib.QI_BANK_STYX, _lib.ptr(sig), n_ch, C.byref(desc_c),
                                      C.byref(desc_s), self._stream())
        _lib.check(rc)
        return res_c, res_s

    def cwt(self, sig, coef=True, bits=False, reductions=False, power_scale=1.0, eps=0.0, out=None, reduced_out=None):
        return self._run(_lib.QI_BANK_STYX, sig, coef, bits, reductions, power_scale, eps, out, reduced_out)

    def cwt_atoms(self, sig, coef=True, bits=False, reductions=False, power_scale=1.0, eps=0.0, out=None, reduced_out=None):
        return self._run(_lib.QI_BANK_ATOMS, sig, coef, bits, reductions, power_scale, eps, out, reduced_out)

    def stx(self, sig, coef=True, bits=False, reductions=False, power_scale=1.0, eps=0.0, out=None, reduced_out=None):
# ... 322 lines not shown
```

Before: 423,300 Mpoints/s.

## Fold earlier time-partial planes into block stage and precompute zoom plane descriptors

The block-stage kernels now read time partial rows written by earlier stages (pass2 and zoom) and add them into their own time-partial output. The tail time-reduce then skips those folded planes, cutting the number of planes it reads per time sample. Separately, the zoom coarse gather loads a per-plane BandDesc directly instead of going through the plane-to-band indirection table. The cost is extra loads in the block kernel and the requirement that earlier stages finish writing before the block stage reads their rows.

Result: no change. 425,800 Mpoints/s (median of 6 runs) (+0.6%).

```diff
diff --git a/include/qi_tfr.h b/include/qi_tfr.h
--- a/include/qi_tfr.h
+++ b/include/qi_tfr.h
@@ -77,6 +77,8 @@
 int64_t qi_plan_stage_bands(const qi_plan* plan, int which, int stage);
 
 int64_t qi_plan_forward_low(const qi_plan* plan, int which );
+
+int64_t qi_plan_time_fold(const qi_plan* plan, int which, int64_t records, int joint, int32_t* earlier, int32_t* block_planes);
 
 typedef struct {
   int32_t stage, cls, run_cls, flags;
diff --git a/quantum_inferno_amd/_lib.py b/quantum_inferno_amd/_lib.py
--- a/quantum_inferno_amd/_lib.py
+++ b/quantum_inferno_amd/_lib.py
@@ -79,6 +79,7 @@
     "qi_plan_bands": (_i64, [_P, _int]),
     "qi_plan_stage_bands": (_i64, [_P, _int, _int]),
     "qi_plan_forward_low": (_i64, [_P, _int]),
+    "qi_plan_time_fold": (_i64, [_P, _int, _i64, _int, C.POINTER(_i32), C.POINTER(_i32)]),
     "qi_plan_band_route": (_int, [_P, _int, _i32, _i64, C.POINTER(BandRoute)]),
     "qi_plan_profile": (_int, [_P, _int]),
     "qi_plan_profile_read": (_int, [_P, _D, _I64, _i32]),
diff --git a/quantum_inferno_amd/csrc/qi_api.hip b/quantum_inferno_amd/csrc/qi_api.hip
--- a/quantum_inferno_amd/csrc/qi_api.hip
+++ b/quantum_inferno_amd/csrc/qi_api.hip
@@ -45,6 +45,8 @@
   if (const char* e = tune_env("QI_NATIVE_DEBUG")) p->native_debug = atoi(e);
   if (const char* e = tune_env("QI_NATIVE_FWD")) p->native_fwd = atoi(e);
   if (const char* e = tune_env("QI_NATIVE_FWD_LOW")) p->native_fwd_low = atoi(e);
+  if (const char* e = tune_env("QI_NATIVE_TIME_FOLD")) p->native_time_fold = atoi(e);
+  if (const char* e = tune_env("QI_NATIVE_COARSE_DESC")) p->native_coarse_desc = atoi(e);
 #ifdef QI_NATIVE_STAMPS
   if (tune_env("QI_NATIVE_STAMPS")) {
     if (hipMalloc((void**)&p->stamps, 65536 * 8 * sizeof(unsigned long long)) != hipSuccess) p->stamps = nullptr;
@@ -318,6 +320,11 @@
   return table_low_bins(p, which);
 }
 
+int64_t qi_plan_time_fold(const qi_plan* p, int which, int64_t records, int joint, int32_t* earlier, int32_t* block_planes) {
+  if (!p) return 0;
+  return time_fold_planes(p, which, records, joint != 0, earlier, block_planes);
+}
+
 int64_t qi_plan_stage_bands(const qi_plan* p, int which, int stage) {
   if (!p || which < 0 || which > 2) return 0;
   const int64_t total = qi_plan_bands(p, which);
diff --git a/quantum_inferno_amd/csrc/qi_block.hip b/quantum_inferno_amd/csrc/qi_block.hip
--- a/quantum_inferno_amd/csrc/qi_block.hip
+++ b/quantum_inferno_amd/csrc/qi_block.hip
@@ -300,6 +300,13 @@
   for (int c = 0; c < 16; ++c) t[c] = S[brev(c, 4)];
 #pragma unroll
   for (int c = 0; c < 16; ++c) S[c] = t[c];
+}
+
+template <typename T>
+__device__ __forceinline__ const char* fold_source_row(const BlockArgs<T>& a, int64_t ch, int32_t plane) {
+  if ((uint32_t)plane >= (uint32_t)a.fold_k) return nullptr;
+  const int32_t e = a.fold_first + plane;
+  return reinterpret_cast<const char*>(a.time_part + ((int64_t)ch * a.chunk_total + (e < a.fold_p2 ? e : e + a.fold_gap)) * a.n);
 }
 
 template <typename T, int WQ, bool DEMOD, bool COEF, bool BITS, bool EDGE = false>
@@ -529,8 +536,25 @@
   char* __restrict__ time_row = reinterpret_cast<char*>(
       a.time_part ? a.time_part + ((int64_t)ch * a.chunk_total + a.chunk_base + plane) * n : nullptr);
 #pragma unroll
+  for (int i = 0; i < NOUT; i += 2) tot += col_p[i] + col_p[i + 1];
+  if constexpr (!F64 && !EDGE) {
+    if (const char* __restrict__ src_row = fold_source_row(a, ch, plane); src_row && time_row) {
+      float2 src[NOUT / 2];
+#pragma unroll
+      for (int i = 0; i < NOUT; i += 2) {
+        const uint32_t tt = tb_pair + 256u * (uint32_t)i;
+        src[i / 2] = tt < (uint32_t)n ? *reinterpret_cast<const float2*>(src_row + (size_t)(tt * (uint32_t)sizeof(float)))
+                                      : make_float2(0.0f, 0.0f);
+      }
+#pragma unroll
+      for (int i = 0; i < NOUT; i += 2) {
+        col_p[i] += src[i / 2].x;
+        col_p[i + 1] += src[i / 2].y;
+      }
+    }
+  }
+#pragma unroll
   for (int i = 0; i < NOUT; i += 2) {
-    tot += col_p[i] + col_p[i + 1];
     const uint32_t tt = tb_pair + 256u * (uint32_t)i;
     if (time_row && tt < (uint32_t)n) store_real_pair(time_row, tt, col_p[i], col_p[i + 1]);
   }
@@ -696,8 +720,22 @@
   char* __restrict__ time_row = reinterpret_cast<char*>(
       a.time_part ? a.time_part + ((int64_t)ch * a.chunk_total + a.chunk_base + plane) * n : nullptr);
 #pragma unroll
+  for (int i = 0; i < NOUT; ++i) tot += col_p[2 * i] + col_p[2 * i + 1];
+  if (const char* __restrict__ src_row = fold_source_row(a, ch, plane); src_row && time_row) {
+    float2 src[NOUT];
+#pragma unroll
+    for (int i = 0; i < NOUT; ++i) {
+      const uint32_t tt = tb0 + 512u * (uint32_t)i;
+      src[i] = tt < (uint32_t)n ? *reinterpret_cast<const float2*>(src_row + (size_t)(tt * (uint32_t)sizeof(T))) : make_float2(0.0f, 0.0f);
+    }
+#pragma unroll
+    for (int i = 0; i < NOUT; ++i) {
+      col_p[2 * i] += src[i].x;
+      col_p[2 * i + 1] += src[i].y;
+    }
+  }
+#pragma unroll
   for (int i = 0; i < NOUT; ++i) {
-    tot += col_p[2 * i] + col_p[2 * i + 1];
     const uint32_t tt = tb0 + 512u * (uint32_t)i;
     if (time_row && tt < (uint32_t)n)
       *reinterpret_cast<float2*>(time_row + (size_t)(tt * (uint32_t)sizeof(T))) = make_float2(col_p[2 * i], col_p[2 * i + 1]);
@@ -1095,7 +1133,8 @@
 __device__ __forceinline__ void zoom_coarse_plane_gather(const ZoomArgs<T>& a, const uint32_t plane_i,
                                                          cplx<T>* __restrict__ buf, cplx<T>* __restrict__ tw256) {
   const int tid = threadIdx.x, col = fft4096_col(tid);
-  const BandDesc bd = load_uniform(a.bands + *as_const(a.plane_band + plane_i));
+  const BandDesc bd = a.plane_desc ? load_uniform(a.plane_desc + plane_i)
+                                   : load_uniform(a.bands + *as_const(a.plane_band + plane_i));
   const uint32_t tau1 = plane_i - (uint32_t)bd.edge;
   const int64_t ch = blockIdx.z;
   const cplx<T>* __restrict__ X = a.X + ch * ((int64_t)a.x_mask + 1);
diff --git a/quantum_inferno_amd/csrc/qi_host.hpp b/quantum_inferno_amd/csrc/qi_host.hpp
--- a/quantum_inferno_amd/csrc/qi_host.hpp
+++ b/quantum_inferno_amd/csrc/qi_host.hpp
@@ -242,6 +242,7 @@
     void* Hfull = nullptr;
     native::BandDesc* d_zoom = nullptr;
     int32_t* d_zoom_plane_band = nullptr;
+    native::BandDesc* d_zoom_plane_desc = nullptr;
     std::vector<std::pair<int32_t, int32_t>> h_zoom;
     std::vector<int32_t> h_rows;
     std::vector<int32_t> h_row_mode;
@@ -261,6 +262,7 @@
       free_device(d_z64_wave_ph);
       free_device(d_zoom);
       free_device(d_zoom_plane_band);
+      free_device(d_zoom_plane_desc);
       free_device(d_bands);
       free_device(d_gen_list);
       free_device(Hc);
@@ -284,6 +286,7 @@
       std::vector<Route> h_route;
       native::BlockItem* d_items = nullptr;
       int32_t nitems = 0, nplanes = 0;
+      int32_t nband_planes = 0;
       int32_t nlong = 0;
       int32_t nedge_items = 0;
       bool edge_merged = false;
@@ -373,6 +376,8 @@
   int native_debug = 0;
   int native_fwd = 1;
   int native_fwd_low = 1;
+  int native_time_fold = 1;
+  int native_coarse_desc = 1;
   int native_wgs = 256;
   unsigned long long* stamps = nullptr;
   unsigned long long* blk_stamps = nullptr;
@@ -431,6 +436,7 @@
               bool* ran);
 int run_native64(qi_plan* p, int kind, const void* sig_v, int64_t C, const qi_tfr_out* out, hipStream_t st);
 int flush_carry(qi_plan* p, FusedCarry* c, hipStream_t st);
+int64_t time_fold_planes(const qi_plan* p, int kind, int64_t C, bool joint, int32_t* earlier, int32_t* block_planes);
 
 }
 }
diff --git a/quantum_inferno_amd/csrc/qi_native.hip b/quantum_inferno_amd/csrc/qi_native.hip
--- a/quantum_inferno_amd/csrc/qi_native.hip
+++ b/quantum_inferno_amd/csrc/qi_native.hip
@@ -570,16 +570,24 @@
 }
 
 template <typename T, int VEC>
-__device__ __forceinline__ void time_reduce_block(const T* __restrict__ part, T* __restrict__ out, int64_t n, int nchunk,
+__device__ __forceinline__ void time_reduce_block(const T* __restrict__ part, T* __restrict__ out, int64_t n, PlaneSet ps,
                                                   const T* __restrict__ edge_time, int64_t wmax, int64_t bx, int64_t gx,
                                                   int64_t c) {
   struct alignas(sizeof(T) * VEC) Pack {
     T v[VEC];
   };
+  const int nchunk = ps.stride;
+  const int q0 = ps.nskip > 0 && ps.skip0 == 0 ? ps.nskip : 0;
+  const int hole = ps.nskip > 0 && ps.skip0 > 0 ? ps.skip0 : ps.count, hole_end = hole < ps.count ? hole + ps.nskip : ps.count;
   for (int64_t t = (bx * blockDim.x + threadIdx.x) * VEC; t < n; t += gx * blockDim.x * VEC) {
     if (t + VEC <= n) {
-      Pack s = *reinterpret_cast<const Pack*>(part + (c * nchunk) * n + t);
-      for (int q = 1; q < nchunk; ++q) {
+      Pack s = *reinterpret_cast<const Pack*>(part + (c * nchunk + q0) * n + t);
+      for (int q = q0 + 1; q < hole; ++q) {
+        const Pack x = *reinterpret_cast<const Pack*>(part + (c * nchunk + q) * n + t);
+#pragma unroll
+        for (int i = 0; i < VEC; ++i) s.v[i] += x.v[i];
+      }
+      for (int q = hole_end; q < ps.count; ++q) {
         const Pack x = *reinterpret_cast<const Pack*>(part + (c * nchunk + q) * n + t);
 #pragma unroll
         for (int i = 0; i < VEC; ++i) s.v[i] += x.v[i];
@@ -595,7 +603,8 @@
     } else {
       for (int64_t u = t; u < n; ++u) {
         T s = T(0);
-        for (int q = 0; q < nchunk; ++q) s += part[(c * nchunk + q) * n + u];
+        for (int q = q0; q < hole; ++q) s += part[(c * nchunk + q) * n + u];
+        for (int q = hole_end; q < ps.count; ++q) s += part[(c * nchunk + q) * n + u];
         if (edge_time) {
           if (u < wmax) s += edge_time[(c * 2 + 0) * wmax + u];
           if (u >= n - wmax) s += edge_time[(c * 2 + 1) * wmax + (n - 1 - u)];
@@ -606,9 +615,9 @@
   }
 }
 template <typename T, int VEC>
-__global__ void __launch_bounds__(256) k_time_reduce(const T* __restrict__ part, T* __restrict__ out, int64_t n, int nchunk,
+__global__ void __launch_bounds__(256) k_time_reduce(const T* __restrict__ part, T* __restrict__ out, int64_t n, PlaneSet ps,
                                                      const T* __restrict__ edge_time, int64_t wmax) {
-  time_reduce_block<T, VEC>(part, out, n, nchunk, edge_time, wmax, blockIdx.x, gridDim.x, blockIdx.y);
+  time_reduce_block<T, VEC>(part, out, n, ps, edge_time, wmax, blockIdx.x, gridDim.x, blockIdx.y);
 }
 
 struct TailFin {
@@ -620,7 +629,7 @@
   const int32_t* band_slots;
 };
 template <typename T, int VEC>
-__global__ void __launch_bounds__(256) k_tail(const T* __restrict__ part, T* __restrict__ out, int64_t n, int nchunk,
+__global__ void __launch_bounds__(256) k_tail(const T* __restrict__ part, T* __restrict__ out, int64_t n, PlaneSet ps,
                                               const T* __restrict__ edge_time, int64_t wmax, TailFin f, int nfin) {
   __shared__ double s[3][256 / kWave];
   if ((int)blockIdx.x < nfin) {
@@ -628,7 +637,7 @@
                    blockIdx.y, s);
     return;
   }
-  time_reduce_block<T, VEC>(part, out, n, nchunk, edge_time, wmax, (int64_t)blockIdx.x - nfin, (int64_t)gridDim.x - nfin,
+  time_reduce_block<T, VEC>(part, out, n, ps, edge_time, wmax, (int64_t)blockIdx.x - nfin, (int64_t)gridDim.x - nfin,
                             blockIdx.y);
 }
 
@@ -981,16 +990,16 @@
 }
 
 template <typename T>
-int launch_time_reduce(const T* part, T* out, int64_t C, int64_t n, int nchunk, const T* edge_time, int64_t wmax,
+int launch_time_reduce(const T* part, T* out, int64_t C, int64_t n, PlaneSet planes, const T* edge_time, int64_t wmax,
                        hipStream_t st) {
   const bool aligned = n % 4 == 0 && reinterpret_cast<uintptr_t>(out) % (4 * sizeof(T)) == 0 &&
                        reinterpret_cast<uintptr_t>(part) % (4 * sizeof(T)) == 0;
   if (aligned) {
     dim3 g((unsigned)(ceil_div(n, 1024) > 4096 ? 4096 : ceil_div(n, 1024)), (unsigned)C);
-    k_time_reduce<T, 4><<<g, 256, 0, st>>>(part, out, n, nchunk, edge_time, wmax);
+    k_time_reduce<T, 4><<<g, 256, 0, st>>>(part, out, n, planes, edge_time, wmax);
   } else {
     dim3 g((unsigned)(ceil_div(n, 256) > 4096 ? 4096 : ceil_div(n, 256)), (unsigned)C);
-    k_time_reduce<T, 1><<<g, 256, 0, st>>>(part, out, n, nchunk, edge_time, wmax);
+    k_time_reduce<T, 1><<<g, 256, 0, st>>>(part, out, n, planes, edge_time, wmax);
   }
   QI_LAUNCH_CHECK();
   return QI_OK;
@@ -1000,7 +1009,8 @@
   const T* part;
   T* out;
   int64_t n;
-  int nchunk, nfin;
+  PlaneSet planes;
+  int nfin;
   TailFin f;
 };
 template <typename T, int VEC>
@@ -1012,7 +1022,7 @@
                    blockIdx.x, blockIdx.y, s);
     return;
   }
-  time_reduce_block<T, VEC>(p.part, p.out, p.n, p.nchunk, nullptr, 0, (int64_t)blockIdx.x - p.nfin,
+  time_reduce_block<T, VEC>(p.part, p.out, p.n, p.planes, nullptr, 0, (int64_t)blockIdx.x - p.nfin,
                             (int64_t)gridDim.x - p.nfin, blockIdx.y);
 }
 
@@ -1021,14 +1031,14 @@
   const bool aligned = t.n % 4 == 0 && reinterpret_cast<uintptr_t>(t.out_time) % (4 * sizeof(T)) == 0 &&
                        reinterpret_cast<uintptr_t>(t.time_part) % (4 * sizeof(T)) == 0;
   if (!aligned) {
-    if (int rc = launch_time_reduce<T>(t.time_part, t.out_time, t.ct, t.n, t.chunk_total, t.edge_time, t.wmax, st)) return rc;
+    if (int rc = launch_time_reduce<T>(t.time_part, t.out_time, t.ct, t.n, t.planes(), t.edge_time, t.wmax, st)) return rc;
     return launch_finalize(t.part_band, t.part_stat, t.power_band, t.stats, t.ct, t.B, t.nbk, t.stat_slots, st, t.band_slots);
   }
   const TailFin f{t.part_band, t.part_stat, t.power_band, t.stats, t.B, t.nbk, t.stat_slots, t.band_slots};
   const int nfin = (int)t.B + 1;
   const int64_t gt = ceil_div(t.n, 1024) > 4096 ? 4096 : ceil_div(t.n, 1024);
   dim3 g((unsigned)(gt + nfin), (unsigned)t.ct);
-  k_tail<T, 4><<<g, 256, 0, st>>>(t.time_part, t.out_time, t.n, t.chunk_total, t.edge_time, t.wmax, f, nfin);
+  k_tail<T, 4><<<g, 256, 0, st>>>(t.time_part, t.out_time, t.n, t.planes(), t.edge_time, t.wmax, f, nfin);
   QI_LAUNCH_CHECK();
   return QI_OK;
 }
@@ -1043,9 +1053,9 @@
     if (int rc = launch_tail<T>(t0, st)) return rc;
     return launch_tail<T>(t1, st);
   }
-  TailPack<T> p0{t0.time_part, t0.out_time, n, t0.chunk_total, (int)t0.B + 1,
+  TailPack<T> p0{t0.time_part, t0.out_time, n, t0.planes(), (int)t0.B + 1,
                  TailFin{t0.part_band, t0.part_stat, t0.power_band, t0.stats, t0.B, t0.nbk, t0.stat_slots, t0.band_slots}};
-  TailPack<T> p1{t1.time_part, t1.out_time, n, t1.chunk_total, (int)t1.B + 1,
+  TailPack<T> p1{t1.time_part, t1.out_time, n, t1.planes(), (int)t1.B + 1,
                  TailFin{t1.part_band, t1.part_stat, t1.power_band, t1.stats, t1.B, t1.nbk, t1.stat_slots, t1.band_slots}};
   const int64_t gt = ceil_div(n, 1024) > 4096 ? 4096 : ceil_div(n, 1024);
   const int nfin = p0.nfin > p1.nfin ? p0.nfin : p1.nfin;
@@ -1058,8 +1068,8 @@
 template int launch_tail2<double>(const TailCall<double>&, const TailCall<double>&, hipStream_t);
 template int launch_tail<float>(const TailCall<float>&, hipStream_t);
 template int launch_tail<double>(const TailCall<double>&, hipStream_t);
-template int launch_time_reduce<float>(const float*, float*, int64_t, int64_t, int, const float*, int64_t, hipStream_t);
-template int launch_time_reduce<double>(const double*, double*, int64_t, int64_t, int, const double*, int64_t,
+template int launch_time_reduce<float>(const float*, float*, int64_t, int64_t, PlaneSet, const float*, int64_t, hipStream_t);
+template int launch_time_reduce<double>(const double*, double*, int64_t, int64_t, PlaneSet, const double*, int64_t,
                                         hipStream_t);
 
 template <typename T>
diff --git a/quantum_inferno_amd/csrc/qi_native.hpp b/quantum_inferno_amd/csrc/qi_native.hpp
--- a/quantum_inferno_amd/csrc/qi_native.hpp
+++ b/quantum_inferno_amd/csrc/qi_native.hpp
@@ -149,6 +149,7 @@
   float two_over_n;
   int32_t debug;
   unsigned long long* stamps;
+  int32_t fold_k, fold_first, fold_p2, fold_gap;
 };
 int block_valid(int wq);
 template <typename T>
@@ -183,6 +184,7 @@
   int32_t nbands, panel_bands;
   const BandDesc* bands;
   const int32_t* plane_band;
+  const BandDesc* plane_desc;
   int32_t lvl_first[kZoomClasses], lvl_count[kZoomClasses], lvl_chunk0[kZoomClasses], lvl_nchunk[kZoomClasses];
   int64_t lvl_stat_base[kZoomClasses];
   const float* lvl_weights[kZoomClasses];
@@ -315,8 +317,12 @@
 int launch_small_forward(const T* sig, cplx<T>* X2, cplx<T>* X1, const cplx<T>* tw, int64_t tw_len, int64_t n, int64_t ct,
                          hipStream_t st);
 
-template <typename T>
-int launch_time_reduce(const T* part, T* out, int64_t C, int64_t n, int nchunk, const T* edge_time, int64_t wmax,
+struct PlaneSet {
+  int32_t stride = 0, count = 0, skip0 = 0, nskip = 0;
+};
+inline PlaneSet all_planes(int nchunk) { return PlaneSet{nchunk, nchunk, 0, 0}; }
+template <typename T>
+int launch_time_reduce(const T* part, T* out, int64_t C, int64_t n, PlaneSet planes, const T* edge_time, int64_t wmax,
                        hipStream_t st);
 template <typename T>
 struct TailCall {
@@ -324,6 +330,8 @@
   T* out_time = nullptr;
   int64_t ct = 0, n = 0;
   int chunk_total = 0;
+  int sum_planes = -1, skip0 = 0, nskip = 0;
+  PlaneSet planes() const { return PlaneSet{chunk_total, sum_planes < 0 ? chunk_total : sum_planes, skip0, nskip}; }
   const T* edge_time = nullptr;
   int64_t wmax = 0;
   const double* part_band = nullptr;
diff --git a/quantum_inferno_amd/csrc/qi_plan_build.hip b/quantum_inferno_amd/csrc/qi_plan_build.hip
--- a/quantum_inferno_amd/csrc/qi_plan_build.hip
+++ b/quantum_inferno_amd/csrc/qi_plan_build.hip
@@ -198,6 +198,9 @@
     for (int64_t q = 0; q < planes; ++q) owner[(size_t)(zoom[j].edge + q)] = (int32_t)j;
   }
   QI_TRY(upload_table(&t.d_zoom_plane_band, owner));
+  std::vector<native::BandDesc> plane_desc((size_t)t.zoom_planes);
+  for (size_t q = 0; q < plane_desc.size(); ++q) plane_desc[q] = zoom[(size_t)owner[q]];
+  QI_TRY(upload_table(&t.d_zoom_plane_desc, plane_desc));
   for (int g = 0; g < native::kZoomClasses; ++g) {
     const bool needed = t.zoom_count[g] > 0 || (g == 0 && t.zoom_count[5] + t.zoom_count[6] > 0);
     if (p->d_zoom_w[g] || !needed) continue;
@@ -536,6 +539,7 @@
       il.nplanes += 1;
     }
   }
+  il.nband_planes = il.nplanes;
   std::stable_sort(items.begin(), items.end(), [](const native::BlockItem& x, const native::BlockItem& y) {
     const bool lx = x.wq == native::kBlkLongWq, ly = y.wq == native::kBlkLongWq;
     return lx != ly ? lx : x.band_count > y.band_count;
diff --git a/quantum_inferno_amd/csrc/qi_run.hip b/quantum_inferno_amd/csrc/qi_run.hip
--- a/quantum_inferno_amd/csrc/qi_run.hip
+++ b/quantum_inferno_amd/csrc/qi_run.hip
@@ -585,12 +585,36 @@
   const bool sums = t.part_band || t.part_stat;
   if (time_via_part && sums && one_launch) return native::launch_tail<T>(t, st);
   if (time_via_part)
-    QI_TRY(native::launch_time_reduce<T>(t.time_part, t.out_time, t.ct, t.n, t.chunk_total, t.edge_time, t.wmax, st));
+    QI_TRY(native::launch_time_reduce<T>(t.time_part, t.out_time, t.ct, t.n, t.planes(), t.edge_time, t.wmax, st));
   if (sums)
     QI_TRY(launch_finalize(t.part_band, t.part_stat, t.power_band, t.stats, t.ct, t.B, t.nbk, t.stat_slots, st, t.band_slots));
   return QI_OK;
 }
 
+
+struct TimeFold {
+  int k = 0, chunk_p2 = 0, chunk_z0 = 0, chunk_total = 0;
+  template <typename T>
+  void fill(native::BlockArgs<T>& b) const {
+    b.fold_k = k;
+    b.fold_first = chunk_p2 + (chunk_total - chunk_z0) - k;
+    b.fold_p2 = chunk_p2;
+    b.fold_gap = chunk_z0 - chunk_p2;
+  }
+  template <typename T>
+  void fill(native::TailCall<T>& t) const {
+    const int zoom_rows = chunk_total - chunk_z0, kz = k < zoom_rows ? k : zoom_rows;
+    t.sum_planes = chunk_total - kz;
+    t.skip0 = chunk_p2 - (k - kz);
+    t.nskip = k - kz;
+  }
+};
+TimeFold plan_time_fold(const qi_plan* p, bool time_via_part, int chunk_p2, int block_planes, int chunk_z0, int chunk_total) {
+  TimeFold f{0, chunk_p2, chunk_z0, chunk_total};
+  const int earlier = chunk_p2 + (chunk_total - chunk_z0);
+  if (p->native_time_fold && time_via_part) f.k = earlier < block_planes ? earlier : block_planes;
+  return f;
+}
 
 struct ZoomRows {
   int count[native::kZoomClasses] = {}, nchunk[native::kZoomClasses] = {};
@@ -685,6 +709,7 @@
   z.panel_bands = (int32_t)v.B;
   z.bands = zt.d_zoom;
   z.plane_band = zt.d_zoom_plane_band;
+  z.plane_desc = p->native_coarse_desc ? zt.d_zoom_plane_desc : nullptr;
   z.X = s.X;
   z.x_shift = x_shift ? 1 : 0;
   z.x_mask = (uint32_t)((forward_low(p) ? native::fwd_low_len(zt.Lf) : zt.Lf) << z.x_shift) - 1u;
@@ -791,6 +816,21 @@
   return native::launch_tail<float>(tc, st);
 }
 
+int64_t time_fold_planes(const qi_plan* p, int kind, int64_t C, bool joint, int32_t* earlier, int32_t* block_planes) {
+  if (earlier) *earlier = 0;
+  if (block_planes) *block_planes = 0;
+  if (p->d.dtype != QI_F32 || kind < 0 || kind > 2 || !p->nat[kind].ready || on_small(p, kind) || C <= 0) return 0;
+  const TwoPass tp = plan_two_pass(p, kind, C, p->native_rows);
+  const auto& bt = p->blk[kind];
+  const bool blocks = kind != 1 && bt.ready;
+  const auto& il = bt.var[C >= batch_from(p) ? 1 : 0];
+  const ZoomRows zr = plan_zoom_rows(p, kind, C, joint);
+  const int chunk_z0 = tp.chunk_total + (blocks ? il.nplanes : 0), chunk_total = chunk_z0 + zr.planes;
+  if (earlier) *earlier = tp.chunk_total + zr.planes;
+  if (block_planes) *block_planes = blocks ? il.nband_planes : 0;
+  return plan_time_fold(p, chunk_total > 1 || tp.shorts, tp.chunk_total, blocks ? il.nband_planes : 0, chunk_z0, chunk_total).k;
+}
+
 template <typename T>
 int run_native(qi_plan* p, int kind, const void* sig_v, int64_t C, const qi_tfr_out* out, hipStream_t st, bool may_share,
                FusedCarry* defer, FusedCarry* finish, size_t* probe) {
@@ -824,6 +864,7 @@
   const int64_t stat_slots = p2_stats + blk_stats + zr.stats + (shorts ? p->nedge : 0);
   const bool sums = out->power_band || out->stats;
   const bool time_via_part = out->power_time && (chunk_total > 1 || shorts);
+  const TimeFold fold = plan_time_fold(p, time_via_part, chunk_p2, blocks ? il.nband_planes : 0, chunk_z0, chunk_total);
   if (!shorts) QI_TRY(upload_band_slots(p, kind, cut, tp.nblk_max, blocks));
   const int32_t* band_slots = shorts ? nullptr : p->d_band_slots[kind][cut];
   bool share = may_share && kind == 2 && (probe || (p->shared_valid && p->shared_sig == sig_v && p->shared_C == C)) &&
@@ -898,11 +939,13 @@
     if (blocks) {
       native::BlockArgs<T> b = block_args<T>(p, bt, il, v, sig_t, s.zadd, nsplit, p2_stats, chunk_p2);
       b.nlong = il.nlong;
+      fold.fill(b);
       QI_TRY(launch_block_stage(p, b, bt.demod, cut, deferring ? defer : nullptr, finishing ? finish : nullptr, ct, st));
     }
     p->prof.begin(st, QI_STAGE_EPILOGUE);
     if (shorts) QI_TRY(launch_edges<T>(p, v, s, sig_t, ct, st));
     native::TailCall<T> tc = tail_call<T>(v, ct, band_slots);
+    fold.fill(tc);
     if (deferring) {
       defer->tail = tc;
       defer->ws_used = (size_t)(ar.w - p->ws);
diff --git a/quantum_inferno_amd/engine.py b/quantum_inferno_amd/engine.py
--- a/quantum_inferno_amd/engine.py
+++ b/quantum_inferno_amd/engine.py
@@ -222,6 +222,11 @@
 
     def forward_low(self, which):
         return int(self._lib.qi_plan_forward_low(self._handle, which))
+
+    def time_fold(self, which, records=1, joint=False):
+        e, b = C.c_int32(0), C.c_int32(0)
+        k = self._lib.qi_plan_time_fold(self._handle, which, int(records), 1 if joint else 0, C.byref(e), C.byref(b))
+        return int(k), e.value, b.value
 
     def band_route(self, which, band, records=1):
         r = _lib.BandRoute()
```
